# mattiagualtieri/multimodal-path-omic

Hardware: AMD Instinct MI355X
Metric: slides/sec (fwd+bwd) at 15k-patch bags (higher is better)
Workload: dtype bf16; 1 GPU; MCAT medium whole model fwd+bwd+Adam, 15000x1024 bf16 patch bag + 6x256 omic tokens per slide, ces loss; parallelism=dp1, resident_windows=2, launch=hipgraph(fwd+bwd+adam), setup_replays_before_warmup=40, training_state_rewound_every=48

## Files before the change

include/mpo_hip.h:

```cpp
#ifndef MPO_HIP_H
#define MPO_HIP_H
#include <stddef.h>
#include <stdint.h>

#define MPO_ABI_VERSION 14

#ifdef __cplusplus
extern "C" {
#endif

typedef struct ihipStream_t* mpo_stream_t;

enum { MPO_F32 = 0, MPO_BF16 = 1 };

typedef struct mpo_bag_plan {
    const int32_t* wg_start;
    int32_t n_wg;
    int32_t rows_per_wg;
} mpo_bag_plan;
int mpo_coattn_target_workgroups(void);
enum { MPO_ACT_NONE_ = 0, MPO_ACT_RELU_ = 1, MPO_ACT_ELU_ = 2, MPO_ACT_TANH_ = 3, MPO_ACT_SIGMOID_ = 4 };

int mpo_abi_version(void);
const char* mpo_last_error(void);

int mpo_linear_forward(const float* x, const float* weight, const float* bias, float* y,
                       int rows, int in_features, int out_features, float alpha, int act, mpo_stream_t stream);
int mpo_linear_backward_input(const float* dy, const float* weight, float* dx,
                              int rows, int in_features, int out_features, float alpha, int accumulate,
                              mpo_stream_t stream);
int mpo_linear_backward_weight(const float* dy, const float* x, float* dweight, float* dbias ,
                               int rows, int in_features, int out_features, float alpha, mpo_stream_t stream);

size_t mpo_coattn_saved_floats(int n_slides, int n_q, int embed);
size_t mpo_coattn_workspace_bytes(int n_slides, int n_q, int embed, int max_rows);
int mpo_coattn_mcat_forward(const void* bag, int bag_dtype, const int32_t* cu_rows, int n_slides,
                            int total_rows, int max_rows,
                            const float* query, int n_q, int embed,
                            const float* in_proj_weight, const float* in_proj_bias,
                            const float* out_proj_weight, const float* out_proj_bias,
                            float* out, float* attn_map, float* saved, const mpo_bag_plan* plan ,
                            void* workspace, size_t workspace_bytes, mpo_stream_t stream);
size_t mpo_patch_coattn_workspace_bytes(int n_slides, int n_q, int embed, int patch_dim);
int mpo_patch_coattn_mcat_forward(const void* patches, const int32_t* cu_rows, int n_slides, int total_rows, int max_rows,
                                  int patch_dim, const float* patch_weight, const float* patch_bias, float drop_p,
                                  uint64_t seed, uint64_t offset, const uint64_t* rng_epoch ,
                                  const float* query, int n_q, int embed,
                                  const float* in_proj_weight, const float* in_proj_bias,
                                  const float* out_proj_weight, const float* out_proj_bias,
                                  void* h_bag, float* out, float* attn_map , float* saved,
                                  const mpo_bag_plan* plan , void* workspace, size_t workspace_bytes,
                                  mpo_stream_t stream);
size_t mpo_patch_fc_workspace_bytes(int embed, int patch_dim);
int mpo_patch_fc_forward(const void* patches, const int32_t* cu_rows, int n_slides, int total_rows, int max_rows, int patch_dim,
                         const float* patch_weight, const float* patch_bias, int embed, float drop_p, uint64_t seed,
                         uint64_t offset, const uint64_t* rng_epoch, void* h_bag, const mpo_bag_plan* plan ,
                         void* workspace, size_t workspace_bytes, mpo_stream_t stream);
size_t mpo_patch_fc_f32_workspace_bytes(int backward);
int mpo_patch_fc_f32_forward(const float* patches, int64_t total_rows, int patch_dim, const float* patch_weight,
                             const float* patch_bias, int embed, float drop_p, uint64_t seed, uint64_t offset,
                             const uint64_t* rng_epoch, float x_scale, float* h_bag, void* workspace, size_t workspace_bytes,
                             mpo_stream_t stream);
int mpo_patch_fc_f32_backward(const float* d_h_bag, const float* h_bag , const float* patches, int64_t total_rows,
                              int embed, int patch_dim, float gate, float* d_weight, float* d_bias, void* workspace,
                              size_t workspace_bytes, mpo_stream_t stream);

int mpo_patch_coattn_fwd_bagpass(const void* patches, const void* w_packed, const float* bias, const int32_t* cu_rows, int n_slides,
                                 const float* qk2, void* h_bag, float* part_ml, float* part_ctx, int n_q, int max_rows,
                                 float drop_p, uint64_t seed, uint64_t offset, const mpo_bag_plan* plan ,
                                 mpo_stream_t stream);
int mpo_pack_patch_weight(const float* weight , void* packed, int embed, int patch_dim, mpo_stream_t stream);

int mpo_coattn_mcat_backward(const void* bag, int bag_dtype, const int32_t* cu_rows, int n_slides,
                             int total_rows, int max_rows,
                             const float* query, int n_q, int embed,
                             const float* in_proj_weight, const float* out_proj_weight,
                             const float* saved, const float* attn_map,
                             const float* d_out, const float* d_attn_map,
                             float* d_query, int d_query_accumulate ,
                             void* d_bag, float* d_bag_colsum ,
                             float* d_in_proj_weight, float* d_in_proj_bias,
                             float* d_out_proj_weight, float* d_out_proj_bias,
                             float bag_relu_gate, const mpo_bag_plan* plan ,
                             void* workspace, size_t workspace_bytes, mpo_stream_t stream);

int mpo_patch_epilogue_forward(void* h_bf16, const float* bias, int64_t rows, int cols, float drop_p, uint64_t seed,
                               uint64_t offset, const uint64_t* rng_epoch, mpo_stream_t stream);
size_t mpo_patch_epilogue_backward_workspace_bytes(int64_t n, int cols);
int mpo_patch_epilogue_backward(const void* h_bf16, const void* dy_bf16, void* g_bf16, int64_t n, int cols, float drop_p,
                                float* d_bias , void* workspace, size_t workspace_bytes, mpo_stream_t stream);
int mpo_colsum_bf16(const void* x_bf16, float* out, int64_t rows, int cols, mpo_stream_t stream);

size_t mpo_patch_weight_grad_workspace_bytes(int embed, int patch_dim);
int mpo_patch_weight_grad(const void* g_bf16, const void* patches_bf16, int64_t total_rows, int embed, int patch_dim,
                          float* d_weight, int workgroups, void* workspace, size_t workspace_bytes, mpo_stream_t stream);

int mpo_adam_step_flat(float* params, const float* grads, float* exp_avg, float* exp_avg_sq, int64_t n, float lr,
                       float beta1, float beta2, float eps, float weight_decay, int step,
                       const int32_t* step_dev ,
                       mpo_stream_t stream);

enum { MPO_OPTIM_ADAM = 0, MPO_OPTIM_ADAMAX = 1, MPO_OPTIM_ADADELTA = 2, MPO_OPTIM_SGD = 3 };
int mpo_optim_step_flat(int algorithm, float* params, const float* grads, float* state1, float* state2, int64_t n, float lr,
                        const float* lr_dev, float beta1, float beta2, float eps, float weight_decay, float l1, int step,
                        const int32_t* step_dev, mpo_stream_t stream);
size_t mpo_abs_sum_flat_workspace_bytes(int64_t n);
int mpo_abs_sum_flat(const float* x, int64_t n, float* out, void* workspace, size_t workspace_bytes, mpo_stream_t stream);

int mpo_set_gemm_fast_path(int enabled);

enum { MPO_GEMM_ROUTE_NONE = 0, MPO_GEMM_ROUTE_GENERAL_NB4 = 1, MPO_GEMM_ROUTE_GENERAL_NB8 = 2, MPO_GEMM_ROUTE_FAST = 3,
       MPO_GEMM_ROUTE_ROWS = 4, MPO_GEMM_ROUTE_LONGK = 5 };
int mpo_gemm_last_route(void);
int mpo_gemm_last_group_routes(void);

int mpo_set_coattn_bwd_two_wave(int enabled);

int mpo_set_coattn_bwd_f32_vector(int enabled);

int mpo_set_nacagat_one_pass_key_grad(int enabled);

int mpo_step_counters_bump(uint64_t* rng_epoch, int32_t* adam_step, mpo_stream_t stream);

int mpo_map_block_dot(const float* a_map, const float* b_map, const int32_t* cu_rows, int n_slides, int n_q, float* out,
                      mpo_stream_t stream);
int mpo_map_block_scale(const float* a_map, const float* scale, const int32_t* cu_rows, int n_slides, int n_q, float* out,
                        mpo_stream_t stream);

int mpo_key_projection(const void* hbag_bf16, int64_t rows, int embed, const float* w_k, const float* b_k, float* kbag,
                       mpo_stream_t stream);
size_t mpo_nacagat_saved_floats(int n_slides, int n_q, int embed);
size_t mpo_nacagat_workspace_bytes(int n_slides, int n_q, int embed, int max_rows, int total_rows);
int mpo_coattn_nacagat_forward(const void* kbag, int k_dtype, const void* hbag, int bag_dtype, const int32_t* cu_rows, int n_slides,
                               int total_rows, int max_rows, const float* query, int n_q, int embed,
                               const float* in_proj_weight, const float* in_proj_bias,
                               const float* out_proj_weight, const float* out_proj_bias,
                               float drop_p, uint64_t seed, uint64_t offset, const uint64_t* rng_epoch,
                               float* q_proj, float* out, float* attn_map, float* score_maps,
                               float* saved, const mpo_bag_plan* plan ,
                               void* workspace, size_t workspace_bytes, mpo_stream_t stream);
int mpo_coattn_nacagat_backward(const void* kbag, int k_dtype, const void* hbag, int bag_dtype,
                                const int32_t* cu_rows, int n_slides, int total_rows, int max_rows,
                                const float* query, int n_q, int embed,
                                const float* in_proj_weight, const float* in_proj_bias, const float* out_proj_weight,
                                float drop_p, uint64_t seed, uint64_t offset, const uint64_t* rng_epoch,
                                const float* saved, const float* score_maps, const float* attn_map,
                                const float* d_out, const float* d_attn_map, const float* d_q_proj,
                                float* d_query, int d_query_accumulate ,
                                void* d_kbag, int dk_dtype, float* d_kbag_colsum ,
                                void* d_hbag ,
                                float* d_ctx ,
                                float* d_in_proj_weight, float* d_in_proj_bias,
                                float* d_out_proj_weight, float* d_out_proj_bias, const mpo_bag_plan* plan ,
                                void* workspace, size_t workspace_bytes, mpo_stream_t stream);

int mpo_nacagat_patch_grad(const int32_t* cu_rows, int n_slides, int total_rows, int max_rows, int n_q, int embed,
                           const float* attn_map, const float* d_ctx, const void* addend_bf16, const void* hbag_bf16,
                           void* d_bag_bf16, float relu_gate, float* d_bias, const mpo_bag_plan* plan ,
                           void* workspace, size_t workspace_bytes, mpo_stream_t stream);

int mpo_nacagat_patch_grad_fused(const int32_t* cu_rows, int n_slides, int total_rows, int max_rows, int n_q, int embed,
                                 const float* attn_map, const float* d_ctx, const void* d_kbag_bf16, const float* w_k,
                                 const void* hbag_bf16, void* d_bag_bf16, float relu_gate, float* d_bias,
                                 const mpo_bag_plan* plan , void* workspace, size_t workspace_bytes,
                                 mpo_stream_t stream);


size_t mpo_encoder_saved_floats(int n_slides, int T, int d, int ff, int heads, int layers);
size_t mpo_encoder_workspace_bytes(int n_slides, int T, int d, int ff);
uint64_t mpo_encoder_rng_span(int n_slides, int T, int d, int ff, int layers);
int mpo_encoder_forward(const float* x, int n_branches, int n_slides, int T, int d, int ff, int heads, int layers,
                        const float* const* params, float drop_p, uint64_t seed, uint64_t offset, const uint64_t* rng_epoch,
                        float* y, float* saved, mpo_stream_t stream);
int mpo_encoder_backward(const float* x, int n_branches, int n_slides, int T, int d, int ff, int heads, int layers,
                         const float* const* params, float drop_p, uint64_t seed, uint64_t offset, const uint64_t* rng_epoch,
                         const float* saved, const float* dy, float* dx, float* const* grads,
                         void* workspace, size_t workspace_bytes, mpo_stream_t stream);

size_t mpo_bag_self_attention_saved_floats(int n_bags, int M, int d, int heads);
size_t mpo_bag_self_attention_workspace_bytes(int n_bags, int M, int d, int heads);
int mpo_set_bag_self_attention_bf16x3(int enabled);
int mpo_bag_self_attention_forward(const float* qkv, int n_bags, int M, int d, int heads, float drop_p, uint64_t seed, uint64_t offset,
                                   const uint64_t* rng_epoch, float* out, float* saved, float* attn_map, mpo_stream_t stream);
int mpo_bag_self_attention_backward(const float* qkv, const float* out, const float* saved, const float* d_out, int n_bags, int M, int d,
                                    int heads, float drop_p, uint64_t seed, uint64_t offset, const uint64_t* rng_epoch, float* d_qkv,
                                    void* workspace, size_t workspace_bytes, mpo_stream_t stream);

size_t mpo_gated_pool_saved_floats(int n_slides, int L, int d);
size_t mpo_gated_pool_workspace_bytes(int n_slides, int L, int d);
uint64_t mpo_gated_pool_rng_span(int n_slides, int L, int d);
int mpo_gated_pool_forward(const float* x, int n_branches, int n_slides, int L, int d, const float* const* params,
                           float head_drop_p, float rho_drop_p, uint64_t seed, uint64_t offset, const uint64_t* rng_epoch,
                           float* scores, float* h, int h_interleaved, float* saved, mpo_stream_t stream);
int mpo_gated_pool_backward(const float* x, int n_branches, int n_slides, int L, int d, const float* const* params,
                            float head_drop_p, float rho_drop_p, const float* saved, const float* h,
                            const float* dh, int h_interleaved, const float* d_scores_ext , float* dx,
                            float* const* grads,
                            void* workspace, size_t workspace_bytes, mpo_stream_t stream);

size_t mpo_fusion_head_saved_floats(int n_slides, int hidden, int dout, int n_classes);
size_t mpo_fusion_head_workspace_bytes(int n_slides, int hidden, int dout, int n_classes);
int mpo_fusion_head_forward(const float* hcat, int n_slides, int din, int hidden, int dout, int n_classes,
                            const float* const* params, float* hazards, float* survs, float* y, float* saved,
                            mpo_stream_t stream);
int mpo_fusion_head_backward(const float* hcat, int n_slides, int din, int hidden, int dout, int n_classes,
                             const float* const* params, const float* saved, const float* hazards,
                             const float* survs, const float* y, const float* d_hazards, const float* d_survs,
                             const float* d_y, float* d_hcat, float* const* grads,
                             void* workspace, size_t workspace_bytes, mpo_stream_t stream);

int mpo_survival_head_forward(const float* logits, int n_slides, int n_classes, float* hazards, float* survs, float* y,
                              mpo_stream_t stream);
int mpo_survival_head_backward(const float* hazards, const float* survs, const float* y, const float* d_hazards,
                               const float* d_survs, const float* d_y, int n_slides, int n_classes, float* d_logits,
                               mpo_stream_t stream);

int mpo_ces_loss_forward(const float* hazards, const float* survs, const int64_t* label, const float* censorship,
                         int n_slides, int n_classes, float alpha, float eps, float* loss, float* risk, mpo_stream_t stream);
int mpo_ces_loss_backward(const float* hazards, const float* survs, const int64_t* label, const float* censorship,
                          int n_slides, int n_classes, float alpha, float eps, const float* d_loss, int d_loss_is_scalar,
                          float* d_hazards, float* d_survs, mpo_stream_t stream);

size_t mpo_fusion_head_loss_saved_floats(int n_slides, int hidden, int dout, int n_classes);
int mpo_fusion_head_loss_forward(const float* hcat, int n_slides, int din, int hidden, int dout, int n_classes,
                                 const float* const* params, const int64_t* label, const float* censorship,
                                 const float* slide_weight, float alpha, float eps, float* hazards, float* survs, float* y,
                                 float* loss, float* risk , float* saved, mpo_stream_t stream);
int mpo_fusion_head_loss_backward(const float* hcat, int n_slides, int din, int hidden, int dout, int n_classes,
                                  const float* const* params, const float* saved, float* d_hcat, float* const* grads,
                                  void* workspace, size_t workspace_bytes, mpo_stream_t stream);

int mpo_sct_loss_forward(const float* y, const int64_t* label, const float* censorship, int n_slides, int n_classes,
                         float eps, float* loss, mpo_stream_t stream);
int mpo_sct_loss_backward(const float* y, const int64_t* label, const float* censorship, int n_slides, int n_classes,
                          float eps, const float* d_loss, int d_loss_is_scalar, float* d_y, mpo_stream_t stream);
int mpo_fusion_head_sct_loss_forward(const float* hcat, int n_slides, int din, int hidden, int dout, int n_classes,
                                     const float* const* params, const int64_t* label, const float* censorship,
                                     const float* slide_weight, float eps, float* hazards, float* survs, float* y,
                                     float* loss, float* risk , float* saved, mpo_stream_t stream);

int mpo_ge_head_loss_forward(const float* h, int n_bags, int d, int n_classes, const float* const* params,
                             const int64_t* label, float* y, float* loss, mpo_stream_t stream);
int mpo_ge_head_loss_backward(const float* h, int n_bags, int d, int n_classes, const float* const* params,
                              const int64_t* label, const float* d_loss, float* d_h, float* const* grads,
                              mpo_stream_t stream);

size_t mpo_cag_saved_floats(int rows, int hidden);
size_t mpo_cag_workspace_bytes(int rows, int hidden);
int mpo_cag_forward(const float* q, const float* q_hat, int rows, int dim, int hidden, const float* const* params,
                    float* c_out, float* saved, const float* residual ,
                    float* sum_out , mpo_stream_t stream);
int mpo_cag_backward(const float* q, const float* q_hat, int rows, int dim, int hidden, const float* const* params,
                     const float* saved, const float* c_out, const float* d_c, float* d_q, int d_q_accumulate, float* d_q_hat,
                     float* const* grads, void* workspace, size_t workspace_bytes, mpo_stream_t stream);

size_t mpo_omic_snn_saved_floats(int n_slides, int n_groups, int d);
size_t mpo_omic_snn_workspace_bytes(int n_slides, int n_groups, int d);
uint64_t mpo_omic_snn_rng_span(int n_slides, int n_groups, int d);
int mpo_omic_snn_forward(const float* const* x, const int* widths, int n_groups, int n_slides, int d,
                         const float* const* params, float drop_p, uint64_t seed, uint64_t offset,
                         const uint64_t* rng_epoch, float* g_bag, float* saved, mpo_stream_t stream);
int mpo_omic_snn_backward(const float* const* x, const int* widths, int n_groups, int n_slides, int d,
                          const float* const* params, float drop_p, uint64_t seed, uint64_t offset,
                          const uint64_t* rng_epoch, const float* g_bag, const float* saved, const float* d_g_bag,
                          float* const* grads, void* workspace, size_t workspace_bytes, mpo_stream_t stream);

int mpo_coattn_splits(int n_slides, int max_rows);
int mpo_coattn_fwd_bagpass(const void* bag, int bag_dtype, const int32_t* cu_rows, int n_slides, int embed,
                           const float* qk2, float* part_ml, float* part_ctx, float* raw_logits ,
                           int n_q, int max_rows, const mpo_bag_plan* plan , mpo_stream_t stream);
int mpo_nacagat_fwd_bagpass(const float* kbag, const int32_t* cu_rows, int n_slides, int embed, const float* qs2,
                            const float* tq, float* a_map, float* g_map, int n_q, int max_rows,
                            const mpo_bag_plan* plan , mpo_stream_t stream);
int mpo_coattn_bwd_bagpass(const void* bag, int bag_dtype, const int32_t* cu_rows, int n_slides, int embed,
                           const float* qk2, const float* lse2, const float* dctx, const float* delta,
                           const float* d_attn_map , void* d_bag, float* part_dqk,
                           int n_q, int max_rows, const mpo_bag_plan* plan , mpo_stream_t stream);

#include "mpo_bag_sample.h"

#include "mpo_fusion_next.h"

#include "mpo_cohort.h"

#include "mpo_feature_range.h"

#include "mpo_grad_guard.h"

#include "mpo_eval.h"

#include "mpo_classify.h"

#include "mpo_patch_f16.h"

#ifdef __cplusplus
}
#endif
#endif
```

multimodal_path_omic_amd/csrc/capi.hip:

```cpp
#include <stdarg.h>
#include <stdio.h>
#include <stdlib.h>

#include <algorithm>

#include "../../include/mpo_hip.h"
#include "coattn_tile.h"
#include "mpo_common.h"
#include "mpo_kernels.h"
#include "mpo_layout.h"

static thread_local char g_err[512] = "";

void mpo_set_error(const char* fmt, ...) {
    va_list ap;
    va_start(ap, fmt);
    vsnprintf(g_err, sizeof(g_err), fmt, ap);
    va_end(ap);
}

template <typename T> struct K1Saved { T *qs, *qk2, *ctx, *attn, *lse2; };
template <class A> K1Saved<typename A::elem> k1_saved(A& a, size_t R, size_t E) {
    return {a.floats(R * E), a.floats(R * E), a.floats(R * E), a.floats(R * E), a.floats(R)};
}
// ... 12 lines not shown
    return {a.floats(R * E), a.floats(R * E), a.floats(R * E), a.floats(R * E), a.floats(R * E), a.floats(R), a.floats(R)};
}
struct K2FwdWs { float *part, *hq1, *hq2, *hctx, *tmp_maps; };
template <class A> K2FwdWs k2_fwd_ws(A& a, size_t R, size_t parts, size_t n_q, size_t E, size_t total_rows) {
    K2FwdWs w{a.floats(parts * n_q * E), nullptr, nullptr, nullptr, nullptr};
    if (E == 512) { w.hq1 = a.floats(R * E / 2); w.hq2 = a.floats(R * E / 2); w.hctx = a.floats(R * E / 2); w.tmp_maps = a.floats(2 * n_q * total_rows); }
    return w;
}
struct K2BwdWs { float *dattn, *dctx, *dqt, *dtq, *dq, *spare, *dasum, *part, *part2, *part_cs, *ds1_map, *dg_map, *hb[6], *tmp_map; };
template <class A> K2BwdWs k2_bwd_ws(A& a, size_t R, size_t parts, size_t n_q, size_t E, size_t total_rows, bool colsum) {
    K2BwdWs w{a.floats(R * E), a.floats(R * E), a.floats(R * E), a.floats(R * E), a.floats(R * E), a.floats(R * E), a.floats(R),
              a.floats(parts * n_q * E), a.floats(parts * n_q * E), colsum ? a.floats(parts * E) : nullptr,
              a.floats(n_q * total_rows), a.floats(n_q * total_rows), {}, nullptr};
    if (E == 512) {
        for (float*& h : w.hb) h = a.floats(R * E / 2);
        w.tmp_map = a.floats(2 * n_q * total_rows);
    }
    return w;
}
template <class A> float* k2_patch_grad_ws(A& a, size_t parts, size_t E, bool colsum) { return colsum ? a.floats(parts * E) : nullptr; }

static size_t patch_weight_floats(int embed, int patch_dim) { return (size_t)(embed < 256 ? 256 : embed) * patch_dim / 2; }
static size_t patch_epilogue_bwd_floats(int64_t n, int cols) { return (size_t)mpo_relu_dropout_bwd_blocks((size_t)n, 1) * (size_t)cols; }
static size_t one_block_workspace_bytes(size_t n_floats) {
    WsCount c;
    c.floats(n_floats);
    return c.workspace_bytes();
}

namespace {
bool g_k2_one_pass_key = true;
}

extern "C" int mpo_coattn_target_workgroups(void) {
    return 256;
}

extern "C" int mpo_coattn_splits(int n_slides, int max_rows) {
    const int target = mpo_coattn_target_workgroups();
    int s = (target + n_slides - 1) / n_slides;
    if (s > 512) s = 512;
    const int cap = (max_rows + 127) / 128;
    if (s > cap) s = cap;
    if (s < 1) s = 1;
    return s;
}

static BagPlan make_plan(const mpo_bag_plan* p, int n_slides, int max_rows) {
    BagPlan pl;
    pl.n_slides = n_slides;
    if (p != nullptr && p->wg_start != nullptr) {
        pl.wg_start = p->wg_start;
        pl.n_wg = p->n_wg;
        pl.rows_per_wg = p->rows_per_wg;
    } else {
        pl.splits = mpo_coattn_splits(n_slides, max_rows);
    }
    return pl;
}
static int check_plan(const BagPlan& pl, int n_slides) {
    if (pl.wg_start == nullptr) return 0;
    MPO_CHECK(pl.rows_per_wg >= kTileRows && pl.rows_per_wg % kTileRows == 0, "bag plan: rows_per_wg %d must be a positive multiple of %d",
              pl.rows_per_wg, kTileRows);
    MPO_CHECK(pl.n_wg >= n_slides && pl.n_wg <= mpo_coattn_target_workgroups() + n_slides,
              "bag plan: n_wg %d outside [n_slides, target + n_slides]", pl.n_wg);
    return 0;
}
static size_t max_parts(int n_slides) { return (size_t)mpo_coattn_target_workgroups() + (size_t)n_slides; }

extern "C" {

int mpo_abi_version(void) { return MPO_ABI_VERSION; }
const char* mpo_last_error(void) { return g_err; }

int mpo_linear_forward(const float* x, const float* weight, const float* bias, float* y, int rows, int in_features,
                       int out_features, float alpha, int act, mpo_stream_t stream) {
    return mpo_linear_fwd(x, weight, bias, y, rows, in_features, out_features, alpha, act, stream);
}
int mpo_linear_backward_input(const float* dy, const float* weight, float* dx, int rows, int in_features,
                              int out_features, float alpha, int accumulate, mpo_stream_t stream) {
    return mpo_linear_bwd_input(dy, weight, dx, rows, in_features, out_features, alpha, accumulate, stream);
}
int mpo_linear_backward_weight(const float* dy, const float* x, float* dweight, float* dbias, int rows,
                               int in_features, int out_features, float alpha, mpo_stream_t stream) {
    return mpo_linear_bwd_weight(dy, x, dweight, dbias, rows, in_features, out_features, alpha, stream);
}
size_t mpo_coattn_saved_floats(int n_slides, int n_q, int embed) {
    Count<kPacked> c;
    k1_saved(c, (size_t)n_slides * n_q, embed);
    return c.n_floats();
}

size_t mpo_coattn_workspace_bytes(int n_slides, int n_q, int embed, int max_rows) {
    (void)max_rows;
    WsCount f, b;
    k1_fwd_ws(f, max_parts(n_slides), n_q, embed, 0);
    k1_bwd_ws(b, (size_t)n_slides * n_q, max_parts(n_slides), n_q, embed, true);
    return std::max(f.end, b.end) + kWorkspaceSlack;
}

static int check_common(int bag_dtype, int n_slides, int total_rows, int max_rows, int n_q, int embed) {
    MPO_CHECK(bag_dtype == MPO_F32 || bag_dtype == MPO_BF16, "bag dtype %d is neither MPO_F32 nor MPO_BF16", bag_dtype);
    MPO_CHECK(n_slides >= 1, "n_slides must be >= 1 (got %d)", n_slides);
    MPO_CHECK(n_q >= 1 && n_q <= 16, "number of omic queries must be in 1..16 (got %d)", n_q);
    MPO_CHECK(embed == 128 || embed == 256 || embed == 512, "embed_dim %d not in {128,256,512}", embed);
    MPO_CHECK(max_rows >= 1 && total_rows >= n_slides, "every slide needs at least one patch (total_rows %d, max_rows %d)",
              total_rows, max_rows);
    return 0;
}

struct PatchStep {
    const void* patches;
    const float *weight, *bias;
    int patch_dim;
    float drop_p;
    uint64_t seed, offset;
    const uint64_t* rng_epoch;
    void* h_bag;
};

static int k1_forward(const void* bag, int bag_f32, const PatchStep* patch, const int32_t* cu_rows, int n_slides, int max_rows,
                      const float* query, int n_q, int E, const float* in_w, const float* in_b, const float* out_w,
                      const float* out_b, float* out, float* attn_map, float* saved, const BagPlan& plan, const K1FwdWs& ws,
                      hipStream_t stream) {
    const int R = n_slides * n_q;
    Carve<kPacked> sv(saved);
    const K1Saved<float> S = k1_saved(sv, R, E);
    if (patch) RC(mpo_launch_pack_patch_weight(patch->weight, ws.w_bf16, E, patch->patch_dim, stream));
    RC(mpo_linear_fwd(query, in_w, in_b, S.qs, R, E, E, 1.0f / sqrtf((float)E), MPO_ACT_NONE, stream));
    RC(mpo_linear_bwd_input(S.qs, in_w + (size_t)E * E, S.qk2, R, E, E, kLog2e, 0, stream));
    if (patch) {
        RC(mpo_launch_patch_fc_fwd(patch->patches, ws.w_bf16, patch->bias, cu_rows, patch->h_bag, E, patch->patch_dim, patch->drop_p, patch->seed,
                                   patch->offset, reinterpret_cast<const unsigned long long*>(patch->rng_epoch), plan, stream));
        bag = patch->h_bag;
    }
    RC(mpo_launch_coattn_fwd_partial(bag, bag_f32, cu_rows, n_slides, E, S.qk2, ws.part_ml, ws.part_ctx, attn_map, n_q, plan, stream));
    RC(mpo_launch_coattn_combine(ws.part_ml, ws.part_ctx, S.ctx, S.lse2, n_slides, n_q, E, plan, stream));
    RC(mpo_linear_fwd(S.ctx, in_w + (size_t)2 * E * E, in_b + 2 * E, S.attn, R, E, E, 1.0f, MPO_ACT_NONE, stream));
    RC(mpo_linear_fwd(S.attn, out_w, out_b, out, R, E, E, 1.0f, MPO_ACT_NONE, stream));
    if (attn_map) RC(mpo_launch_coattn_normalize(attn_map, S.lse2, cu_rows, n_slides, n_q, max_rows, 0.f, 0, 0, stream));
    return 0;
}

int mpo_coattn_mcat_forward(const void* bag, int bag_dtype, const int32_t* cu_rows, int n_slides, int total_rows,
                            int max_rows, const float* query, int n_q, int embed, const float* in_w,
                            const float* in_b, const float* out_w, const float* out_b, float* out, float* attn_map,
                            float* saved, const mpo_bag_plan* plan_, void* workspace, size_t workspace_bytes,
                            mpo_stream_t stream) {
    RC(check_common(bag_dtype, n_slides, total_rows, max_rows, n_q, embed));
    const BagPlan plan = make_plan(plan_, n_slides, max_rows);
    RC(check_plan(plan, n_slides));
    WsCarve ws(workspace, workspace_bytes);
    const K1FwdWs W = k1_fwd_ws(ws, plan_parts(plan), n_q, embed, 0);
    MPO_CHECK(ws.ok(), "coattn forward: workspace too small (%zu bytes)", workspace_bytes);
    return k1_forward(bag, bag_dtype == MPO_F32, nullptr, cu_rows, n_slides, max_rows, query, n_q, embed, in_w, in_b, out_w, out_b,
                      out, attn_map, saved, plan, W, stream);
}

size_t mpo_patch_coattn_workspace_bytes(int n_slides, int n_q, int embed, int patch_dim) {
    WsCount c;
    k1_fwd_ws(c, max_parts(n_slides), n_q, embed, (size_t)embed * patch_dim / 2);
    return c.workspace_bytes();
}

int mpo_patch_coattn_mcat_forward(const void* patches, const int32_t* cu_rows, int n_slides, int total_rows, int max_rows,
                                  int patch_dim, const float* patch_weight, const float* patch_bias, float drop_p,
                                  uint64_t seed, uint64_t offset, const uint64_t* rng_epoch,
                                  const float* query, int n_q, int embed, const float* in_w, const float* in_b,
                                  const float* out_w, const float* out_b, void* h_bag, float* out, float* attn_map,
                                  float* saved, const mpo_bag_plan* plan_, void* workspace, size_t workspace_bytes,
                                  mpo_stream_t stream) {
    RC(check_common(MPO_BF16, n_slides, total_rows, max_rows, n_q, embed));
    MPO_CHECK(embed == 256 && patch_dim == 1024, "fused patch layer + co-attention is built for 1024 -> 256 (got %d -> %d)",
              patch_dim, embed);
    const BagPlan plan = make_plan(plan_, n_slides, max_rows);
    RC(check_plan(plan, n_slides));
    WsCarve ws(workspace, workspace_bytes);
    const K1FwdWs W = k1_fwd_ws(ws, plan_parts(plan), n_q, embed, (size_t)embed * patch_dim / 2);
    MPO_CHECK(ws.ok(), "fused patch layer + co-attention: workspace too small (%zu bytes)", workspace_bytes);
    const PatchStep patch{patches, patch_weight, patch_bias, patch_dim, drop_p, seed, offset, rng_epoch, h_bag};
    return k1_forward(nullptr, 0, &patch, cu_rows, n_slides, max_rows, query, n_q, embed, in_w, in_b, out_w, out_b, out, attn_map,
                      saved, plan, W, stream);
}

size_t mpo_patch_fc_workspace_bytes(int embed, int patch_dim) { return one_block_workspace_bytes(patch_weight_floats(embed, patch_dim)); }
int mpo_patch_fc_forward(const void* patches, const int32_t* cu_rows, int n_slides, int total_rows, int max_rows, int patch_dim,
                         const float* patch_weight, const float* patch_bias, int embed, float drop_p, uint64_t seed,
                         uint64_t offset, const uint64_t* rng_epoch, void* h_bag, const mpo_bag_plan* plan_, void* workspace,
                         size_t workspace_bytes, mpo_stream_t stream) {
    RC(check_common(MPO_BF16, n_slides, total_rows, max_rows, 1, embed));
    MPO_CHECK((embed == 128 || embed == 256 || embed == 512) && (patch_dim == 512 || patch_dim == 1024 || patch_dim == 2048),
              "patch layer kernel is built for patch_dim in {512, 1024, 2048} -> embed in {128, 256, 512} (got %d -> %d)", patch_dim, embed);
    MPO_CHECK((int64_t)max_rows * embed * 2 < ((int64_t)1 << 31), "patch layer: a slide's H_bag of 2 GiB or more (%d rows)", max_rows);
    const BagPlan plan = make_plan(plan_, n_slides, max_rows);
    RC(check_plan(plan, n_slides));
    WsCarve ws(workspace, workspace_bytes);
    float* w_bf16 = ws.floats(patch_weight_floats(embed, patch_dim));
    MPO_CHECK(ws.ok(), "patch layer: workspace too small (%zu bytes)", workspace_bytes);
    RC(mpo_launch_pack_patch_weight(patch_weight, w_bf16, embed, patch_dim, stream));
    return mpo_launch_patch_fc_fwd(patches, w_bf16, patch_bias, cu_rows, h_bag, embed, patch_dim, drop_p, seed, offset,
                                   reinterpret_cast<const unsigned long long*>(rng_epoch), plan, stream);
}

size_t mpo_patch_fc_f32_workspace_bytes(int backward) {
    return one_block_workspace_bytes(backward ? mpo_patch_wgrad_f32_workspace_floats() : mpo_patch_fc_f32_workspace_floats());
}
static int patch_fc_f32_forward(const float* patches, int64_t total_rows, int patch_dim, const float* patch_weight,
                                const float* patch_bias, int embed, float drop_p, uint64_t seed, uint64_t offset,
                                const uint64_t* rng_epoch, float x_scale, const float* x_scale_dev, float* h_bag, void* workspace,
                                size_t workspace_bytes, mpo_stream_t stream) {
    MPO_CHECK(patches && patch_weight && patch_bias && h_bag, "fp32 patch layer: null operand");
    MPO_CHECK(total_rows >= 1, "fp32 patch layer: total_rows %lld", (long long)total_rows);
    WsCarve ws(workspace, workspace_bytes);
    float* wpk = ws.floats(mpo_patch_fc_f32_workspace_floats());
    MPO_CHECK(ws.ok(), "fp32 patch layer: workspace too small (%zu bytes)", workspace_bytes);
    return mpo_launch_patch_fc_f32(patches, patch_weight, patch_bias, h_bag, total_rows, embed, patch_dim, drop_p, seed, offset,
                                   reinterpret_cast<const unsigned long long*>(rng_epoch), x_scale, x_scale_dev, wpk, stream);
}
int mpo_patch_fc_f32_forward(const float* patches, int64_t total_rows, int patch_dim, const float* patch_weight,
                             const float* patch_bias, int embed, float drop_p, uint64_t seed, uint64_t offset,
                             const uint64_t* rng_epoch, float x_scale, float* h_bag, void* workspace, size_t workspace_bytes,
                             mpo_stream_t stream) {
    return patch_fc_f32_forward(patches, total_rows, patch_dim, patch_weight, patch_bias, embed, drop_p, seed, offset, rng_epoch,
                                x_scale, nullptr, h_bag, workspace, workspace_bytes, stream);
}
int mpo_patch_fc_f32_forward_dev(const float* patches, int64_t total_rows, int patch_dim, const float* patch_weight,
                                 const float* patch_bias, int embed, float drop_p, uint64_t seed, uint64_t offset,
                                 const uint64_t* rng_epoch, const float* x_scale, float* h_bag, void* workspace,
                                 size_t workspace_bytes, mpo_stream_t stream) {
    MPO_CHECK(x_scale, "fp32 patch layer: null device scale (mpo_feature_range_f32 writes it)");
    return patch_fc_f32_forward(patches, total_rows, patch_dim, patch_weight, patch_bias, embed, drop_p, seed, offset, rng_epoch,
                                1.0f, x_scale, h_bag, workspace, workspace_bytes, stream);
}
int mpo_patch_fc_f32_backward(const float* d_h_bag, const float* h_bag, const float* patches, int64_t total_rows, int embed,
                              int patch_dim, float gate, float* d_weight, float* d_bias, void* workspace, size_t workspace_bytes,
                              mpo_stream_t stream) {
    MPO_CHECK(d_h_bag && patches && d_weight, "fp32 patch layer backward: null operand");
    MPO_CHECK(total_rows >= 1, "fp32 patch layer backward: total_rows %lld", (long long)total_rows);
    WsCarve ws(workspace, workspace_bytes);
    float* part = ws.floats(mpo_patch_wgrad_f32_workspace_floats());
    MPO_CHECK(ws.ok(), "fp32 patch layer backward: workspace too small (%zu bytes)", workspace_bytes);
    return mpo_launch_patch_wgrad_f32(d_h_bag, h_bag, patches, total_rows, embed, patch_dim, gate, d_weight, d_bias, part, stream);
}

size_t mpo_patch_fc_f16_workspace_bytes(int backward) {
    return one_block_workspace_bytes(backward ? mpo_patch_wgrad_f16x_workspace_floats() : mpo_patch_fc_f16_workspace_floats());
}
static int patch_f16_rate(int drop_256, float* p) {
    *p = (float)drop_256 / 256.0f;
    MPO_CHECK(drop_256 >= 0 && drop_256 <= 256, "patch-layer dropout p must be in [0,1) (got %f)", (double)*p);
    MPO_CHECK(drop_256 <= 255, "patch-layer dropout p = %g is realised as round(256 p) / 256 = %u/256: "
              "nothing would be kept (p must be below 1 - 1/512)", (double)*p, (unsigned)drop_256);
    return 0;
}
int mpo_patch_fc_f16_forward(const void* patches, int64_t total_rows, int patch_dim, const float* patch_weight,
                             const float* patch_bias, int embed, int drop_256, uint64_t seed, uint64_t offset,
                             const uint64_t* rng_epoch, float* h_bag, void* workspace, size_t workspace_bytes, mpo_stream_t stream) {
    MPO_CHECK(patches && patch_weight && patch_bias && h_bag, "fp16 patch layer: null operand");
    float drop_p;
    RC(patch_f16_rate(drop_256, &drop_p));
    MPO_CHECK(total_rows >= 1, "fp16 patch layer: total_rows %lld", (long long)total_rows);
    WsCarve ws(workspace, workspace_bytes);
    float* wpk = ws.floats(mpo_patch_fc_f16_workspace_floats());
    MPO_CHECK(ws.ok(), "fp16 patch layer: workspace too small (%zu bytes)", workspace_bytes);
    return mpo_launch_patch_fc_f16(patches, patch_weight, patch_bias, h_bag, total_rows, embed, patch_dim, drop_p, seed, offset,
                                   reinterpret_cast<const unsigned long long*>(rng_epoch), wpk, stream);
}
int mpo_patch_fc_f16_backward(const float* d_h_bag, const float* h_bag, const void* patches, int64_t total_rows, int embed,
                              int patch_dim, int drop_256, float* d_weight, float* d_bias, void* workspace, size_t workspace_bytes,
                              mpo_stream_t stream) {
    MPO_CHECK(d_h_bag && patches && d_weight, "fp16 patch layer backward: null operand");
    float drop_p;
    RC(patch_f16_rate(drop_256, &drop_p));
    const float gate = 256.0f / (256.0f - (float)drop_256);
    MPO_CHECK(total_rows >= 1, "fp16 patch layer backward: total_rows %lld", (long long)total_rows);
    WsCarve ws(workspace, workspace_bytes);
    float* part = ws.floats(mpo_patch_wgrad_f16x_workspace_floats());
    MPO_CHECK(ws.ok(), "fp16 patch layer backward: workspace too small (%zu bytes)", workspace_bytes);
    return mpo_launch_patch_wgrad_f16x(d_h_bag, h_bag, patches, total_rows, embed, patch_dim, gate, d_weight, d_bias, part, stream);
}

int mpo_patch_coattn_fwd_bagpass(const void* patches, const void* w_packed, const float* bias, const int32_t* cu_rows, int n_slides,
                                 const float* qk2, void* h_bag, float* part_ml, float* part_ctx, int n_q, int max_rows,
                                 float drop_p, uint64_t seed, uint64_t offset, const mpo_bag_plan* plan_, mpo_stream_t stream) {
    const BagPlan plan = make_plan(plan_, n_slides, max_rows);
    RC(check_plan(plan, n_slides));
    RC(mpo_launch_patch_fc_fwd(patches, w_packed, bias, cu_rows, h_bag, 256, 1024, drop_p, seed, offset, nullptr, plan, stream));
    if (qk2 == nullptr) return 0;
    return mpo_launch_coattn_fwd_partial(h_bag, 0, cu_rows, n_slides, 256, qk2, part_ml, part_ctx, nullptr, n_q, plan, stream);
}
int mpo_pack_patch_weight(const float* weight, void* packed, int embed, int patch_dim, mpo_stream_t stream) {
    return mpo_launch_pack_patch_weight(weight, packed, embed, patch_dim, stream);
}

int mpo_coattn_mcat_backward(const void* bag, int bag_dtype, const int32_t* cu_rows, int n_slides, int total_rows,
                             int max_rows, const float* query, int n_q, int embed, const float* in_w,
                             const float* out_w, const float* saved, const float* attn_map, const float* d_out,
                             const float* d_attn_map, float* d_query, int d_query_accumulate, void* d_bag,
                             float* d_bag_colsum, float* d_in_w,
                             float* d_in_b, float* d_out_w, float* d_out_b, float bag_relu_gate, const mpo_bag_plan* plan_,
                             void* workspace, size_t workspace_bytes, mpo_stream_t stream) {
    RC(check_common(bag_dtype, n_slides, total_rows, max_rows, n_q, embed));
    MPO_CHECK(!d_attn_map || attn_map, "coattn backward: a gradient on the attention map needs the forward's map");
    const int E = embed, R = n_slides * n_q;
    const BagPlan plan = make_plan(plan_, n_slides, max_rows);
    RC(check_plan(plan, n_slides));
    WsCarve ws(workspace, workspace_bytes);
    const K1BwdWs W = k1_bwd_ws(ws, R, plan_parts(plan), n_q, E, d_bag_colsum != nullptr);
    MPO_CHECK(ws.ok(), "coattn backward: workspace too small (%zu bytes)", workspace_bytes);
    Carve<kPacked, const float> sv(saved);
    const K1Saved<const float> S = k1_saved(sv, R, E);
    const float* w_q = in_w;
    const float* w_k = in_w + (size_t)E * E;
    const float* w_v = in_w + (size_t)2 * E * E;
    const float scale = 1.0f / sqrtf((float)E);
    RC(mpo_linear_bwd_pair(mpo_args_bwd_input(d_out, out_w, W.dattn, R, E, E, 1.0f, 0),
                           mpo_args_bwd_weight(d_out, S.attn, d_out_w, d_out_b, R, E, E, 1.0f), stream));
    RC(mpo_linear_bwd_pair(mpo_args_bwd_input(W.dattn, w_v, W.dctx, R, E, E, 1.0f, 0),
                           mpo_args_bwd_weight(W.dattn, S.ctx, d_in_w + (size_t)2 * E * E, d_in_b + 2 * E, R, E, E, 1.0f), stream));
    if (d_attn_map) {
        RC(mpo_launch_rowdot(W.dctx, S.ctx, W.delta, R, E, stream));
        RC(mpo_launch_map_rowdot(attn_map, d_attn_map, cu_rows, W.delta, n_slides, n_q, 1, stream));
    }
    RC(mpo_launch_coattn_bwd(bag, bag_dtype == MPO_F32, cu_rows, n_slides, E, S.qk2, S.lse2, W.dctx, d_attn_map ? W.delta : nullptr,
                             S.ctx, attn_map, d_attn_map, d_bag, W.part_dqk, W.part_cs, n_q, plan, bag_relu_gate, stream));
    {
        BagFinish f{};
        f.part[0] = W.part_dqk; f.out[0] = W.dqk; f.n_red = 1;
        f.part_cs = W.part_cs; f.colsum = d_bag_colsum; f.cs_cols = E;
        f.zero[0] = d_in_b + E; f.n_zero[0] = E;
        RC(mpo_launch_bag_finish(f, n_slides, n_q, E, plan, stream));
    }
    RC(mpo_gemm_together(stream, mpo_args_fwd(W.dqk, w_k, nullptr, W.dq_pre, R, E, E, scale, MPO_ACT_NONE),
                         mpo_args_bwd_weight(S.qs, W.dqk, d_in_w + (size_t)E * E, nullptr, R, E, E, 1.0f)));
    return mpo_linear_bwd_pair(mpo_args_bwd_input(W.dq_pre, w_q, d_query, R, E, E, 1.0f, d_query_accumulate ? 1 : 0),
                               mpo_args_bwd_weight(W.dq_pre, query, d_in_w, d_in_b, R, E, E, 1.0f), stream);
}

size_t mpo_nacagat_saved_floats(int n_slides, int n_q, int embed) {
    Count<kPacked> c;
    k2_saved(c, (size_t)n_slides * n_q, embed);
    return c.n_floats();
}
size_t mpo_nacagat_workspace_bytes(int n_slides, int n_q, int embed, int max_rows, int total_rows) {
    (void)max_rows;
    const size_t R = (size_t)n_slides * n_q, parts = max_parts(n_slides);
    WsCount f, b, p;
    k2_fwd_ws(f, R, parts, n_q, embed, total_rows);
    k2_bwd_ws(b, R, parts, n_q, embed, total_rows, true);
    k2_patch_grad_ws(p, parts, embed, true);
    return std::max({f.end, b.end, p.end}) + kWorkspaceSlack;
}

static int copy_cols(float* dst, size_t dst_ld, const float* src, size_t src_ld, int rows, int cols, hipStream_t s) {
    MPO_HIP(hipMemcpy2DAsync(dst, dst_ld * 4, src, src_ld * 4, (size_t)cols * 4, rows, hipMemcpyDeviceToDevice, s));
    return 0;
}

struct K2Call {
    BagPlan splits;
    int E, R, NH, EH, f32;
    size_t half_k, half_h, half_dk;
    hipStream_t stream;
    int take(const float*& half, const float* src, float* scratch, int h) const {
        half = NH > 1 ? scratch : src;
        return NH > 1 ? copy_cols(scratch, EH, src + h * EH, E, R, EH, stream) : 0;
    }
    float* put_to(float* dst, float* scratch) const { return NH > 1 ? scratch : dst; }
    int put(float* dst, const float* scratch, int h) const { return NH > 1 ? copy_cols(dst + h * EH, E, scratch, EH, R, EH, stream) : 0; }
    static float* map_to(float* map, float* tmp, int h) { return h == 0 ? map : tmp; }
    int map_add(float* map, const float* tmp, size_t n, int h) const { return h > 0 ? mpo_launch_ew_add(map, tmp, n, stream) : 0; }
};
static int k2_begin(K2Call& c, int k_dtype, int bag_dtype, int dk_dtype, int n_slides, int total_rows, int max_rows, int n_q, int embed,
                    float drop_p, const mpo_bag_plan* plan_, hipStream_t stream) {
    RC(check_common(bag_dtype, n_slides, total_rows, max_rows, n_q, embed));
    MPO_CHECK(drop_p >= 0.f && drop_p < 1.f, "attention dropout p must be in [0,1) (got %f)", (double)drop_p);
    MPO_CHECK(k_dtype == MPO_F32, "nacagat co-attention: K must be fp32 (k_dtype %d): the narrow gate amplifies key rounding", k_dtype);
    MPO_CHECK(dk_dtype == MPO_F32 || dk_dtype == MPO_BF16, "d_kbag dtype %d is neither MPO_F32 nor MPO_BF16", dk_dtype);
    const int f32 = bag_dtype == MPO_F32, NH = embed == 512 ? 2 : 1, EH = embed / NH;
    const size_t half = (size_t)total_rows * EH;
    c = {make_plan(plan_, n_slides, max_rows), embed, n_slides * n_q, NH, EH, f32, half * 4, half * (f32 ? 4 : 2),
         half * (dk_dtype == MPO_F32 ? 4 : 2), stream};
    return check_plan(c.splits, n_slides);
}

int mpo_coattn_nacagat_forward(const void* kbag, int k_dtype, const void* hbag, int bag_dtype, const int32_t* cu_rows, int n_slides,
                               int total_rows, int max_rows, const float* query, int n_q, int embed,
                               const float* in_w, const float* in_b, const float* out_w, const float* out_b,
                               float drop_p, uint64_t seed, uint64_t offset, const uint64_t* rng_epoch,
                               float* q_proj, float* out, float* attn_map, float* score_maps,
                               float* saved, const mpo_bag_plan* plan_, void* workspace, size_t workspace_bytes,
                               mpo_stream_t stream) {
    K2Call c;
    RC(k2_begin(c, k_dtype, bag_dtype, MPO_F32, n_slides, total_rows, max_rows, n_q, embed, drop_p, plan_, stream));
    const int E = c.E, R = c.R, NH = c.NH, EH = c.EH, f32 = c.f32;
    const BagPlan& splits = c.splits;
    WsCarve ws(workspace, workspace_bytes);
    const K2FwdWs W = k2_fwd_ws(ws, R, plan_parts(splits), n_q, E, total_rows);
    MPO_CHECK(ws.ok(), "nacagat forward: workspace too small (%zu bytes)", workspace_bytes);
    Carve<kPacked> sv(saved);
    const K2Saved<float> S = k2_saved(sv, R, E);
    const size_t map_n = (size_t)n_q * total_rows;
    float* a_map = score_maps;
    float* g_map = score_maps + map_n;
    RC(mpo_linear_fwd(query, in_w, in_b, q_proj, R, E, E, 1.0f, MPO_ACT_NONE, stream));
    RC(mpo_launch_qprep(q_proj, S.qt, S.qs2, S.tq, R * E, 1.0f / sqrtf((float)E), stream));
    for (int h = 0; h < NH; ++h) {
        const float *r1, *r2;
        RC(c.take(r1, S.qs2, W.hq1, h));
        RC(c.take(r2, S.tq, W.hq2, h));
        RC(mpo_launch_bag_rowdot_gated(static_cast<const char*>(kbag) + h * c.half_k, 1, cu_rows, n_slides, EH, r1, r2,
                                       c.map_to(a_map, W.tmp_maps, h), c.map_to(g_map, W.tmp_maps + map_n, h), n_q, splits, stream));
        RC(c.map_add(score_maps, W.tmp_maps, 2 * map_n, h));
    }
    RC(mpo_launch_gated_softmax_fwd(a_map, g_map, cu_rows, attn_map, S.lse2, S.asum, n_slides, n_q, drop_p, seed, offset,
                                    reinterpret_cast<const unsigned long long*>(rng_epoch), stream));
    for (int h = 0; h < NH; ++h) {
        RC(mpo_launch_bag_colacc(static_cast<const char*>(hbag) + h * c.half_h, f32, cu_rows, n_slides, EH, attn_map, W.part, n_q,
                                 splits, stream));
        RC(mpo_launch_coattn_bwd_reduce(W.part, c.put_to(S.ctx, W.hctx), n_slides, n_q, EH, splits, stream));
        RC(c.put(S.ctx, W.hctx, h));
    }
    RC(mpo_linear_fwd(S.ctx, in_w + (size_t)2 * E * E, nullptr, S.attn, R, E, E, 1.0f, MPO_ACT_NONE, stream));
    RC(mpo_launch_row_scaled_bias(S.attn, S.asum, in_b + 2 * E, R, E, stream));
    return mpo_linear_fwd(S.attn, out_w, out_b, out, R, E, E, 1.0f, MPO_ACT_NONE, stream);
}

int mpo_coattn_nacagat_backward(const void* kbag, int k_dtype, const void* hbag, int bag_dtype,
                                const int32_t* cu_rows, int n_slides, int total_rows, int max_rows,
                                const float* query, int n_q, int embed, const float* in_w, const float* in_b,
                                const float* out_w, float drop_p, uint64_t seed, uint64_t offset, const uint64_t* rng_epoch,
                                const float* saved, const float* score_maps, const float* attn_map,
                                const float* d_out, const float* d_attn_map, const float* d_q_proj,
                                float* d_query, int d_query_accumulate, void* d_kbag, int dk_dtype, float* d_kbag_colsum, void* d_hbag,
                                float* d_ctx, float* d_in_w, float* d_in_b, float* d_out_w, float* d_out_b,
                                const mpo_bag_plan* plan_, void* workspace, size_t workspace_bytes, mpo_stream_t stream) {
    K2Call c;
    RC(k2_begin(c, k_dtype, bag_dtype, dk_dtype, n_slides, total_rows, max_rows, n_q, embed, drop_p, plan_, stream));
    const int E = c.E, R = c.R, NH = c.NH, EH = c.EH, f32 = c.f32;
    const BagPlan& splits = c.splits;
    MPO_CHECK(d_ctx != nullptr || d_hbag != nullptr, "nacagat backward: neither d_hbag nor d_ctx given");
    WsCarve ws(workspace, workspace_bytes);
    const K2BwdWs W = k2_bwd_ws(ws, R, plan_parts(splits), n_q, E, total_rows, d_kbag_colsum != nullptr);
    MPO_CHECK(ws.ok(), "nacagat backward: workspace too small (%zu bytes)", workspace_bytes);
    float* dctx = d_ctx ? d_ctx : W.dctx;
    float* const* hb = W.hb;
    Carve<kPacked, const float> sv(saved);
    const K2Saved<const float> S = k2_saved(sv, R, E);
    const float* a_map = score_maps;
    const float* g_map = score_maps + (size_t)n_q * total_rows;
    const float* w_q = in_w;
    const float* w_v = in_w + (size_t)2 * E * E;
    const float* b_v = in_b + 2 * E;
    RC(mpo_linear_bwd_pair(mpo_args_bwd_input(d_out, out_w, W.dattn, R, E, E, 1.0f, 0),
                           mpo_args_bwd_weight(d_out, S.attn, d_out_w, d_out_b, R, E, E, 1.0f), stream));
    {
        const GemmArgs dbv = mpo_args_bwd_weight(S.asum, W.dattn, d_in_b + 2 * E, nullptr, R, E, 1, 1.0f);
        const GemmArgs das = mpo_args_fwd(W.dattn, b_v, nullptr, W.dasum, R, E, 1, 1.0f, MPO_ACT_NONE);
        RC(mpo_gemm_together(stream, mpo_args_bwd_input(W.dattn, w_v, dctx, R, E, E, 1.0f, 0),
                             mpo_args_bwd_weight(W.dattn, S.ctx, d_in_w + (size_t)2 * E * E, nullptr, R, E, E, 1.0f), &dbv, &das));
    }
    const float* dch[2];
    for (int h = 0; h < NH; ++h) {
        RC(c.take(dch[h], dctx, hb[h], h));
        RC(mpo_launch_bag_rowdot(static_cast<const char*>(hbag) + h * c.half_h, f32, cu_rows, n_slides, EH, dch[h],
                                 c.map_to(W.ds1_map, W.tmp_map, h), 1.0f, n_q, splits, stream));
        RC(c.map_add(W.ds1_map, W.tmp_map, (size_t)n_q * total_rows, h));
    }
    RC(mpo_launch_gated_softmax_bwd(a_map, g_map, cu_rows, S.lse2, W.dasum, d_attn_map, W.ds1_map, W.dg_map, n_slides, n_q, drop_p,
                                    seed, offset, reinterpret_cast<const unsigned long long*>(rng_epoch), stream));
    const bool one_pass = g_k2_one_pass_key && NH == 1 && n_q <= 6;
    for (int h = 0; h < NH && !one_pass; ++h) {
        RC(mpo_launch_bag_colacc_gated(static_cast<const char*>(kbag) + h * c.half_k, 1, cu_rows, n_slides, EH, W.ds1_map, W.dg_map,
                                       W.part, W.part2, n_q, splits, stream));
        BagFinish f{};
        f.part[0] = W.part; f.out[0] = c.put_to(W.dqt, hb[2]); f.part[1] = W.part2; f.out[1] = c.put_to(W.dtq, hb[3]); f.n_red = 2;
        RC(mpo_launch_bag_finish(f, n_slides, n_q, EH, splits, stream));
        RC(c.put(W.dqt, hb[2], h));
        RC(c.put(W.dtq, hb[3], h));
    }
    auto query_side = [&]() -> int {
        RC(mpo_launch_qprep_bwd(W.dqt, W.dtq, S.tq, d_q_proj, W.dq, R * E, 1.0f / sqrtf((float)E), stream));
        return mpo_linear_bwd_pair(mpo_args_bwd_input(W.dq, w_q, d_query, R, E, E, 1.0f, d_query_accumulate ? 1 : 0),
                                   mpo_args_bwd_weight(W.dq, query, d_in_w, d_in_b, R, E, E, 1.0f), stream);
    };
    if (!one_pass) RC(query_side());
    for (int h = 0; h < NH; ++h) {
        const float *qth, *tqh;
        RC(c.take(qth, S.qt, hb[4], h));
        RC(c.take(tqh, S.tq, hb[5], h));
        if (one_pass)
            RC(mpo_launch_bag_key_grad(reinterpret_cast<const float*>(kbag), cu_rows, n_slides, EH, W.ds1_map, qth, W.dg_map, tqh,
                                       d_kbag, dk_dtype == MPO_F32, W.part_cs, W.part, W.part2, n_q, splits, stream));
        else
            RC(mpo_launch_bag_outer_gated(reinterpret_cast<const float*>(static_cast<const char*>(kbag) + h * c.half_k), cu_rows,
                                          n_slides, EH, W.ds1_map, qth, W.dg_map, tqh, static_cast<char*>(d_kbag) + h * c.half_dk,
                                          dk_dtype == MPO_F32, W.part_cs, n_q, splits, stream));
        BagFinish f{};
        f.part_cs = d_kbag_colsum ? W.part_cs : nullptr; f.colsum = d_kbag_colsum ? d_kbag_colsum + h * EH : nullptr; f.cs_cols = EH;
        if (h == 0) {
            f.zero[0] = d_in_w + (size_t)E * E; f.n_zero[0] = E * E;
            if (d_kbag_colsum != d_in_b + E) { f.zero[1] = d_in_b + E; f.n_zero[1] = E; }
        }
        if (one_pass) { f.part[0] = W.part; f.out[0] = W.dqt; f.part[1] = W.part2; f.out[1] = W.dtq; f.n_red = 2; }
        RC(mpo_launch_bag_finish(f, n_slides, n_q, EH, splits, stream));
    }
    if (one_pass) RC(query_side());
    if (d_ctx == nullptr)
        for (int h = 0; h < NH; ++h)
            RC(mpo_launch_bag_outer(cu_rows, n_slides, EH, attn_map, dch[h], nullptr, nullptr,
                                    static_cast<char*>(d_hbag) + h * c.half_h, f32, n_q, splits, stream));
    return 0;
}

struct K2PatchGrad {
    BagPlan splits;
    float* part_cs;
};
static int k2_patch_grad_begin(K2PatchGrad& pg, int n_slides, int max_rows, int embed, bool colsum, const mpo_bag_plan* plan_,
                               void* workspace, size_t workspace_bytes) {
    pg.splits = make_plan(plan_, n_slides, max_rows);
    RC(check_plan(pg.splits, n_slides));
    WsCarve ws(workspace, workspace_bytes);
    pg.part_cs = k2_patch_grad_ws(ws, plan_parts(pg.splits), embed, colsum);
    MPO_CHECK(ws.ok(), "nacagat patch grad: workspace too small (%zu bytes)", workspace_bytes);
    return 0;
}
static int k2_patch_grad_end(const K2PatchGrad& pg, float* d_bias, int embed, hipStream_t stream) {
    return d_bias ? mpo_launch_colsum(pg.part_cs, d_bias, (int)plan_parts(pg.splits), embed, embed, 0, stream) : 0;
}

int mpo_nacagat_patch_grad(const int32_t* cu_rows, int n_slides, int total_rows, int max_rows, int n_q, int embed,
                           const float* attn_map, const float* d_ctx, const void* addend_bf16, const void* hbag_bf16,
                           void* d_bag_bf16, float relu_gate, float* d_bias, const mpo_bag_plan* plan_,
                           void* workspace, size_t workspace_bytes, mpo_stream_t stream) {
    RC(check_common(MPO_BF16, n_slides, total_rows, max_rows, n_q, embed));
    MPO_CHECK(attn_map && d_ctx && addend_bf16 && hbag_bf16 && d_bag_bf16, "nacagat patch grad: null operand");
    MPO_CHECK(((reinterpret_cast<uintptr_t>(addend_bf16) | reinterpret_cast<uintptr_t>(hbag_bf16) |
                reinterpret_cast<uintptr_t>(d_bag_bf16)) & 15) == 0, "nacagat patch grad: bag operands must be 16-byte aligned");
    K2PatchGrad pg;
    RC(k2_patch_grad_begin(pg, n_slides, max_rows, embed, d_bias != nullptr, plan_, workspace, workspace_bytes));
    RC(mpo_launch_bag_outer_gate(cu_rows, n_slides, embed, attn_map, d_ctx, addend_bf16, hbag_bf16, d_bag_bf16, relu_gate,
                                 pg.part_cs, n_q, pg.splits, stream));
    return k2_patch_grad_end(pg, d_bias, embed, stream);
}

int mpo_nacagat_patch_grad_fused(const int32_t* cu_rows, int n_slides, int total_rows, int max_rows, int n_q, int embed,
                                 const float* attn_map, const float* d_ctx, const void* d_kbag_bf16, const float* w_k,
                                 const void* hbag_bf16, void* d_bag_bf16, float relu_gate, float* d_bias,
                                 const mpo_bag_plan* plan_, void* workspace, size_t workspace_bytes, mpo_stream_t stream) {
    RC(check_common(MPO_BF16, n_slides, total_rows, max_rows, n_q, embed));
    MPO_CHECK(attn_map && d_ctx && d_kbag_bf16 && w_k && hbag_bf16 && d_bag_bf16, "nacagat patch grad: null operand");
    MPO_CHECK(d_bag_bf16 != d_kbag_bf16, "nacagat patch grad (fused): d_bag must not alias d_kbag");
    MPO_CHECK(((reinterpret_cast<uintptr_t>(d_kbag_bf16) | reinterpret_cast<uintptr_t>(hbag_bf16) |
                reinterpret_cast<uintptr_t>(d_bag_bf16)) & 15) == 0, "nacagat patch grad: bag operands must be 16-byte aligned");
    K2PatchGrad pg;
    RC(k2_patch_grad_begin(pg, n_slides, max_rows, embed, d_bias != nullptr, plan_, workspace, workspace_bytes));
    RC(mpo_launch_k2_patch_grad(cu_rows, d_kbag_bf16, w_k, attn_map, d_ctx, hbag_bf16, d_bag_bf16, relu_gate, pg.part_cs, n_q, embed,
                                pg.splits, stream));
    return k2_patch_grad_end(pg, d_bias, embed, stream);
}

int mpo_coattn_fwd_bagpass(const void* bag, int bag_dtype, const int32_t* cu_rows, int n_slides, int embed,
                           const float* qk2, float* part_ml, float* part_ctx, float* raw_logits, int n_q, int max_rows,
                           const mpo_bag_plan* plan_, mpo_stream_t stream) {
    const BagPlan plan = make_plan(plan_, n_slides, max_rows);
    RC(check_plan(plan, n_slides));
    return mpo_launch_coattn_fwd_partial(bag, bag_dtype == MPO_F32, cu_rows, n_slides, embed, qk2, part_ml, part_ctx,
                                         raw_logits, n_q, plan, stream);
}
int mpo_map_block_dot(const float* a_map, const float* b_map, const int32_t* cu_rows, int n_slides, int n_q, float* out,
                      mpo_stream_t stream) {
    MPO_CHECK(a_map && b_map && cu_rows && out && n_slides >= 1 && n_q >= 1, "map block dot: bad argument");
    return mpo_launch_map_rowdot(a_map, b_map, cu_rows, out, n_slides, n_q, 0, stream);
}
int mpo_map_block_scale(const float* a_map, const float* scale, const int32_t* cu_rows, int n_slides, int n_q, float* out,
                        mpo_stream_t stream) {
    MPO_CHECK(a_map && scale && cu_rows && out && n_slides >= 1 && n_q >= 1, "map block scale: bad argument");
    return mpo_launch_map_block_scale(a_map, scale, cu_rows, out, n_slides, n_q, stream);
}
int mpo_key_projection(const void* hbag_bf16, int64_t rows, int embed, const float* w_k, const float* b_k, float* kbag,
                       mpo_stream_t stream) {
    MPO_CHECK(rows >= 1 && rows <= 0x7fffffff, "key projection: %lld rows out of range", (long long)rows);
    return mpo_launch_key_proj(hbag_bf16, w_k, b_k, kbag, (int)rows, embed, stream);
}
int mpo_nacagat_fwd_bagpass(const float* kbag, const int32_t* cu_rows, int n_slides, int embed, const float* qs2,
                            const float* tq, float* a_map, float* g_map, int n_q, int max_rows, const mpo_bag_plan* plan_,
                            mpo_stream_t stream) {
    const BagPlan plan = make_plan(plan_, n_slides, max_rows);
    RC(check_plan(plan, n_slides));
    return mpo_launch_bag_rowdot_gated(kbag, 1, cu_rows, n_slides, embed, qs2, tq, a_map, g_map, n_q, plan, stream);
}
int mpo_coattn_bwd_bagpass(const void* bag, int bag_dtype, const int32_t* cu_rows, int n_slides, int embed,
                           const float* qk2, const float* lse2, const float* dctx, const float* delta,
                           const float* d_attn_map, void* d_bag, float* part_dqk, int n_q, int max_rows,
                           const mpo_bag_plan* plan_, mpo_stream_t stream) {
    const BagPlan plan = make_plan(plan_, n_slides, max_rows);
    RC(check_plan(plan, n_slides));
    MPO_CHECK(delta, "coattn backward bag pass: delta is required here");
    return mpo_launch_coattn_bwd(bag, bag_dtype == MPO_F32, cu_rows, n_slides, embed, qk2, lse2, dctx, delta, nullptr, nullptr,
                                 d_attn_map, d_bag, part_dqk, nullptr, n_q, plan, 0.f, stream);
}

int mpo_patch_epilogue_forward(void* h_bf16, const float* bias, int64_t rows, int cols, float drop_p, uint64_t seed,
                               uint64_t offset, const uint64_t* rng_epoch, mpo_stream_t stream) {
    MPO_CHECK(h_bf16 && bias, "patch epilogue: null operand");
    MPO_CHECK(rows >= 0, "patch epilogue: %lld rows", (long long)rows);
    MPO_CHECK(((reinterpret_cast<uintptr_t>(h_bf16) | reinterpret_cast<uintptr_t>(bias)) & 15) == 0,
              "patch epilogue: h and bias must be 16-byte aligned");
    return mpo_launch_bias_relu_dropout_bf16(h_bf16, bias, (size_t)rows, cols, drop_p, seed, offset,
                                             reinterpret_cast<const unsigned long long*>(rng_epoch), stream);
}
int mpo_colsum_bf16(const void* x_bf16, float* out, int64_t rows, int cols, mpo_stream_t stream) {
    MPO_CHECK(x_bf16 && out, "bf16 column sum: null operand");
    MPO_CHECK(rows >= 0, "bf16 column sum: %lld rows", (long long)rows);
    MPO_CHECK((reinterpret_cast<uintptr_t>(x_bf16) & 15) == 0, "bf16 column sum: x must be 16-byte aligned (bf16 x 8 loads)");
    return mpo_launch_colsum_bf16(x_bf16, out, (size_t)rows, cols, stream);
}
size_t mpo_patch_epilogue_backward_workspace_bytes(int64_t n, int cols) { return one_block_workspace_bytes(patch_epilogue_bwd_floats(n, cols)); }
int mpo_patch_epilogue_backward(const void* h_bf16, const void* dy_bf16, void* g_bf16, int64_t n, int cols, float drop_p,
                                float* d_bias, void* workspace, size_t workspace_bytes, mpo_stream_t stream) {
    MPO_CHECK(h_bf16 && dy_bf16 && g_bf16, "patch epilogue backward: null operand");
    MPO_CHECK(((reinterpret_cast<uintptr_t>(h_bf16) | reinterpret_cast<uintptr_t>(dy_bf16) |
                reinterpret_cast<uintptr_t>(g_bf16)) & 15) == 0,
              "patch epilogue backward: h, dy and g must be 16-byte aligned (bf16 x 8 loads)");
    if (!d_bias) return mpo_launch_relu_dropout_bwd_bf16(h_bf16, dy_bf16, g_bf16, (size_t)n, drop_p, cols, nullptr, stream);
    WsCarve ws(workspace, workspace_bytes);
    float* part = ws.floats(patch_epilogue_bwd_floats(n, cols));
    MPO_CHECK(workspace && ws.ok(), "patch epilogue backward: workspace too small (%zu bytes)", workspace_bytes);
    RC(mpo_launch_relu_dropout_bwd_bf16(h_bf16, dy_bf16, g_bf16, (size_t)n, drop_p, cols, part, stream));
    return mpo_launch_colsum(part, d_bias, mpo_relu_dropout_bwd_blocks((size_t)n, 1), cols, cols, 0, stream);
}

size_t mpo_patch_weight_grad_workspace_bytes(int embed, int patch_dim) {
    return one_block_workspace_bytes(mpo_patch_wgrad_partial_floats(embed, patch_dim));
}
int mpo_patch_weight_grad(const void* g_bf16, const void* patches_bf16, int64_t total_rows, int embed, int patch_dim,
                          float* d_weight, int workgroups, void* workspace, size_t workspace_bytes, mpo_stream_t stream) {
    MPO_CHECK(g_bf16 && patches_bf16 && d_weight, "patch weight gradient: null argument");
    MPO_CHECK(total_rows >= 1 && total_rows < (int64_t)1 << 31, "patch weight gradient: %lld rows", (long long)total_rows);
    WsCarve ws(workspace, workspace_bytes);
    float* part = ws.floats(mpo_patch_wgrad_partial_floats(embed, patch_dim));
    MPO_CHECK(ws.ok(), "patch weight gradient: workspace too small (%zu bytes)", workspace_bytes);
    return mpo_launch_patch_wgrad(g_bf16, patches_bf16, total_rows, embed, patch_dim, part, d_weight, workgroups,
                                  static_cast<hipStream_t>(stream));
}

int mpo_adam_step_flat(float* params, const float* grads, float* exp_avg, float* exp_avg_sq, int64_t n, float lr,
                       float beta1, float beta2, float eps, float weight_decay, int step, const int32_t* step_dev,
                       mpo_stream_t stream) {
    MPO_CHECK(step >= 1 || step_dev, "adam: step counts from 1 (got %d)", step);
    return mpo_launch_adam_flat(params, grads, exp_avg, exp_avg_sq, (size_t)n, lr, beta1, beta2, eps, weight_decay,
                                step < 1 ? 1 : step, step_dev, stream);
}

int mpo_optim_step_flat(int algorithm, float* params, const float* grads, float* state1, float* state2, int64_t n, float lr,
                        const float* lr_dev, float beta1, float beta2, float eps, float weight_decay, float l1, int step,
                        const int32_t* step_dev, mpo_stream_t stream) {
    MPO_CHECK(algorithm >= MPO_OPTIM_ADAM && algorithm <= MPO_OPTIM_SGD, "flat optimiser: unknown algorithm %d", algorithm);
    MPO_CHECK(n >= 0, "flat optimiser: n = %lld", (long long)n);
    MPO_CHECK(params && grads, "flat optimiser: null parameter or gradient buffer");
    const bool stateful = algorithm != MPO_OPTIM_SGD;
    MPO_CHECK(!stateful || (state1 && state2), "flat optimiser: algorithm %d needs both state buffers", algorithm);
    const auto misaligned = [](const void* q) { return (reinterpret_cast<uintptr_t>(q) & 3u) != 0; };
    MPO_CHECK(!misaligned(params) && !misaligned(grads) && !misaligned(state1) && !misaligned(state2) && !misaligned(lr_dev) &&
              !misaligned(step_dev), "flat optimiser: buffers must be 4-byte aligned");
    const bool counted = algorithm == MPO_OPTIM_ADAM || algorithm == MPO_OPTIM_ADAMAX;
    MPO_CHECK(!counted || step >= 1 || step_dev, "flat optimiser: step counts from 1 (got %d)", step);
    return mpo_launch_optim_flat(algorithm, params, grads, state1, state2, (size_t)n, lr, lr_dev, beta1, beta2, eps,
                                 weight_decay, l1, step < 1 ? 1 : step, step_dev, static_cast<hipStream_t>(stream));
}
size_t mpo_abs_sum_flat_workspace_bytes(int64_t n) {
    return n < 0 ? 0 : mpo_abs_sum_partials((size_t)n) * sizeof(float);
}
int mpo_abs_sum_flat(const float* x, int64_t n, float* out, void* workspace, size_t workspace_bytes, mpo_stream_t stream) {
    MPO_CHECK(n >= 1, "abs sum: n = %lld", (long long)n);
    MPO_CHECK(x && out && workspace, "abs sum: null argument");
    MPO_CHECK((reinterpret_cast<uintptr_t>(x) & 3u) == 0 && (reinterpret_cast<uintptr_t>(out) & 3u) == 0 &&
              (reinterpret_cast<uintptr_t>(workspace) & 3u) == 0, "abs sum: pointers must be 4-byte aligned");
    MPO_CHECK(workspace_bytes >= mpo_abs_sum_flat_workspace_bytes(n), "abs sum: workspace too small (%zu bytes)",
              workspace_bytes);
    return mpo_launch_abs_sum(x, (size_t)n, static_cast<float*>(workspace), out, static_cast<hipStream_t>(stream));
}

int mpo_set_gemm_fast_path(int enabled) { return mpo_gemm_fast_path(enabled); }
int mpo_gemm_last_route(void) { return mpo_gemm_route_last(); }
int mpo_gemm_last_group_routes(void) { return mpo_gemm_route_group_take(); }
int mpo_set_coattn_bwd_two_wave(int enabled) { return mpo_coattn_bwd8_enable(enabled); }
int mpo_set_coattn_bwd_f32_vector(int enabled) { return mpo_coattn_bwd_f32_enable(enabled); }
int mpo_set_nacagat_one_pass_key_grad(int enabled) {
    const int was = g_k2_one_pass_key ? 1 : 0;
    g_k2_one_pass_key = enabled != 0;
    return was;
}

int mpo_step_counters_bump(uint64_t* rng_epoch, int32_t* adam_step, mpo_stream_t stream) {
    MPO_CHECK(rng_epoch || adam_step, "step counters: nothing to bump");
    return mpo_launch_counters_bump(reinterpret_cast<unsigned long long*>(rng_epoch), adam_step, static_cast<hipStream_t>(stream));
}

}
```

multimodal_path_omic_amd/csrc/coattn_bwd8.hip:

```cpp
#include "coattn_tile.h"
#include "mpo_kernels.h"

namespace {

constexpr int E8 = 256;
constexpr int W8 = 8;
constexpr int QS = 8;
using G8 = TileGeom<E8>;
constexpr int OFF_Z8 = W8 * G8::TILEB;
constexpr int Z8_BYTES = G8::DT * 32 * 16;
constexpr int OFF_QF8 = OFF_Z8 + Z8_BYTES;
constexpr int QF8_ARR = G8::KS * 4 * QS * 16;
constexpr int LDS8 = OFF_QF8 + 4 * QF8_ARR;
static_assert(LDS8 <= 160 * 1024, "LDS budget");

__device__ __forceinline__ int sw8(int r) { return ((r & 7) << 1) ^ ((r >> 4) & 1); }
__device__ __forceinline__ bf16x8 row_frag8(const char* tile, int pt, int s, int lane) {
    const int p = lane & 15, g = lane >> 4;
    const int c = (4 * s + g) ^ ((lane & 7) << 1) ^ pt;
    return *reinterpret_cast<const bf16x8*>(tile + (16 * pt + p) * G8::ROWB + (c << 4));
}
__device__ __forceinline__ bf16x8 col_frag8(const char* tile, int t, int lane) {
    const int i = lane & 15, g = lane >> 4;
    const int q4 = i >> 2, p4 = i & 3;
    const int r0 = 4 * g + q4;
    const int c = (2 * t + (p4 >> 1)) ^ ((r0 & 7) << 1);
    const int off = r0 * G8::ROWB + 8 * (p4 & 1);
    s16x4 a = __builtin_amdgcn_ds_read_tr16_b64_v4i16(LDS_PTR(s16x4, tile + off + (c << 4)));
    s16x4 b = __builtin_amdgcn_ds_read_tr16_b64_v4i16(LDS_PTR(s16x4, tile + off + ((c ^ 1) << 4) + 16 * G8::ROWB));
    typedef __attribute__((ext_vector_type(8))) short s16x8;
    s16x8 v = {a[0], a[1], a[2], a[3], b[0], b[1], b[2], b[3]};
    return __builtin_bit_cast(bf16x8, v);
}

__device__ __forceinline__ unsigned lds_addr8(const char* p) {
    return (unsigned)(uintptr_t)(__attribute__((address_space(3))) const char*)p;
}
__device__ __forceinline__ void glds16_8(const char* src, unsigned lds_dst) {
#pragma clang diagnostic push
#pragma clang diagnostic ignored "-Winline-asm"
    asm volatile("s_mov_b32 m0, %1\n\ts_nop 0\n\tglobal_load_lds_dwordx4 %0, off" :: "v"(src), "s"(lds_dst) : "memory", "m0");
#pragma clang diagnostic pop
}

typedef __attribute__((ext_vector_type(4))) unsigned u32x4;

__global__ __launch_bounds__(W8 * 64, 1)
void coattn_bwd8_kernel(const __bf16* __restrict__ bag, const int* __restrict__ cu,
                        const float* __restrict__ qk2,
                        const float* __restrict__ lse2,
                        const float* __restrict__ dctx,
                        const float* __restrict__ delta,
                        const float* __restrict__ ctx,
                        __bf16* __restrict__ dbag,
                        float* __restrict__ part_dqk,
                        float* __restrict__ part_colsum,
                        int n_q, BagPlan plan,
                        float relu_gate ) {
    __shared__ __attribute__((aligned(1024))) char lds[LDS8];
    const int tid = threadIdx.x;
    const int lane = tid & 63;
    const int wave = __builtin_amdgcn_readfirstlane(tid >> 6);
    const WgGeom wg = wg_geom(cu, plan);
    const int b = wg.b, row_begin = wg.row_begin, m_rows = wg.m_rows, r0 = wg.r0, r1 = wg.r1, ntiles = wg.ntiles;
    const int n_my = wave < ntiles ? (ntiles - wave + W8 - 1) / W8 : 0;
    const int c16 = lane & 15, g = lane >> 4;
    const float* qk_b = qk2 + (size_t)b * n_q * E8;
    const float* dc_b = dctx + (size_t)b * n_q * E8;
    char* img = lds + wave * G8::TILEB;
    const unsigned img_lds = lds_addr8(img);
    const char* slide = reinterpret_cast<const char*>(bag) + (size_t)row_begin * G8::ROWB;
    char* dslide = reinterpret_cast<char*>(dbag) + (size_t)row_begin * G8::ROWB;

    auto issue_tile = [&](int trow) {
        int el = lane;
        asm volatile("" : "+v"(el));
        const int rl = el >> 5, cpos = el & 31;
#pragma unroll
        for (int i = 0; i < 16; ++i) {
            const int r = 2 * i + rl;
            const int c = cpos ^ sw8(r);
            const int grow = min(trow + r, m_rows - 1);
            glds16_8(slide + (size_t)grow * G8::ROWB + (c << 4), img_lds + i * 1024);
        }
    };
    if (n_my > 0) issue_tile(r0 + kTileRows * wave);

    {
        for (int e = tid; e < 2 * G8::KS * 4 * QS; e += W8 * 64) {
            const int slot = e % QS;
            int rest = e / QS;
            const int gg = rest & 3;
            rest >>= 2;
            const int s = rest & (G8::KS - 1), pair = rest >> 3;
            const float* row = (pair ? dc_b : qk_b) + (slot < n_q ? slot : 0) * E8 + 32 * s + 8 * gg;
            const float live = slot < n_q ? 1.0f : 0.0f;
            const f32x4 a = *reinterpret_cast<const f32x4*>(row), c = *reinterpret_cast<const f32x4*>(row + 4);
            float v[8];
#pragma unroll
            for (int j = 0; j < 4; ++j) {
                v[j] = a[j] * live;
                v[4 + j] = c[j] * live;
            }
            bf16x8 h, l;
            pack_hi_lo(v, h, l);
            char* dst = lds + OFF_QF8 + (2 * pair) * QF8_ARR + (((s * 4 + gg) * QS + slot) << 4);
            *reinterpret_cast<bf16x8*>(dst) = h;
            *reinterpret_cast<bf16x8*>(dst + QF8_ARR) = l;
        }
        const float zs = relu_gate != 0.f ? relu_gate : 1.0f;
        for (int e = tid; e < G8::DT * 32; e += W8 * 64) {
            const int i = e & 15, gg = (e >> 4) & 1, t = e >> 5;
            float z[8];
#pragma unroll
            for (int j = 0; j < 4; ++j) {
                const int qq = 4 * gg + j;
                const int qc = qq < n_q ? qq : n_q - 1;
                const float live = qq < n_q ? zs : 0.0f;
                z[j] = dc_b[qc * E8 + 16 * t + i] * live;
                z[4 + j] = qk_b[qc * E8 + 16 * t + i] * (live * kLn2);
            }
            bf16x8 h, l;
            pack_hi_lo(z, h, l);
            *reinterpret_cast<bf16x8*>(lds + OFF_Z8 + (e << 4)) = h;
        }
    }
    const float lse_q = c16 < n_q ? lse2[(size_t)b * n_q + c16] : INFINITY;
    float del_q, lse_p[4], del_p[4];
    if (delta != nullptr) {
        del_q = c16 < n_q ? delta[(size_t)b * n_q + c16] : 0.f;
#pragma unroll
        for (int r = 0; r < 4; ++r) del_p[r] = 4 * g + r < n_q ? delta[(size_t)b * n_q + 4 * g + r] : 0.f;
    } else {
        const float* cx_b = ctx + (size_t)b * n_q * E8;
        float acc = 0.f;
        if (c16 < n_q) {
#pragma unroll 4
            for (int e = g * (E8 / 4); e < (g + 1) * (E8 / 4); e += 4) {
                const f32x4 u = *reinterpret_cast<const f32x4*>(dc_b + c16 * E8 + e);
                const f32x4 v = *reinterpret_cast<const f32x4*>(cx_b + c16 * E8 + e);
                acc += (u[0] * v[0] + u[1] * v[1]) + (u[2] * v[2] + u[3] * v[3]);
            }
        }
        acc += __shfl_xor(acc, 16, 64);
        acc += __shfl_xor(acc, 32, 64);
        del_q = c16 < n_q ? acc : 0.f;
#pragma unroll
        for (int r = 0; r < 4; ++r) {
            const float t = __shfl(acc, 4 * g + r, 64);
            del_p[r] = 4 * g + r < n_q ? t : 0.f;
        }
    }
#pragma unroll
    for (int r = 0; r < 4; ++r) lse_p[r] = 4 * g + r < n_q ? lse2[(size_t)b * n_q + 4 * g + r] : INFINITY;
    __syncthreads();

    f32x4 accq[G8::DT];
#pragma unroll
    for (int t = 0; t < G8::DT; ++t) accq[t] = f32x4{0.f, 0.f, 0.f, 0.f};
    float csum[8];
#pragma unroll
    for (int j = 0; j < 8; ++j) csum[j] = 0.f;
    const bool gate_on = relu_gate != 0.f;

    for (int it = 0; it < n_my; ++it) {
        const int trow = r0 + kTileRows * (wave + it * W8);
        const int nvalid = min(kTileRows, r1 - trow);
        int el = lane;
        asm volatile("" : "+v"(el));
        const int ec = el & 15, eg = el >> 4;
        asm volatile("s_waitcnt vmcnt(0)" ::: "memory");

        bf16x8 wph[2], wh, wl;
        {
            f32x4 sT[2], dT[2], sN[2], dN[2];
#pragma unroll
            for (int pt = 0; pt < 2; ++pt) sT[pt] = dT[pt] = sN[pt] = dN[pt] = f32x4{0.f, 0.f, 0.f, 0.f};
            const char* qf = lds + OFF_QF8 + ((eg * QS + (ec & 7)) << 4);
#pragma unroll
            for (int s = 0; s < G8::KS; ++s) {
                const bf16x8 a0 = row_frag8(img, 0, s, el);
                const bf16x8 a1 = row_frag8(img, 1, s, el);
                const char* qs = qf + s * (4 * QS * 16);
                const bf16x8 qh = *reinterpret_cast<const bf16x8*>(qs);
                const bf16x8 ql = *reinterpret_cast<const bf16x8*>(qs + QF8_ARR);
                const bf16x8 dh = *reinterpret_cast<const bf16x8*>(qs + 2 * QF8_ARR);
                const bf16x8 dl = *reinterpret_cast<const bf16x8*>(qs + 3 * QF8_ARR);
                sT[0] = mfma_bf16(qh, a0, sT[0]);
                sT[1] = mfma_bf16(qh, a1, sT[1]);
                dT[0] = mfma_bf16(dh, a0, dT[0]);
                dT[1] = mfma_bf16(dh, a1, dT[1]);
                sN[0] = mfma_bf16(a0, qh, sN[0]);
                sN[1] = mfma_bf16(a1, qh, sN[1]);
                dN[0] = mfma_bf16(a0, dh, dN[0]);
                dN[1] = mfma_bf16(a1, dh, dN[1]);
                sT[0] = mfma_bf16(ql, a0, sT[0]);
                sT[1] = mfma_bf16(ql, a1, sT[1]);
                dT[0] = mfma_bf16(dl, a0, dT[0]);
                dT[1] = mfma_bf16(dl, a1, dT[1]);
                sN[0] = mfma_bf16(a0, ql, sN[0]);
                sN[1] = mfma_bf16(a1, ql, sN[1]);
                dN[0] = mfma_bf16(a0, dl, dN[0]);
                dN[1] = mfma_bf16(a1, dl, dN[1]);
            }
#pragma unroll
            for (int pt = 0; pt < 2; ++pt) {
                const bool ok = 16 * pt + ec < nvalid;
                float w[8];
#pragma unroll
                for (int r = 0; r < 4; ++r) {
                    const float a = ok ? __builtin_amdgcn_exp2f(sT[pt][r] - lse_p[r]) : 0.f;
                    w[r] = a;
                    w[4 + r] = a * (dT[pt][r] - del_p[r]);
                }
                bf16x8 lo_unused;
                pack_hi_lo(w, wph[pt], lo_unused);
            }
            float ds[8];
#pragma unroll
            for (int pt = 0; pt < 2; ++pt)
#pragma unroll
                for (int r = 0; r < 4; ++r) {
                    const bool ok = 16 * pt + 4 * eg + r < nvalid;
                    const float a = ok ? __builtin_amdgcn_exp2f(sN[pt][r] - lse_q) : 0.f;
                    ds[4 * pt + r] = a * (dN[pt][r] - del_q);
                }
            pack_hi_lo(ds, wh, wl);
        }
#pragma unroll
        for (int t = 0; t < G8::DT; ++t) {
            const bf16x8 hf = col_frag8(img, t, el);
            accq[t] = mfma_bf16(hf, wh, accq[t]);
            accq[t] = mfma_bf16(hf, wl, accq[t]);
        }

        {
            const int row = 16 * (eg & 1) + ec;
            char* rowp = img + row * G8::ROWB;
            const int swz = sw8(row), chi = eg >> 1;
            const char* zf = lds + OFF_Z8 + ((((eg & 1) << 4) + ec) << 4);
#pragma unroll
            for (int t = 0; t < G8::DT; ++t) {
                const bf16x8 zh = *reinterpret_cast<const bf16x8*>(zf + t * 512);
                const f32x4 z4 = {0.f, 0.f, 0.f, 0.f};
                const f32x4 o0 = mfma_bf16(zh, wph[0], z4);
                const f32x4 o1 = mfma_bf16(zh, wph[1], z4);
                const bf16x4 b0 = {f2bf(o0[0]), f2bf(o0[1]), f2bf(o0[2]), f2bf(o0[3])};
                const bf16x4 b1 = {f2bf(o1[0]), f2bf(o1[1]), f2bf(o1[2]), f2bf(o1[3])};
                typedef __attribute__((ext_vector_type(2))) unsigned u32x2;
                const u32x2 x = __builtin_bit_cast(u32x2, b0), y = __builtin_bit_cast(u32x2, b1);
                const auto s0 = __builtin_amdgcn_permlane16_swap(x[0], y[0], false, false);
                const auto s1 = __builtin_amdgcn_permlane16_swap(x[1], y[1], false, false);
                u32x4 out = {s0[0], s1[0], s0[1], s1[1]};
                u32x4* slot = reinterpret_cast<u32x4*>(rowp + (((2 * t + chi) ^ swz) << 4));
                if (gate_on) {
                    const u32x4 hv = *slot;
#pragma unroll
                    for (int k = 0; k < 4; ++k) {
                        const unsigned u = ((hv[k] & 0x7FFF7FFFu) + 0x7FFF7FFFu) & 0x80008000u;
                        out[k] &= __umul24(u >> 15, 0xFFFFu);
                    }
                }
                *slot = out;
            }
        }
        __builtin_amdgcn_fence(__ATOMIC_RELEASE, "wavefront");
        __builtin_amdgcn_wave_barrier();

        {
            const int rl = el >> 5, cc = el & 31;
#pragma unroll
            for (int i = 0; i < 16; ++i) {
                const int r = 2 * i + rl;
                const f32x4 v = *reinterpret_cast<const f32x4*>(img + r * G8::ROWB + ((cc ^ sw8(r)) << 4));
                if (r < nvalid) *reinterpret_cast<f32x4*>(dslide + ((size_t)(trow + r) * 32 + cc) * 16) = v;
                if (part_colsum != nullptr) {
                    const bf16x8 hv = __builtin_bit_cast(bf16x8, v);
#pragma unroll
                    for (int j = 0; j < 8; ++j) csum[j] += (float)hv[j];
                }
            }
        }
        asm volatile("s_waitcnt lgkmcnt(0)" ::: "memory");
        if (it + 1 < n_my) issue_tile(trow + kTileRows * W8);
    }

    asm volatile("s_waitcnt vmcnt(0)" ::: "memory");
    __syncthreads();
    {
        float* wq = reinterpret_cast<float*>(img);
#pragma unroll
        for (int t = 0; t < G8::DT; ++t)
            *reinterpret_cast<f32x4*>(wq + c16 * E8 + 16 * t + 4 * g) = accq[t];
    }
    __syncthreads();
    const size_t pbase = wg.part;
    for (int idx = tid; idx < n_q * E8; idx += W8 * 64) {
        float a = 0.f;
#pragma unroll
        for (int w = 0; w < W8; ++w) a += reinterpret_cast<const float*>(lds + w * G8::TILEB)[idx];
        part_dqk[pbase * n_q * E8 + idx] = a;
    }
    if (part_colsum != nullptr) {
        __syncthreads();
#pragma unroll
        for (int j = 0; j < 8; ++j) csum[j] += __shfl_xor(csum[j], 32);
        float* wc = reinterpret_cast<float*>(img);
        if (lane < 32) {
#pragma unroll
            for (int j = 0; j < 8; ++j) wc[lane * 8 + j] = csum[j];
        }
        __syncthreads();
        for (int idx = tid; idx < E8; idx += W8 * 64) {
            float a = 0.f;
#pragma unroll
            for (int w = 0; w < W8; ++w) a += reinterpret_cast<const float*>(lds + w * G8::TILEB)[idx];
            part_colsum[pbase * E8 + idx] = a;
        }
    }
}

int g_bwd8_enabled = 1;

}

int mpo_coattn_bwd8_enable(int enabled) {
    const int prev = g_bwd8_enabled;
    g_bwd8_enabled = enabled ? 1 : 0;
    return prev;
}

bool mpo_coattn_bwd8_covers(int bag_f32, int embed, int n_q, const float* da_map) {
    return g_bwd8_enabled && !bag_f32 && embed == E8 && n_q >= 1 && n_q <= 8 && da_map == nullptr;
}

int mpo_launch_coattn_bwd8(const void* bag, const int* cu, const float* qk2, const float* lse2, const float* dctx,
                           const float* delta, const float* ctx, void* dbag, float* part_dqk, float* part_colsum, int n_q,
                           const BagPlan& plan, float relu_gate, hipStream_t stream) {
    MPO_CHECK(n_q >= 1 && n_q <= 8, "coattn backward (8 waves): 1..8 queries (got %d)", n_q);
    MPO_CHECK(delta || ctx, "coattn backward: delta or ctx");
    coattn_bwd8_kernel<<<plan_grid(plan), W8 * 64, 0, stream>>>(
        reinterpret_cast<const __bf16*>(bag), cu, qk2, lse2, dctx, delta, ctx, reinterpret_cast<__bf16*>(dbag), part_dqk,
        part_colsum, n_q, plan, relu_gate);
    MPO_LAUNCH_CHECK();
    return 0;
}
```

multimodal_path_omic_amd/csrc/mpo_kernels.h:

```cpp
#pragma once
#include <hip/hip_runtime.h>
#include <stddef.h>

#include <stdint.h>
enum { MPO_ACT_NONE = 0, MPO_ACT_RELU = 1, MPO_ACT_ELU = 2, MPO_ACT_TANH = 3, MPO_ACT_SIGMOID = 4 };
enum { MPO_GATE_NONE = 0, MPO_GATE_RELU = 1, MPO_GATE_ELU = 2, MPO_GATE_TANH = 3, MPO_GATE_SIGMOID = 4,
       MPO_GATE_RNG = 5, MPO_GATE_MUL = 6, MPO_GATE_ELU_ADROP = 7 };

struct GemmArgs {
    const float* A = nullptr;
    const float* B = nullptr;
    float* C = nullptr;
    const float* bias = nullptr;
    const float* residual = nullptr;
    const float* mask = nullptr;
    int M = 0, N = 0, K = 0;
    int lda = 0, ldb = 0, ldc = 0;
    float alpha = 1.0f;
    int act = MPO_ACT_NONE;
    int accumulate = 0;
    int alpha_dropout = 0;
    float drop_p = 0.f;
    uint64_t drop_seed = 0, drop_off = 0;
    const float* gate = nullptr;
    int gate_mode = MPO_GATE_NONE;
    float gate_p = 0.f;
    uint64_t gate_seed = 0, gate_off = 0;
    float* bias_grad = nullptr;
    const unsigned long long* rng_epoch = nullptr;
    int layout = 3;
};

struct DropSpec {
    float p = 0.f;
    uint64_t seed = 0, off = 0;
    const unsigned long long* epoch = nullptr;
};
struct GateSpec {
    const float* g = nullptr;
    int mode = MPO_GATE_NONE;
    float p = 0.f;
    uint64_t seed = 0, off = 0;
    const unsigned long long* epoch = nullptr;
};

int mpo_launch_gemm(const GemmArgs& g, int a_kc, int b_kc, hipStream_t stream);
struct GemmGroup {
    GemmArgs g[8];
    int n = 0;
};
int mpo_launch_gemm_group(const GemmGroup& grp, int a_kc, int b_kc, hipStream_t stream);
int mpo_launch_gemm_mixed(const GemmGroup& grp, hipStream_t stream);
int mpo_launch_colsum(const float* x, float* out, int M, int N, int ld, int accumulate, hipStream_t stream);

inline GemmArgs mpo_args_fwd(const float* x, const float* w, const float* b, float* y, int R, int I, int O,
                             float alpha, int act, const float* residual = nullptr, DropSpec drop = DropSpec()) {
    GemmArgs g;
    g.A = x; g.B = w; g.C = y; g.bias = b; g.residual = residual;
    g.M = R; g.N = O; g.K = I; g.lda = I; g.ldb = I; g.ldc = O; g.alpha = alpha; g.act = act;
    g.drop_p = drop.p; g.drop_seed = drop.seed; g.drop_off = drop.off; g.rng_epoch = drop.epoch;
    g.layout = 3;
    return g;
}
inline int mpo_linear_fwd(const float* x, const float* w, const float* b, float* y, int R, int I, int O,
                          float alpha, int act, hipStream_t s, const float* residual = nullptr,
                          DropSpec drop = DropSpec()) {
    return mpo_launch_gemm(mpo_args_fwd(x, w, b, y, R, I, O, alpha, act, residual, drop), 1, 1, s);
}
inline GemmArgs mpo_args_bwd_input(const float* dy, const float* w, float* dx, int R, int I, int O, float alpha,
                                   int accumulate, GateSpec gate = GateSpec()) {
    GemmArgs g;
    g.A = dy; g.B = w; g.C = dx;
    g.M = R; g.N = I; g.K = O; g.lda = O; g.ldb = I; g.ldc = I; g.alpha = alpha; g.accumulate = accumulate;
    g.gate = gate.g; g.gate_mode = gate.mode; g.gate_p = gate.p; g.gate_seed = gate.seed; g.gate_off = gate.off;
    g.rng_epoch = gate.epoch;
    g.layout = 2;
    return g;
}
inline int mpo_linear_bwd_input(const float* dy, const float* w, float* dx, int R, int I, int O, float alpha,
                                int accumulate, hipStream_t s, GateSpec gate = GateSpec()) {
    return mpo_launch_gemm(mpo_args_bwd_input(dy, w, dx, R, I, O, alpha, accumulate, gate), 1, 0, s);
}
inline GemmArgs mpo_args_bwd_weight(const float* dy, const float* x, float* dw, float* db, int R, int I, int O,
                                    float alpha, GateSpec gate = GateSpec()) {
    GemmArgs g;
    g.A = dy; g.B = x; g.C = dw;
    g.M = O; g.N = I; g.K = R; g.lda = O; g.ldb = I; g.ldc = I; g.alpha = alpha;
    g.gate = gate.g; g.gate_mode = gate.mode; g.gate_p = gate.p; g.gate_seed = gate.seed; g.gate_off = gate.off;
    g.rng_epoch = gate.epoch;
    g.bias_grad = db;
    g.layout = 0;
    return g;
}
inline int mpo_linear_bwd_weight(const float* dy, const float* x, float* dw, float* db, int R, int I, int O,
                                 float alpha, hipStream_t s, GateSpec gate = GateSpec()) {
    return mpo_launch_gemm(mpo_args_bwd_weight(dy, x, dw, db, R, I, O, alpha, gate), 0, 0, s);
}
inline int mpo_linear_bwd_pair(const GemmArgs& dx, const GemmArgs& dw, hipStream_t s) {
    GemmGroup grp;
    grp.g[0] = dx; grp.g[1] = dw; grp.n = 2;
    return mpo_launch_gemm_mixed(grp, s);
}
inline int mpo_gemm_together(hipStream_t s, const GemmArgs& a, const GemmArgs& b, const GemmArgs* c = nullptr,
                             const GemmArgs* d = nullptr) {
    GemmGroup grp;
    grp.g[0] = a; grp.g[1] = b; grp.n = 2;
    if (c) grp.g[grp.n++] = *c;
    if (d) grp.g[grp.n++] = *d;
    return mpo_launch_gemm_mixed(grp, s);
}

struct BagPlan;
extern "C" int mpo_coattn_splits(int n_slides, int max_rows);
int mpo_launch_pack_patch_weight(const float* w, void* out, int embed, int patch_dim, hipStream_t stream);
int mpo_launch_patch_fc_fwd(const void* x, const void* w_packed, const float* bias, const int* cu, void* h_out, int embed, int patch_dim,
                            float drop_p, unsigned long long seed, unsigned long long offset, const unsigned long long* epoch,
                            const BagPlan& plan, hipStream_t stream);
int mpo_launch_coattn_fwd_partial(const void* bag, int bag_f32, const int* cu, int n_slides, int embed,
                                  const float* qk2, float* part_ml, float* part_ctx, float* s_out,
                                  int n_q, const BagPlan& plan, hipStream_t stream);
int mpo_launch_coattn_combine(const float* part_ml, const float* part_ctx, float* ctx, float* lse2,
                              int n_slides, int n_q, int embed, const BagPlan& plan, hipStream_t stream);
int mpo_launch_coattn_normalize(float* a, const float* lse2, const int* cu, int n_slides, int n_q, int max_rows,
                                float drop_p, unsigned long long seed, unsigned long long offset, hipStream_t stream);
int mpo_launch_coattn_bwd(const void* bag, int bag_f32, const int* cu, int n_slides, int embed,
                          const float* qk2, const float* lse2, const float* dctx, const float* delta ,
                          const float* ctx, const float* a_map, const float* da_map,
                          void* dbag, float* part_dqk, float* part_colsum , int n_q, const BagPlan& plan,
                          float relu_gate, hipStream_t stream);
bool mpo_coattn_bwd8_covers(int bag_f32, int embed, int n_q, const float* da_map);
int mpo_coattn_bwd_f32_enable(int enabled);
bool mpo_coattn_bwd_f32_covers(int bag_f32, int embed, int n_q, const float* da_map);
int mpo_launch_coattn_bwd_f32(const void* bag, const int* cu, const float* qk2, const float* lse2, const float* dctx,
                              const float* delta, const float* ctx, const float* da_map, void* dbag, float* part_dqk,
                              float* part_colsum, int n_q, const BagPlan& plan, hipStream_t stream);
int mpo_coattn_bwd8_enable(int enabled);
int mpo_launch_coattn_bwd8(const void* bag, const int* cu, const float* qk2, const float* lse2, const float* dctx,
                           const float* delta, const float* ctx, void* dbag, float* part_dqk, float* part_colsum, int n_q,
                           const BagPlan& plan, float relu_gate, hipStream_t stream);
size_t mpo_patch_fc_f32_workspace_floats();
size_t mpo_patch_wgrad_f32_workspace_floats();
int mpo_launch_patch_fc_f32(const float* x, const float* w, const float* bias, float* h, long long total_rows, int embed,
                            int patch_dim, float drop_p, unsigned long long seed, unsigned long long offset,
                            const unsigned long long* epoch, float x_scale, const float* x_scale_dev ,
                            float* ws, hipStream_t stream);
int mpo_launch_patch_wgrad_f32(const float* dh, const float* hbag, const float* x, long long total_rows, int embed, int patch_dim,
                               float gate, float* d_weight, float* d_bias, float* ws, hipStream_t stream);
size_t mpo_patch_fc_f16_workspace_floats();
size_t mpo_patch_wgrad_f16x_workspace_floats();
int mpo_launch_patch_fc_f16(const void* x, const float* w, const float* bias, float* h, long long total_rows, int embed,
                            int patch_dim, float drop_p, unsigned long long seed, unsigned long long offset,
                            const unsigned long long* epoch, float* ws, hipStream_t stream);
int mpo_launch_patch_wgrad_f16x(const float* dh, const float* hbag, const void* x, long long total_rows, int embed, int patch_dim,
                                float gate, float* d_weight, float* d_bias, float* ws, hipStream_t stream);
int mpo_launch_k2_patch_grad(const int* cu, const void* dk_bf16, const float* w_k, const float* amap, const float* dctx,
                             const void* hbag_bf16, void* out_bf16, float gate, float* part_colsum, int n_q, int embed,
                             const BagPlan& plan, hipStream_t stream);
int mpo_gemm_fast_path(int enabled);
int mpo_gemm_route_last();
int mpo_gemm_route_group_take();
size_t mpo_patch_wgrad_partial_floats(int embed, int patch_dim);
int mpo_launch_patch_wgrad(const void* g_bf16, const void* x_bf16, int64_t total_rows, int embed, int patch_dim, float* part,
                           float* d_weight, int workgroups, hipStream_t stream);
struct BagFinish {
    const float* part[2];
    float* out[2];
    int n_red;
    const float* part_cs;
    float* colsum;
    int cs_cols;
    float* zero[2];
    int n_zero[2];
};
int mpo_launch_bag_finish(const BagFinish& f, int n_slides, int n_q, int embed, const BagPlan& plan, hipStream_t stream);
int mpo_launch_coattn_bwd_reduce(const float* part_dqk, float* dqk, int n_slides, int n_q, int embed, const BagPlan& plan,
                                 hipStream_t stream);
int mpo_launch_rowdot(const float* a, const float* b, float* out, int rows, int cols, hipStream_t stream);
int mpo_launch_map_block_scale(const float* a_map, const float* scale, const int* cu, float* out, int n_slides, int n_q,
                               hipStream_t stream);
int mpo_launch_map_rowdot(const float* a_map, const float* da_map, const int* cu, float* delta, int n_slides, int n_q,
                          int accumulate, hipStream_t stream);

int mpo_launch_bag_rowdot(const void* bag, int bag_f32, const int* cu, int n_slides, int embed, const float* r,
                          float* map, float alpha, int n_q, const BagPlan& plan, hipStream_t stream);
int mpo_launch_bag_colacc(const void* bag, int bag_f32, const int* cu, int n_slides, int embed, const float* wmap,
                          float* part, int n_q, const BagPlan& plan, hipStream_t stream);
int mpo_launch_bag_outer(const int* cu, int n_slides, int embed, const float* w1, const float* z1, const float* w2,
                         const float* z2, void* dx, int out_f32, int n_q, const BagPlan& plan, hipStream_t stream);
int mpo_launch_gated_softmax_fwd(const float* amap_a, const float* gmap, const int* cu, float* out_map, float* lse2,
                                 float* asum, int n_slides, int n_q, float drop_p, unsigned long long seed,
                                 unsigned long long offset, const unsigned long long* epoch, hipStream_t stream);
int mpo_launch_gated_softmax_bwd(const float* amap_a, const float* gmap, const int* cu, const float* lse2,
                                 const float* dasum, const float* d_ext, float* da_map, float* dg_map, int n_slides,
                                 int n_q, float drop_p, unsigned long long seed, unsigned long long offset,
                                 const unsigned long long* epoch, hipStream_t stream);
int mpo_launch_qprep(const float* q, float* qt, float* qs2, float* tq, int n, float c_nat, hipStream_t stream);
int mpo_launch_qprep_bwd(const float* dqt, const float* dtq, const float* tq, const float* d_ext, float* dq, int n,
                         float c_nat, hipStream_t stream);
int mpo_launch_row_scaled_bias(float* y, const float* s, const float* bias, int rows, int cols, hipStream_t stream);

constexpr int kMaxBranches = 4;
struct LnBranches {
    const float* w[kMaxBranches] = {};
    const float* b[kMaxBranches] = {};
    float* dw[kMaxBranches] = {};
    float* db[kMaxBranches] = {};
    int rows_per_branch = 0, n = 0;
};
int mpo_launch_ln_fwd_br(const float* x, const LnBranches& p, float* y, float* stats, int rows, int d, float eps, hipStream_t s);
int mpo_launch_ln_bwd_br(const float* dy, const float* x, const float* stats, const LnBranches& p, float* dx, int rows, int d,
                         int accumulate, int what, hipStream_t s);
int mpo_launch_ln_bwd_params_only(const float* dy, const float* x, const float* stats, float* dw, float* db, int rows, int d,
                                  hipStream_t s);
constexpr int kSmallAttnMaxT = 16;
int mpo_bag_sa_supported_head_dim(int hd);
int mpo_bag_sa_set_bf16x3(int enabled);
size_t mpo_bag_sa_saved_floats(int n_seq, int M, int d, int H);
size_t mpo_bag_sa_bwd_floats(int n_seq, int M, int d, int H);
int mpo_launch_bag_sa_fwd(const float* qkv, int n_seq, int M, int d, int H, float drop_p, unsigned long long seed,
                          unsigned long long offset, const unsigned long long* epoch, float* o, float* saved, float* map, hipStream_t s);
int mpo_launch_bag_sa_bwd(const float* qkv, const float* o, const float* saved, const float* d_o, int n_seq, int M, int d, int H,
                          float drop_p, unsigned long long seed, unsigned long long offset, const unsigned long long* epoch,
                          float* dqkv, float* scratch, hipStream_t s);
int mpo_check_mha_small(int T, int d, int H);
int mpo_launch_mha_small_fwd(const float* qkv, float* o, float* p_save, int B, int T, int d, int H, float drop_p,
                             unsigned long long seed, unsigned long long offset, const unsigned long long* epoch,
                             hipStream_t s);
int mpo_launch_mha_small_bwd(const float* qkv, const float* p_save, const float* d_o, float* dqkv, int B, int T, int d, int H,
                             hipStream_t s);
struct PoolScorer {
    const float* wc[2] = {nullptr, nullptr};
    const float* bc[2] = {nullptr, nullptr};
    float* dwc[2] = {nullptr, nullptr};
    float* dbc[2] = {nullptr, nullptr};
    int n_slides = 1;
};
int mpo_launch_pool_score_fwd(const float* a, const float* b, const float* x, const PoolScorer& ps, float* scores, float* w,
                              float* h, int B, int L, int d, hipStream_t s);
int mpo_launch_pool_score_bwd(const float* dh, const float* x, const float* w, const float* d_ext, const float* a, const float* b,
                              const PoolScorer& ps, float* d_scores, float* dx, float* da, float* db, int B, int L, int d,
                              hipStream_t s);
int mpo_launch_pool_fwd(const float* scores, const float* x, float* w, float* h, int B, int L, int d, hipStream_t s);
int mpo_launch_pool_bwd(const float* dh, const float* x, const float* w, const float* d_ext, float* d_scores, float* dx,
                        int B, int L, int d, hipStream_t s);
int mpo_head_max_classes();
int mpo_launch_head_fwd(const float* logits, float* hazards, float* survs, float* y, int B, int C, hipStream_t s);
int mpo_launch_head_loss(const float* logits, const long long* label, const float* cens, const float* w, float* hazards,
                         float* survs, float* y, float* loss, float* risk, float* dlogits, int B, int C, float alpha,
                         float eps, hipStream_t s);
int mpo_launch_sct_loss_fwd(const float* y, const long long* label, const float* cens, float* loss, int B, int C, float eps,
                            hipStream_t s);
int mpo_launch_sct_loss_bwd(const float* y, const long long* label, const float* cens, const float* d_loss,
                            int d_loss_scalar, float* d_y, int B, int C, float eps, hipStream_t s);
int mpo_launch_head_sct_loss(const float* logits, const long long* label, const float* cens, const float* w, float* hazards,
                             float* survs, float* y, float* loss, float* risk, float* dlogits, int B, int C, float eps,
                             hipStream_t s);
int mpo_launch_counters_bump(unsigned long long* epoch, int* step, hipStream_t s);
int mpo_launch_head_bwd(const float* hazards, const float* survs, const float* y, const float* dhz, const float* dsv,
                        const float* dy, float* dlogits, int B, int C, hipStream_t s);
int mpo_check_gate_concat(const float* x0, const float* x1, int ldx, int n_slides, int d);
int mpo_launch_gate_concat_fwd(const float* x0, const float* x1, int ldx, const float* const* params, float* hcat, float* g,
                               int n_slides, int d, hipStream_t s);
int mpo_launch_gate_concat_bwd(const float* x0, const float* x1, int ldx, const float* const* params, const float* d_hcat,
                               const float* g, float* t, float* dx0, float* dx1, float* const* grads, int n_slides, int d,
                               hipStream_t s);
unsigned long long mpo_bilinear_stream_stride(int n_slides);
int mpo_check_bilinear(const float* x0, const float* x1, int ldx, int n_slides, int d, int hidden, int mm_hidden);
int mpo_launch_bilinear_z_fwd(const float* x0, const float* x1, int ld, const float* wz0, const float* wz1, float* zp, int B, int d,
                              hipStream_t s);
int mpo_launch_bilinear_gate_fwd(const float* zp, const float* bz0, const float* bz1, const float* h, float* sz, float* gated, int B,
                                 hipStream_t s);
int mpo_launch_bilinear_gate_bwd(const float* dgated, const float* h, const float* sz, float* dz, float* dh, int B, hipStream_t s);
int mpo_launch_bilinear_kron_fc1_fwd(const float* o, const float* W1, const float* b1, float* cat, int B, float p,
                                     unsigned long long seed, unsigned long long off, const unsigned long long* epoch, hipStream_t s);
int mpo_launch_bilinear_kron_fc1_bwd(const float* o, const float* W1, const float* cat, const float* dcat, float* dupre, float* d_o,
                                     float* dW1, float* db1, int B, float p, unsigned long long seed, unsigned long long off,
                                     const unsigned long long* epoch, hipStream_t s);
int mpo_launch_bilinear_z_bwd(const float* x0, const float* x1, int ld, const float* wz0, const float* wz1, const float* dz,
                              float* dwz0, float* dwz1, float* dbz0, float* dbz1, float* da_part, float* dx_part, float* dx0,
                              float* dx1, int B, int d, hipStream_t s);
int mpo_launch_ew_add(float* acc, const float* b, size_t n, hipStream_t s);
int mpo_launch_ew_mul(const float* a, const float* b, float* out, int n, hipStream_t s);
int mpo_launch_ew_mul2(const float* x, const float* p, const float* q, float* xp, float* xq, int n, hipStream_t s);
int mpo_launch_ew_add(const float* a, const float* b, float* out, int n, hipStream_t s);
int mpo_launch_cag_mid_fwd(const float* u1, const float* u2, const float* u3, const float* gw, const float* gb, const float* ew,
                           const float* eb, float* t1, float* t3, float* gout, float* eout, float* m, float* stats_g, float* stats_e,
                           int rows, int d, float eps, hipStream_t s);
int mpo_launch_cag_mid_bwd(const float* dm, const float* t1, const float* t3, const float* gout, const float* eout,
                           const float* gw, const float* ew, const float* stats_g, const float* stats_e, float* dG, float* dE,
                           float* ds12, float* ds3, int rows, int d, hipStream_t s);

int mpo_launch_bias_relu_dropout_bf16(void* h, const float* bias, size_t rows, int cols, float drop_p,
                                      unsigned long long seed, unsigned long long offset, const unsigned long long* epoch,
                                      hipStream_t stream);
int mpo_relu_dropout_bwd_blocks(size_t n, int with_colsum);
int mpo_launch_relu_dropout_bwd_bf16(const void* h, const void* dy, void* g, size_t n, float drop_p, int cols,
                                     float* part_colsum , hipStream_t stream);
int mpo_launch_colsum_bf16(const void* x, float* out, size_t rows, int cols, hipStream_t stream);

int mpo_launch_adam_flat(float* p, const float* g, float* m, float* v, size_t n, float lr, float b1, float b2, float eps,
                         float wd, int step, const int* step_dev, hipStream_t stream);
int mpo_launch_optim_flat(int algorithm, float* p, const float* g, float* s1, float* s2, size_t n, float lr,
                          const float* lr_dev, float b1, float b2, float eps, float wd, float l1, int step,
                          const int* step_dev, hipStream_t stream);
size_t mpo_abs_sum_partials(size_t n);
int mpo_launch_abs_sum(const float* x, size_t n, float* partials, float* out, hipStream_t stream);

int mpo_launch_bag_rowdot_gated(const void* bag, int bag_f32, const int* cu, int n_slides, int embed, const float* r1,
                                const float* r2, float* a_map, float* g_map, int n_q, const BagPlan& plan, hipStream_t stream);
int mpo_launch_bag_colacc_gated(const void* bag, int bag_f32, const int* cu, int n_slides, int embed, const float* w1map,
                                const float* w2map, float* part1, float* part2, int n_q, const BagPlan& plan,
                                hipStream_t stream);
int mpo_launch_bag_outer_gate(const int* cu, int n_slides, int embed, const float* w1, const float* z1, const void* addend,
                              const void* hbag, void* out, float gate, float* part_colsum, int n_q, const BagPlan& plan,
                              hipStream_t stream);
int mpo_launch_bag_key_grad(const float* kbag, const int* cu, int n_slides, int embed, const float* w1, const float* z1,
                            const float* w2, const float* z2, void* dk, int dk_f32, float* part_colsum, float* part1,
                            float* part2, int n_q, const BagPlan& plan, hipStream_t stream);
int mpo_launch_bag_outer_gated(const float* kbag, const int* cu, int n_slides, int embed, const float* w1, const float* z1,
                               const float* w2, const float* z2, void* dk, int dk_f32, float* part_colsum ,
                               int n_q, const BagPlan& plan, hipStream_t stream);

int mpo_launch_ces_loss_fwd(const float* hazards, const float* survs, const long long* label, const float* cens, float* loss,
                            float* risk, int B, int C, float alpha, float eps, hipStream_t s);
int mpo_launch_ces_loss_bwd(const float* hazards, const float* survs, const long long* label, const float* cens,
                            const float* d_loss, int d_loss_scalar, float* d_hazards, float* d_survs, int B, int C,
                            float alpha, float eps, hipStream_t s);

int mpo_launch_key_proj(const void* hbag_bf16, const float* w, const float* bias, float* kout, int rows, int embed,
                        hipStream_t stream);
```

multimodal_path_omic_amd/csrc/mpo_layout.h:

```cpp
#pragma once
#include <stddef.h>
#include <stdint.h>

#include <type_traits>

enum Placement {
    kWorkspace,
    kPad64,
    kPacked
};
constexpr size_t kWorkspaceSlack = 256;

template <Placement P>
inline size_t place_block(size_t& end, size_t n) {
    const size_t o = P == kWorkspace ? (end + 255) / 256 * 256 : end;
    end = o + (P == kPad64 ? (n + 63) / 64 * 64 : n) * sizeof(float);
    return o;
}

template <Placement P>
struct Count {
    using elem = float;
    size_t end = 0;
    float* floats(size_t n) { place_block<P>(end, n); return nullptr; }
    size_t n_floats() const { return end / sizeof(float); }
    size_t workspace_bytes() const { return end + kWorkspaceSlack; }
};

template <Placement P, typename T = float>
struct Carve {
    using elem = T;
    using Raw = typename std::conditional<std::is_const<T>::value, const void, void>::type;
    T* base;
    size_t size, end = 0;
    bool fits = true;
    explicit Carve(Raw* p, size_t bytes = SIZE_MAX) : base(static_cast<T*>(p)), size(bytes) {}
    T* floats(size_t n) {
        size_t e = end;
        const size_t o = place_block<P>(e, n);
        if (e > size) { fits = false; return nullptr; }
        end = e;
        return base + o / sizeof(float);
    }
    bool ok() const { return fits; }
};

using WsCount = Count<kWorkspace>;
using WsCarve = Carve<kWorkspace>;
```

multimodal_path_omic_amd/ops.py:

```python
from __future__ import annotations

import ctypes
import math
from dataclasses import dataclass
from typing import List, Optional

import torch

from . import _lib as L


plan_workgroups = None
wgrad_workgroups = None


@dataclass
class BagBatch:
    data: torch.Tensor
    cu: torch.Tensor
    lengths: List[int]
    _plan: object = None
    sampler_source = "window"
    cycle = False

    def __post_init__(self):
        if len(self.lengths) == 0 or any(int(m) <= 0 for m in self.lengths):
            raise ValueError(f"every slide of a window needs at least one patch row (lengths {list(self.lengths)[:8]}...)")
        if int(self.data.shape[0]) != sum(int(m) for m in self.lengths):
            raise ValueError(f"{int(self.data.shape[0])} rows for lengths summing to {sum(self.lengths)}")

    def plan(self):
        if self._plan is None:
            target = L.lib().mpo_coattn_target_workgroups()
            if plan_workgroups is not None:
                target = max(len(self.lengths), min(target, int(plan_workgroups)))
            rpw = -(-self.total_rows // target)
            rpw = max(32, -(-rpw // 32) * 32)
            while len(self.lengths) <= target and sum(-(-m // rpw) for m in self.lengths) > target:
                rpw += 32
            starts = [0]
            for m in self.lengths:
                starts.append(starts[-1] + -(-m // rpw))
            wg = torch.tensor(starts, dtype=torch.int32).to(self.data.device, non_blocking=True)
            c = L.BagPlanC(L.ptr(wg), starts[-1], rpw)
            self._plan = (wg, c)
        return ctypes.byref(self._plan[1])

    @property
    def n_slides(self):
        return len(self.lengths)

    @property
    def total_rows(self):
        return int(self.data.shape[0])

    @property
    def max_rows(self):
        return max(self.lengths)

    @property
    def width(self):
        return int(self.data.shape[1])

    @property
    def dtype(self):
        return self.data.dtype

    @property
    def device(self):
        return self.data.device

    def row_tensors(self):
        return [self.data]

    @staticmethod
    def from_list(bags: "List[torch.Tensor]") -> "BagBatch":
        lengths = [int(b.shape[0]) for b in bags]
        data = bags[0] if len(bags) == 1 else torch.cat(bags, 0)
        return BagBatch(data.contiguous(), make_cu(lengths, data.device), lengths)

    @staticmethod
    def from_lengths(data: torch.Tensor, lengths: "List[int]") -> "BagBatch":
        lengths = [int(m) for m in lengths]
        if int(data.shape[0]) != sum(lengths):
            raise ValueError(f"{int(data.shape[0])} rows for lengths summing to {sum(lengths)}")
        return BagBatch(data, make_cu(lengths, data.device), lengths)

    def with_data(self, data: torch.Tensor) -> "BagBatch":
        assert data.shape[0] == self.total_rows
        return BagBatch(data, self.cu, self.lengths, self._plan)

    def split_map(self, flat_map: torch.Tensor, n_q: int) -> "List[torch.Tensor]":
        out, off = RaggedMaps(), 0
        out.flat, out.batch, out.n_q = flat_map, self, n_q
        for m in self.lengths:
            out.append(flat_map[n_q * off:n_q * (off + m)].view(n_q, m))
            off += m
        return out


@dataclass
class SlideSet:
    slides: List[torch.Tensor]
    lengths: List[int]
    table_ptrs: torch.Tensor
    table_lens: torch.Tensor
    ids: torch.Tensor
    cycle: bool = False
    sampler_source = "slides"

    def __post_init__(self):
        self.lengths = [int(m) for m in self.lengths]
        if len(self.lengths) == 0 or any(m <= 0 for m in self.lengths):
            raise ValueError(f"every slide of a window needs at least one patch row (lengths {self.lengths[:8]}...)")
        if len(self.slides) != len(self.lengths) or int(self.ids.numel()) != len(self.lengths):
            raise ValueError(f"SlideSet: {len(self.slides)} slides, {len(self.lengths)} lengths and {int(self.ids.numel())} ids")
        if self.ids.dtype != torch.int32 or self.table_lens.dtype != torch.int32 or self.table_ptrs.dtype != torch.int64:
            raise ValueError("SlideSet: ids and table_lens are int32, table_ptrs int64 (device addresses)")
        if self.table_ptrs.numel() != self.table_lens.numel():
            raise ValueError("SlideSet: table_ptrs and table_lens differ in length")

    @property
    def n_slides(self):
        return len(self.lengths)

    @property
    def n_table(self):
        return int(self.table_lens.numel())

    @property
    def width(self):
        return int(self.slides[0].shape[1])

    @property
    def dtype(self):
        return self.slides[0].dtype

    @property
    def device(self):
        return self.slides[0].device

    def row_tensors(self):
        return self.slides

    @staticmethod
    def slide_table(slides: "List[torch.Tensor]"):
        for i, x in enumerate(slides):
            if x.dim() != 2 or not x.is_contiguous() or x.data_ptr() % 16:
                raise ValueError(f"SlideSet: slide {i} must be a contiguous (M, width) tensor whose first row is 16-byte aligned")
        dev = slides[0].device
        return (torch.tensor([x.data_ptr() for x in slides], dtype=torch.int64).to(dev, non_blocking=True),
                torch.tensor([int(x.shape[0]) for x in slides], dtype=torch.int32).to(dev, non_blocking=True))

    @staticmethod
    def from_batch(bags: "BagBatch", cycle: bool = False) -> "SlideSet":
        slides = list(bags.data.split(bags.lengths))
        ptrs, lens = SlideSet.slide_table(slides)
        ids = torch.arange(len(slides), dtype=torch.int32).to(bags.data.device, non_blocking=True)
        return SlideSet(slides, list(bags.lengths), ptrs, lens, ids, bool(cycle))

    def materialize(self) -> "BagBatch":
        return BagBatch.from_list(list(self.slides))


class RaggedMaps(list):
    flat: Optional[torch.Tensor] = None
    batch: Optional["BagBatch"] = None
    n_q: int = 0


def make_cu(lengths, device):
    cu = [0]
    for m in lengths:
        if m < 1:
            raise ValueError("every slide needs at least one patch")
        cu.append(cu[-1] + int(m))
    return torch.tensor(cu, dtype=torch.int32).to(device, non_blocking=True)


def grad_out(p):
    view = getattr(p, "_mpo_grad_view", None)
    if view is not None and p.grad is None and not getattr(p, "_mpo_slice_taken", False):
        p._mpo_slice_taken = True
        return view.view(p.shape)
    return torch.empty_like(p)


_rng_epoch_tensor = None


def set_rng_epoch(t):
    global _rng_epoch_tensor
    _rng_epoch_tensor = t


def _epoch():
    return L.ptr(_rng_epoch_tensor) if _rng_epoch_tensor is not None else None


def _workspace(nbytes, device):
    return torch.empty(max(int(nbytes), 256), dtype=torch.uint8, device=device)


class LinearFn(torch.autograd.Function):

    @staticmethod
    def forward(ctx, x, weight, bias, act: str = "none"):
        x2 = x.reshape(-1, x.shape[-1]).contiguous()
        y = torch.empty(x2.shape[0], weight.shape[0], device=x.device, dtype=torch.float32)
        L.call("mpo_linear_forward", L.ptr(x2), L.ptr(weight), L.ptr(bias), L.ptr(y), x2.shape[0],
               weight.shape[1], weight.shape[0], 1.0, L.ACT[act], L.stream_of(x))
        ctx.save_for_backward(x2, weight, y)
        ctx.act = act
        ctx.has_bias = bias is not None
        ctx.xshape = x.shape
        return y.view(*x.shape[:-1], weight.shape[0])

    @staticmethod
    def backward(ctx, dy):
        x2, weight, y = ctx.saved_tensors
        dy = dy.reshape(-1, dy.shape[-1]).contiguous()
        if ctx.act == "relu":
            dy = dy * (y > 0)
        elif ctx.act == "tanh":
            dy = dy * (1 - y * y)
        elif ctx.act == "sigmoid":
            dy = dy * (y * (1 - y))
        elif ctx.act == "elu":
            dy = dy * torch.where(y > 0, torch.ones_like(y), y + 1)
        dy = dy.contiguous()
        R, I, O = x2.shape[0], weight.shape[1], weight.shape[0]
        dx = torch.empty_like(x2) if ctx.needs_input_grad[0] else None
        dw = torch.empty_like(weight)
        db = torch.empty(O, device=dy.device, dtype=torch.float32) if ctx.has_bias else None
        s = L.stream_of(dy)
        if dx is not None:
            L.call("mpo_linear_backward_input", L.ptr(dy), L.ptr(weight), L.ptr(dx), R, I, O, 1.0, 0, s)
        L.call("mpo_linear_backward_weight", L.ptr(dy), L.ptr(x2), L.ptr(dw), L.ptr(db), R, I, O, 1.0, s)
        return (dx.view(ctx.xshape) if dx is not None else None), dw, db, None


def linear(x, weight, bias=None, act="none"):
    return LinearFn.apply(x, weight, bias, act)


class CoAttnMCATFn(torch.autograd.Function):

    @staticmethod
    def forward(ctx, query, bag_data, in_w, in_b, out_w, out_b, batch: BagBatch, need_weights: bool,
                bag_relu_gate: float = 0.0):
        lib = L.lib()
        ctx.set_materialize_grads(False)
        ctx.bag_relu_gate = float(bag_relu_gate)
        ctx.bag_bias = getattr(bag_data, "_mpo_bias_param", None)
        n_slides = batch.n_slides
        R, E = query.shape
        n_q = R // n_slides
        dev = query.device
        query = query.contiguous()
        out = torch.empty(R, E, device=dev, dtype=torch.float32)
        amap = torch.empty(n_q * batch.total_rows, device=dev, dtype=torch.float32) if need_weights else None
        saved = torch.empty(lib.mpo_coattn_saved_floats(n_slides, n_q, E), device=dev, dtype=torch.float32)
        ws = _workspace(lib.mpo_coattn_workspace_bytes(n_slides, n_q, E, batch.max_rows), dev)
        L.call("mpo_coattn_mcat_forward",
            L.ptr(bag_data), L.bag_dtype_code(bag_data), L.ptr(batch.cu), n_slides, batch.total_rows, batch.max_rows,
            L.ptr(query), n_q, E, L.ptr(in_w), L.ptr(in_b), L.ptr(out_w), L.ptr(out_b),
            L.ptr(out), L.ptr(amap), L.ptr(saved), batch.plan(), L.ptr(ws), ws.numel(), L.stream_of(query))
        ctx.save_for_backward(query, bag_data, in_w, out_w, saved, amap)
        ctx.param_refs = (in_w, in_b, out_w, out_b)
        ctx.batch = batch
        ctx.n_q = n_q
        return out, amap

    @staticmethod
    def backward(ctx, d_out, d_map):
        lib = L.lib()
        query, bag_data, in_w, out_w, saved, amap = ctx.saved_tensors
        batch, n_q = ctx.batch, ctx.n_q
        R, E = query.shape
        dev = query.device
        d_out = d_out.contiguous() if d_out is not None else torch.zeros(R, E, device=dev)
        if d_map is not None:
            d_map = d_map.contiguous()
        d_query = torch.empty_like(query)
        d_bag = torch.empty_like(bag_data)
        colsum = _bias_grad_slot(ctx.bag_bias, E, dev) if ctx.bag_relu_gate != 0.0 else None
        d_in_w, d_in_b, d_out_w, d_out_b = (grad_out(p) for p in ctx.param_refs)
        ws = _workspace(lib.mpo_coattn_workspace_bytes(batch.n_slides, n_q, E, batch.max_rows), dev)
        L.call("mpo_coattn_mcat_backward",
            L.ptr(bag_data), L.bag_dtype_code(bag_data), L.ptr(batch.cu), batch.n_slides, batch.total_rows,
            batch.max_rows, L.ptr(query), n_q, E, L.ptr(in_w), L.ptr(out_w), L.ptr(saved), L.ptr(amap),
            L.ptr(d_out), L.ptr(d_map), L.ptr(d_query), 0, L.ptr(d_bag), L.ptr(colsum), L.ptr(d_in_w), L.ptr(d_in_b),
            L.ptr(d_out_w), L.ptr(d_out_b), ctx.bag_relu_gate, batch.plan(), L.ptr(ws), ws.numel(), L.stream_of(query))
        if colsum is not None:
            d_bag._mpo_colsum = colsum
        return d_query, d_bag, d_in_w, d_in_b, d_out_w, d_out_b, None, None, None


def coattn_mcat(query, batch: BagBatch, in_w, in_b, out_w, out_b, need_weights: bool, bag_relu_gate: float = 0.0):
    return CoAttnMCATFn.apply(query, batch.data, in_w, in_b, out_w, out_b, batch, need_weights, bag_relu_gate)


stats = {"colsum_handoffs": 0, "qpass_in_place": 0, "qpass_copied": 0, "head_loss_ces": 0, "head_loss_sct": 0,
         "head_loss_ce": 0, "gated_concat_head": 0, "bilinear_head": 0}


def _query_grad_buffer(d_qpass, owned: bool, query):
    if d_qpass is None:
        return torch.empty_like(query), False
    if owned:
        stats["qpass_in_place"] += 1
        return d_qpass.contiguous(), True
    stats["qpass_copied"] += 1
    return d_qpass.clone(memory_format=torch.contiguous_format), True


def _bias_grad_slot(bag_param, E, dev):
    if bag_param is not None and getattr(bag_param, "_mpo_grad_view", None) is not None and bag_param.grad is None \
            and bag_param.numel() == E and not getattr(bag_param, "_mpo_slice_taken", False):
        return bag_param._mpo_grad_view.view(E)
    return torch.empty(E, device=dev, dtype=torch.float32)

defer_patch_weight_grad = False
_deferred_patch = []

def flush_patch_weight_grads():
    for g, x, dw in _deferred_patch:
        patch_weight_grad(g, x, dw)
    _deferred_patch.clear()

def _patch_weight_grad_now_or_deferred(g, x, dw, weight):
    if defer_patch_weight_grad and getattr(weight, "_mpo_grad_view", None) is not None \
            and dw.data_ptr() == weight._mpo_grad_view.data_ptr():
        _deferred_patch.append((g, x, dw))
    else:
        patch_weight_grad(g, x, dw)


class PatchFcFn(torch.autograd.Function):

    @staticmethod
    def forward(ctx, x, weight, bias, drop_p: float, pre_gated_grad: bool, batch=None):
        lib = L.lib()
        if not patch_fc_kernel_supported(x, weight):
            raise ValueError(f"patch layer: built for a contiguous bf16 window through Linear(512 | 1024 | 2048, 128 | 256 | 512) "
                             f"(patch_dim in {set(PATCH_DIMS)}; got {x.dtype} {tuple(x.shape)} through a weight {tuple(weight.shape)})")
        if batch is None:
            batch = BagBatch(x, make_cu([x.shape[0]], x.device), [x.shape[0]])
        h = torch.empty(x.shape[0], weight.shape[0], device=x.device, dtype=torch.bfloat16)
        realised = _realised_drop(drop_p) if drop_p > 0 else 0.0
        seed, off = _reserve(h.numel() // 16 + 2) if drop_p > 0 else (0, 0)
        ws = _workspace(lib.mpo_patch_fc_workspace_bytes(weight.shape[0], weight.shape[1]), x.device)
        L.call("mpo_patch_fc_forward", L.ptr(x), L.ptr(batch.cu), batch.n_slides, batch.total_rows, batch.max_rows,
               x.shape[1], L.ptr(weight), L.ptr(bias), weight.shape[0], float(drop_p), seed, off,
               _epoch(), L.ptr(h), batch.plan(), L.ptr(ws), ws.numel(), L.stream_of(x))
        ctx.save_for_backward(x, h)
        ctx.param_refs = (weight, bias)
        ctx.drop_p, ctx.pre_gated = float(realised), bool(pre_gated_grad)
        return h

    @staticmethod
    def backward(ctx, dh):
        lib = L.lib()
        x, h = ctx.saved_tensors
        dh = dh.contiguous()
        if ctx.pre_gated:
            g = dh
        else:
            g = None
        dw, db = (grad_out(p) for p in ctx.param_refs)
        if g is None:
            g = torch.empty_like(dh)
            ws = _workspace(lib.mpo_patch_epilogue_backward_workspace_bytes(g.numel(), g.shape[1]), g.device)
            L.call("mpo_patch_epilogue_backward", L.ptr(h), L.ptr(dh), L.ptr(g), g.numel(), g.shape[1], ctx.drop_p,
                   L.ptr(db), L.ptr(ws), ws.numel(), L.stream_of(g))
        else:
            ready = getattr(dh, "_mpo_colsum", None)
            if ready is not None and ready.shape == db.shape:
                if ready.data_ptr() != db.data_ptr():
                    db.copy_(ready)
                stats["colsum_handoffs"] += 1
            else:
                _colsum_two_stage(g, db)
        _patch_weight_grad_now_or_deferred(g, x, dw, ctx.param_refs[0])
        return None, dw, db, None, None, None


def _colsum_two_stage(g: torch.Tensor, out: torch.Tensor, block: int = 256) -> torch.Tensor:
    rows, d = g.shape
    main = rows // block * block
    if main:
        torch.sum(g[:main].view(rows // block, block, d).sum(1, dtype=torch.float32), 0, out=out)
    else:
        out.zero_()
    if main < rows:
        out += g[main:].sum(0, dtype=torch.float32)
    return out


def patch_weight_grad(g: torch.Tensor, x: torch.Tensor, out: torch.Tensor) -> torch.Tensor:
    e, k = out.shape
    if not (g.dtype == torch.bfloat16 and x.dtype == torch.bfloat16 and e in (128, 256, 512) and k in (128, 256, 512, 1024, 2048)
            and g.shape == (x.shape[0], e) and x.shape[1] == k
            and g.is_contiguous() and x.is_contiguous() and out.is_contiguous() and out.dtype == torch.float32):
        raise ValueError(f"patch weight gradient: g {g.dtype} {tuple(g.shape)} x {x.dtype} {tuple(x.shape)} -> {tuple(out.shape)} is not a "
                         f"geometry the kernel is built for (contiguous bf16, embed 128/256/512, patch_dim 128/256/512/1024/2048)")
    lib = L.lib()
    ws = _workspace(lib.mpo_patch_weight_grad_workspace_bytes(e, k), g.device)
    wgs = int(wgrad_workgroups or 0)
    if wgs and k != 1024:
        wgs = 0
    L.call("mpo_patch_weight_grad", L.ptr(g), L.ptr(x), g.shape[0], e, k, L.ptr(out), wgs, L.ptr(ws), ws.numel(),
           L.stream_of(g))
    return out


class PatchFcF32Fn(torch.autograd.Function):

    @staticmethod
    def forward(ctx, x, weight, bias, drop_p: float):
        lib = L.lib()
        h = torch.empty(x.shape[0], weight.shape[0], device=x.device, dtype=torch.float32)
        ctx.gate = 1.0 / (1.0 - _realised_drop(drop_p)) if drop_p > 0 else 1.0
        seed, off = _reserve(h.numel() // 16 + 2) if drop_p > 0 else (0, 0)
        ws = _workspace(lib.mpo_patch_fc_f32_workspace_bytes(0), x.device)
        scale_dev = getattr(x, "_mpo_feature_scale_dev", None)
        entry, scale = ("mpo_patch_fc_f32_forward", feature_scale(x)) if scale_dev is None else \
                       ("mpo_patch_fc_f32_forward_dev", L.ptr(_check_scale_tensor(scale_dev, x)))
        L.call(entry, L.ptr(x), x.shape[0], x.shape[1], L.ptr(weight), L.ptr(bias), weight.shape[0],
               float(drop_p), seed, off, _epoch(), scale, L.ptr(h), L.ptr(ws), ws.numel(),
               L.stream_of(x))
        ctx.save_for_backward(x, h)
        ctx.param_refs = (weight, bias)
        return h

    @staticmethod
    def backward(ctx, dh):
        lib = L.lib()
        x, h = ctx.saved_tensors
        dh = dh.contiguous()
        dw, db = (grad_out(p) for p in ctx.param_refs)
        ws = _workspace(lib.mpo_patch_fc_f32_workspace_bytes(1), x.device)
        L.call("mpo_patch_fc_f32_backward", L.ptr(dh), L.ptr(h), L.ptr(x), x.shape[0], h.shape[1], x.shape[1], ctx.gate, L.ptr(dw),
               L.ptr(db), L.ptr(ws), ws.numel(), L.stream_of(x))
        return None, dw, db, None


def feature_scale(x) -> float:
    if x.numel() == 0:
        return 1.0
    try:
        key = (x._version, x.data_ptr(), tuple(x.shape))
    except RuntimeError:
        key = None
    cached = getattr(x, "_mpo_feature_scale", None) if key is not None else None
    if cached is not None and cached[:3] == key:
        return cached[3]
    if x.is_cuda and torch.cuda.is_current_stream_capturing():
        raise RuntimeError("feature_scale(x) needs one host read: call ops.feature_scale(window.data) before capturing the graph")
    m = float(x.detach().abs().amax())
    s = math.ldexp(1.0, max(-100, min(100, 15 - math.frexp(m)[1]))) if (m > 0.0 and math.isfinite(m)) else 1.0
    if key is not None:
        try:
            x._mpo_feature_scale = (*key, s)
        except AttributeError:
            pass
    return s


def _check_scale_tensor(scale, x):
    if scale.shape != (1,) or scale.dtype != torch.float32 or scale.device != x.device or not scale.is_contiguous():
        raise ValueError(f"a device feature scale is one contiguous fp32 value on the window's device (got {tuple(scale.shape)} "
                         f"{scale.dtype} on {scale.device})")
    return scale


def feature_scale_device(x, out=None) -> torch.Tensor:
    if not x.is_cuda or x.dtype != torch.float32:
        raise ValueError(f"feature_scale_device: an fp32 tensor on the GPU (got {x.dtype} on {x.device})")
    out = torch.empty(1, dtype=torch.float32, device=x.device) if out is None else _check_scale_tensor(out, x)
    ws = _workspace(L.lib().mpo_feature_range_workspace_bytes(), x.device)
    L.call("mpo_feature_range_f32", L.ptr(x) if x.numel() else None, x.numel(), L.ptr(out), L.ptr(ws), ws.numel(), L.stream_of(x))
    return out


def patch_fc_f32_supported(x, weight) -> bool:
    return x.dtype == torch.float32 and x.is_contiguous() and tuple(weight.shape) == (256, 1024)


def patch_fc_f32(x, weight, bias, drop_p: float):
    return PatchFcF32Fn.apply(x, weight, bias, float(drop_p))


class PatchFcF16Fn(torch.autograd.Function):

    @staticmethod
    def forward(ctx, x, weight, bias, drop_p: float):
        lib = L.lib()
        if not patch_fc_f16_supported(x, weight):
            raise ValueError(f"fp16 patch layer: built for a contiguous fp16 window through Linear(1024, 256) (got {x.dtype} "
                             f"{tuple(x.shape)} through a weight {tuple(weight.shape)})")
        h = torch.empty(x.shape[0], weight.shape[0], device=x.device, dtype=torch.float32)
        ctx.drop_256 = int(round(_realised_drop(drop_p) * 256)) if drop_p > 0 else 0
        ctx.gate = 256.0 / (256.0 - ctx.drop_256)
        seed, off = _reserve(h.numel() // 16 + 2) if drop_p > 0 else (0, 0)
        ws = _workspace(lib.mpo_patch_fc_f16_workspace_bytes(0), x.device)
        L.call("mpo_patch_fc_f16_forward", L.ptr(x), x.shape[0], x.shape[1], L.ptr(weight), L.ptr(bias), weight.shape[0],
               ctx.drop_256, seed, off, _epoch(), L.ptr(h), L.ptr(ws), ws.numel(), L.stream_of(x))
        ctx.save_for_backward(x, h)
        ctx.param_refs = (weight, bias)
        return h

    @staticmethod
    def backward(ctx, dh):
        lib = L.lib()
        x, h = ctx.saved_tensors
        dh = dh.contiguous()
        dw, db = (grad_out(p) for p in ctx.param_refs)
        ws = _workspace(lib.mpo_patch_fc_f16_workspace_bytes(1), x.device)
        L.call("mpo_patch_fc_f16_backward", L.ptr(dh), L.ptr(h), L.ptr(x), x.shape[0], h.shape[1], x.shape[1], ctx.drop_256,
               L.ptr(dw), L.ptr(db), L.ptr(ws), ws.numel(), L.stream_of(x))
        return None, dw, db, None


def patch_fc_f16_supported(x, weight) -> bool:
    return x.dtype == torch.float16 and x.is_contiguous() and x.dim() == 2 and x.shape[1] == 1024 and tuple(weight.shape) == (256, 1024)


def patch_fc_f16(x, weight, bias, drop_p: float):
    return PatchFcF16Fn.apply(x, weight, bias, float(drop_p))


class PatchCoAttnMCATFn(torch.autograd.Function):

    @staticmethod
    def forward(ctx, x, patch_w, patch_b, query, in_w, in_b, out_w, out_b, batch: BagBatch, need_weights: bool, drop_p: float,
                tokens: "TokenPair | None" = None, qpass_owned: bool = False):
        lib = L.lib()
        ctx.set_materialize_grads(False)
        n_slides = batch.n_slides
        R, E = query.shape
        n_q = R // n_slides
        dev, T = query.device, batch.total_rows
        query = query.contiguous()
        h_bag = torch.empty(T, E, device=dev, dtype=torch.bfloat16)
        out = tokens.slot(0, (R, E)) if tokens is not None else torch.empty(R, E, device=dev, dtype=torch.float32)
        amap = torch.empty(n_q * T, device=dev, dtype=torch.float32) if need_weights else None
        saved = torch.empty(lib.mpo_coattn_saved_floats(n_slides, n_q, E), device=dev, dtype=torch.float32)
        ws = _workspace(lib.mpo_patch_coattn_workspace_bytes(n_slides, n_q, E, x.shape[1]), dev)
        ctx.gate = 1.0 / (1.0 - _realised_drop(drop_p)) if drop_p > 0 else 1.0
        seed, off = _reserve(T * E // 16 + 2) if drop_p > 0 else (0, 0)
        L.call("mpo_patch_coattn_mcat_forward",
            L.ptr(x), L.ptr(batch.cu), n_slides, T, batch.max_rows, x.shape[1], L.ptr(patch_w), L.ptr(patch_b), float(drop_p),
            seed, off, _epoch(), L.ptr(query), n_q, E, L.ptr(in_w), L.ptr(in_b), L.ptr(out_w), L.ptr(out_b),
            L.ptr(h_bag), L.ptr(out), L.ptr(amap), L.ptr(saved), batch.plan(), L.ptr(ws), ws.numel(), L.stream_of(query))
        ctx.save_for_backward(x, h_bag, query, in_w, out_w, saved, amap)
        ctx.param_refs = (patch_w, patch_b, in_w, in_b, out_w, out_b)
        ctx.batch, ctx.n_q = batch, n_q
        ctx.qpass_owned = bool(qpass_owned)
        ctx.mark_non_differentiable(h_bag)
        return out, amap, h_bag, query.view_as(query)

    @staticmethod
    def backward(ctx, d_out, d_map, _d_h, d_qpass):
        lib = L.lib()
        x, h_bag, query, in_w, out_w, saved, amap = ctx.saved_tensors
        batch, n_q = ctx.batch, ctx.n_q
        R, E = query.shape
        dev = query.device
        d_out = d_out.contiguous() if d_out is not None else torch.zeros(R, E, device=dev)
        d_map = d_map.contiguous() if d_map is not None else None
        d_query, accumulate = _query_grad_buffer(d_qpass, ctx.qpass_owned, query)
        g = torch.empty_like(h_bag)
        patch_w, patch_b, p_in_w, p_in_b, p_out_w, p_out_b = ctx.param_refs
        d_pw, d_pb = grad_out(patch_w), grad_out(patch_b)
        d_in_w, d_in_b, d_out_w, d_out_b = (grad_out(p) for p in (p_in_w, p_in_b, p_out_w, p_out_b))
        ws = _workspace(lib.mpo_coattn_workspace_bytes(batch.n_slides, n_q, E, batch.max_rows), dev)
        L.call("mpo_coattn_mcat_backward",
            L.ptr(h_bag), L.MPO_BF16, L.ptr(batch.cu), batch.n_slides, batch.total_rows, batch.max_rows, L.ptr(query), n_q, E,
            L.ptr(in_w), L.ptr(out_w), L.ptr(saved), L.ptr(amap), L.ptr(d_out), L.ptr(d_map), L.ptr(d_query), int(accumulate),
            L.ptr(g), L.ptr(d_pb), L.ptr(d_in_w), L.ptr(d_in_b), L.ptr(d_out_w), L.ptr(d_out_b), ctx.gate, batch.plan(),
            L.ptr(ws), ws.numel(), L.stream_of(query))
        stats["colsum_handoffs"] += 1
        _patch_weight_grad_now_or_deferred(g, x, d_pw, patch_w)
        return None, d_pw, d_pb, d_query, d_in_w, d_in_b, d_out_w, d_out_b, None, None, None, None, None


class TokenPair:

    def __init__(self, rows: int, d: int, device):
        self.buf = torch.empty(2, rows, d, device=device, dtype=torch.float32)

    def slot(self, i: int, shape):
        return self.buf[i].view(*shape)

    def stack(self, first, second):
        for i, t in enumerate((first, second)):
            if t.data_ptr() != self.buf[i].data_ptr() or t.numel() != self.buf[i].numel() or not t.is_contiguous():
                raise ValueError("TokenPair.stack: the halves must be the tensors produced into slot(0) and slot(1)")
        return _TokenPairFn.apply(first, second, self)


class _TokenPairFn(torch.autograd.Function):
    @staticmethod
    def forward(ctx, first, second, pair):
        ctx.shapes = (first.shape, second.shape)
        return pair.buf.view_as(pair.buf)

    @staticmethod
    def backward(ctx, d):
        return d[0].view(ctx.shapes[0]), d[1].view(ctx.shapes[1]), None


def _realised_drop(p: float) -> float:
    thr8 = int(p * 256.0 + 0.5)
    if thr8 > 255:
        raise ValueError(f"patch-layer dropout p = {p:g} is realised as round(256 p) / 256 = {thr8}/256: nothing would be kept "
                         f"(p must be below 1 - 1/512)")
    return float(thr8) / 256.0


def patch_coattn_mcat(x_bf16, batch: BagBatch, patch_w, patch_b, drop_p: float, query, in_w, in_b, out_w, out_b,
                      need_weights: bool, tokens: "TokenPair | None" = None, _qpass_owned: bool = False):
    return PatchCoAttnMCATFn.apply(x_bf16, patch_w, patch_b, query, in_w, in_b, out_w, out_b, batch, need_weights,
                                   float(drop_p), tokens, bool(_qpass_owned))


def fused_patch_coattn_supported(x, embed: int, n_q: int) -> bool:
    return x.dtype == torch.bfloat16 and x.shape[1] == 1024 and embed == 256 and n_q <= 8


PATCH_DIMS = (512, 1024, 2048)


def patch_fc_kernel_supported(x, weight) -> bool:
    return (x.dtype == torch.bfloat16 and x.is_contiguous() and x.dim() == 2 and weight.shape[0] in (128, 256, 512)
            and weight.shape[1] in PATCH_DIMS and x.shape[1] == weight.shape[1])


def patch_fc(x_bf16, weight, bias, drop_p: float, pre_gated_grad: bool = False, batch: "BagBatch | None" = None):
    h = PatchFcFn.apply(x_bf16, weight, bias, drop_p, pre_gated_grad, batch)
    if pre_gated_grad:
        h._mpo_bias_param = bias
    if drop_p > 0:
        h._mpo_keep_scale = 1.0 / (1.0 - _realised_drop(drop_p))
    return h


import torch.nn.functional as F


_rng_calls = 0


def _reserve(span: int):
    global _rng_calls
    seed = torch.initial_seed() & 0xFFFFFFFFFFFFFFFF
    off = _rng_calls
    _rng_calls += int(span) + 1
    return seed, off


def gated_scores(x, wa, ba, wb, bb, wc, bc, drop_p: float):
    a = linear(x, wa, ba, "tanh")
    b = linear(x, wb, bb, "sigmoid")
    if drop_p > 0.0:
        a = F.dropout(a, drop_p, True)
        b = F.dropout(b, drop_p, True)
    return linear(a * b, wc, bc)


class CagFn(torch.autograd.Function):

    @staticmethod
    def forward(ctx, q, q_hat, residual, dest, qpass_owned, *params):
        lib = L.lib()
        ctx.set_materialize_grads(False)
        q, q_hat = q.contiguous(), q_hat.contiguous()
        rows, dim = q.shape
        hidden = params[0].shape[0]
        c = torch.empty(rows, hidden, device=q.device, dtype=torch.float32)
        saved = torch.empty(lib.mpo_cag_saved_floats(rows, hidden), device=q.device, dtype=torch.float32)
        pa = L.ptr_array(params)
        total = None
        if residual is not None:
            residual = residual.contiguous()
            total = dest[0].slot(dest[1], (rows, hidden)) if dest is not None else torch.empty_like(c)
        L.call("mpo_cag_forward", L.ptr(q), L.ptr(q_hat), rows, dim, hidden, pa, L.ptr(c), L.ptr(saved), L.ptr(residual),
               L.ptr(total), L.stream_of(q))
        ctx.save_for_backward(q, q_hat, c, saved, *params)
        ctx.param_refs = params
        ctx.has_residual = residual is not None
        ctx.qpass_owned = bool(qpass_owned)
        return (total if total is not None else c), q.view_as(q)

    @staticmethod
    def backward(ctx, dc, d_qpass):
        lib = L.lib()
        q, q_hat, c, saved, *params = ctx.saved_tensors
        rows, dim = q.shape
        hidden = params[0].shape[0]
        if dc is None:
            dc = torch.zeros_like(c)
        dc = dc.contiguous()
        dq, accumulate = _query_grad_buffer(d_qpass, ctx.qpass_owned, q)
        dqh = torch.empty_like(q_hat)
        grads = [grad_out(p) for p in ctx.param_refs]
        ws = _workspace(lib.mpo_cag_workspace_bytes(rows, hidden), q.device)
        pa, ga = L.ptr_array(params), L.ptr_array(grads)
        L.call("mpo_cag_backward", L.ptr(q), L.ptr(q_hat), rows, dim, hidden, pa, L.ptr(saved), L.ptr(c),
               L.ptr(dc), L.ptr(dq), int(accumulate), L.ptr(dqh), ga, L.ptr(ws), ws.numel(),
               L.stream_of(q))
        return (dq, dqh, dc if ctx.has_residual else None, None, None, *grads)


def contextual_gate(q, q_hat, cag, residual=None, dest=None, hand_on: bool = False, _qpass_owned: bool = False):
    out, q_pass = CagFn.apply(q, q_hat, residual, dest, bool(_qpass_owned), cag.fc1[0].weight, cag.fc1[0].bias, cag.fc2[0].weight, cag.fc2[0].bias,
                              cag.fc3[0].weight, cag.fc3[0].bias, cag.G[1].weight, cag.G[1].bias,
                              cag.E[1].weight, cag.E[1].bias, cag.fc_c[0].weight, cag.fc_c[0].bias)
    return (out, q_pass) if hand_on else out


class EncoderFn(torch.autograd.Function):

    @staticmethod
    def forward(ctx, x, geom, drop_p, *params):
        lib = L.lib()
        branches, n_slides, T, d, ff, heads, layers = geom
        x = x.contiguous()
        y = torch.empty_like(x)
        saved = torch.empty(lib.mpo_encoder_saved_floats(branches * n_slides, T, d, ff, heads, layers), device=x.device,
                            dtype=torch.float32)
        seed, off = _reserve(lib.mpo_encoder_rng_span(branches * n_slides, T, d, ff, layers)) if drop_p > 0 else (0, 0)
        pa = L.ptr_array(params)
        L.call("mpo_encoder_forward", L.ptr(x), branches, n_slides, T, d, ff, heads, layers, pa, float(drop_p), seed, off,
               _epoch(), L.ptr(y), L.ptr(saved), L.stream_of(x))
        ctx.save_for_backward(x, saved, *params)
        ctx.param_refs = params
        ctx.geom, ctx.drop = geom, (float(drop_p), seed, off)
        return y

    @staticmethod
    def backward(ctx, dy):
        lib = L.lib()
        x, saved, *params = ctx.saved_tensors
        branches, n_slides, T, d, ff, heads, layers = ctx.geom
        drop_p, seed, off = ctx.drop
        dx = torch.empty_like(x)
        grads = [grad_out(p) for p in ctx.param_refs]
        ws = _workspace(lib.mpo_encoder_workspace_bytes(branches * n_slides, T, d, ff), x.device)
        pa, ga = L.ptr_array(params), L.ptr_array(grads)
        dy = dy.contiguous()
        L.call("mpo_encoder_backward",
            L.ptr(x), branches, n_slides, T, d, ff, heads, layers, pa, drop_p, seed, off, _epoch(), L.ptr(saved), L.ptr(dy),
            L.ptr(dx), ga, L.ptr(ws), ws.numel(), L.stream_of(x))
        return (dx, None, None, *grads)


def _encoder_params(layers):
    params = []
    for ly in layers:
        params += [ly.self_attn.in_proj_weight, ly.self_attn.in_proj_bias, ly.self_attn.out_proj.weight,
                   ly.self_attn.out_proj.bias, ly.linear1.weight, ly.linear1.bias, ly.linear2.weight, ly.linear2.bias,
                   ly.norm1.weight, ly.norm1.bias, ly.norm2.weight, ly.norm2.bias]
    return params


def _encoder_geom(layers):
    l0 = layers[0]
    return (l0.linear1.in_features, l0.linear1.out_features, l0.self_attn.num_heads, len(layers), l0.dropout.p)


def encoder(x, layers, training: bool):
    return encoder_branches([x], [layers], training)[0]


def encoder_branches(xs, layer_stacks, training: bool):
    if len(xs) == 1:
        return [encoder_stacked(xs[0].unsqueeze(0), layer_stacks, training)[0]]
    if any(x.shape != xs[0].shape for x in xs):
        raise ValueError("branch-batched encoders need identical input shapes")
    return list(encoder_stacked(torch.stack(list(xs)), layer_stacks, training).unbind(0))


def encoder_stacked(x, layer_stacks, training: bool):
    nb, b, t, d = x.shape
    g0 = _encoder_geom(layer_stacks[0])
    if len(layer_stacks) != nb or any(_encoder_geom(ls) != g0 for ls in layer_stacks) or g0[0] != d:
        raise ValueError("branch-batched encoders need one layer stack per branch, all of identical geometry")
    params = [p for ls in layer_stacks for p in _encoder_params(ls)]
    geom = (nb, b, t, d, g0[1], g0[2], g0[3])
    y = EncoderFn.apply(x.reshape(nb * b * t, d), geom, g0[4] if training else 0.0, *params)
    return y.view(nb, b, t, d)


class BagSelfAttentionFn(torch.autograd.Function):

    @staticmethod
    def forward(ctx, qkv, heads: int, drop_p: float, need_map: bool):
        lib = L.lib()
        n_bags, m, d3 = qkv.shape
        d = d3 // 3
        qkv = qkv.contiguous()
        out = torch.empty((n_bags, m, d), device=qkv.device, dtype=torch.float32)
        saved = torch.empty(lib.mpo_bag_self_attention_saved_floats(n_bags, m, d, heads), device=qkv.device, dtype=torch.float32)
        amap = torch.empty((n_bags, m, m), device=qkv.device, dtype=torch.float32) if need_map else None
        seed, off = _reserve(1) if drop_p > 0 else (0, 0)
        L.call("mpo_bag_self_attention_forward", L.ptr(qkv), n_bags, m, d, heads, float(drop_p), seed, off, _epoch(), L.ptr(out),
               L.ptr(saved), L.ptr(amap), L.stream_of(qkv))
        ctx.save_for_backward(qkv, out, saved)
        ctx.geom, ctx.drop = (n_bags, m, d, heads), (float(drop_p), seed, off)
        if amap is not None:
            ctx.mark_non_differentiable(amap)
        return out, amap

    @staticmethod
    def backward(ctx, d_out, _d_map):
        lib = L.lib()
        qkv, out, saved = ctx.saved_tensors
        n_bags, m, d, heads = ctx.geom
        drop_p, seed, off = ctx.drop
        d_qkv = torch.empty_like(qkv)
        ws = _workspace(lib.mpo_bag_self_attention_workspace_bytes(n_bags, m, d, heads), qkv.device)
        d_out = d_out.contiguous()
        L.call("mpo_bag_self_attention_backward", L.ptr(qkv), L.ptr(out), L.ptr(saved), L.ptr(d_out), n_bags, m, d, heads, drop_p,
               seed, off, _epoch(), L.ptr(d_qkv), L.ptr(ws), ws.numel(), L.stream_of(qkv))
        return d_qkv, None, None, None


def bag_self_attention(x, mha, training: bool, need_weights: bool = True):
    if mha.in_proj_weight is None or mha.bias_k is not None or mha.add_zero_attn:
        raise NotImplementedError("bag self-attention: packed in_proj, no bias_k / zero-attn (the reference's constructor)")
    if need_weights and mha.num_heads != 1:
        raise NotImplementedError("bag self-attention: the M x M map is returned for one head (models/ge_nacagat/ge_nacagat.py:27)")
    xb = x if x.dim() == 3 else x.unsqueeze(0)
    qkv = linear(xb.float(), mha.in_proj_weight, mha.in_proj_bias)
    out, amap = BagSelfAttentionFn.apply(qkv, mha.num_heads, mha.dropout if training else 0.0, bool(need_weights))
    out = linear(out, mha.out_proj.weight, mha.out_proj.bias)
    if x.dim() == 2:
        out, amap = out[0], (amap[0] if amap is not None else None)
    return out, amap


class GatedPoolFn(torch.autograd.Function):

    @staticmethod
    def forward(ctx, x, geom, head_p, rho_p, interleave, *params):
        lib = L.lib()
        ctx.set_materialize_grads(False)
        branches, n_slides, Lr, d = geom
        bt = branches * n_slides
        x = x.contiguous()
        scores = torch.empty(bt * Lr, device=x.device, dtype=torch.float32)
        h = torch.empty((n_slides, branches * d) if interleave else (bt, d), device=x.device, dtype=torch.float32)
        saved = torch.empty(lib.mpo_gated_pool_saved_floats(bt, Lr, d), device=x.device, dtype=torch.float32)
        seed, off = _reserve(lib.mpo_gated_pool_rng_span(bt, Lr, d)) if (head_p > 0 or rho_p > 0) else (0, 0)
        pa = L.ptr_array(params)
        L.call("mpo_gated_pool_forward", L.ptr(x), branches, n_slides, Lr, d, pa, float(head_p), float(rho_p), seed, off,
               _epoch(), L.ptr(scores), L.ptr(h), int(interleave), L.ptr(saved), L.stream_of(x))
        ctx.save_for_backward(x, saved, h, *params)
        ctx.param_refs = params
        ctx.geom, ctx.drop, ctx.interleave = geom, (float(head_p), float(rho_p)), bool(interleave)
        return scores, h

    @staticmethod
    def backward(ctx, d_scores, dh):
        lib = L.lib()
        x, saved, h, *params = ctx.saved_tensors
        branches, n_slides, Lr, d = ctx.geom
        head_p, rho_p = ctx.drop
        dx = torch.empty_like(x)
        grads = [grad_out(p) for p in ctx.param_refs]
        if dh is None:
            dh = torch.zeros_like(h)
        ws = _workspace(lib.mpo_gated_pool_workspace_bytes(branches * n_slides, Lr, d), x.device)
        pa, ga = L.ptr_array(params), L.ptr_array(grads)
        dh = dh.contiguous()
        d_sc = d_scores.contiguous() if d_scores is not None else None
        L.call("mpo_gated_pool_backward",
            L.ptr(x), branches, n_slides, Lr, d, pa, head_p, rho_p, L.ptr(saved), L.ptr(h), L.ptr(dh), int(ctx.interleave),
            L.ptr(d_sc), L.ptr(dx), ga, L.ptr(ws), ws.numel(), L.stream_of(x))
        return (dx, None, None, None, None, *grads)


def gated_pool(tokens, head, rho, training: bool):
    return gated_pool_branches([tokens], [head], [rho], training)[0]

# ... 780 lines not shown
```

Before: 30530 slides/s.

## Emit bag gradient in low-rank coefficient form and rebuild it inside patch wgrad

```diff
diff --git a/include/mpo_hip.h b/include/mpo_hip.h
--- a/include/mpo_hip.h
+++ b/include/mpo_hip.h
@@ -83,6 +83,8 @@
                              float* d_out_proj_weight, float* d_out_proj_bias,
                              float bag_relu_gate, const mpo_bag_plan* plan ,
                              void* workspace, size_t workspace_bytes, mpo_stream_t stream);
+#define MPO_DBAG_COEFFICIENTS 2
+#define MPO_WGRAD_G_COEFFICIENTS 65536
 
 int mpo_patch_epilogue_forward(void* h_bf16, const float* bias, int64_t rows, int cols, float drop_p, uint64_t seed,
                                uint64_t offset, const uint64_t* rng_epoch, mpo_stream_t stream);
diff --git a/multimodal_path_omic_amd/csrc/capi.hip b/multimodal_path_omic_amd/csrc/capi.hip
--- a/multimodal_path_omic_amd/csrc/capi.hip
+++ b/multimodal_path_omic_amd/csrc/capi.hip
@@ -338,6 +338,13 @@
                              void* workspace, size_t workspace_bytes, mpo_stream_t stream) {
     RC(check_common(bag_dtype, n_slides, total_rows, max_rows, n_q, embed));
     MPO_CHECK(!d_attn_map || attn_map, "coattn backward: a gradient on the attention map needs the forward's map");
+    const bool coef_form = (d_query_accumulate & MPO_DBAG_COEFFICIENTS) != 0;
+    d_query_accumulate &= 1;
+    const BagCoefLayout coef_at = bag_coef_layout((size_t)total_rows, (size_t)n_slides);
+    MPO_CHECK(!coef_form || (bag_dtype == MPO_BF16 && embed == 256 && n_q <= 8 && !d_attn_map && d_bag && bag_relu_gate != 0.f && coef_at.ok),
+              "coattn backward: d_bag in coefficient form is built for a gated bf16 bag of embed 256, at most 8 queries, no map "
+              "gradient and at least %d rows per slide on average (got dtype %d, embed %d, n_q %d, %d rows in %d slides)",
+              43, bag_dtype, embed, n_q, total_rows, n_slides);
     const int E = embed, R = n_slides * n_q;
     const BagPlan plan = make_plan(plan_, n_slides, max_rows);
     RC(check_plan(plan, n_slides));
@@ -358,6 +365,11 @@
         RC(mpo_launch_rowdot(W.dctx, S.ctx, W.delta, R, E, stream));
         RC(mpo_launch_map_rowdot(attn_map, d_attn_map, cu_rows, W.delta, n_slides, n_q, 1, stream));
     }
+    if (coef_form)
+        RC(mpo_launch_coattn_bwd8_coef(bag, cu_rows, S.qk2, S.lse2, W.dctx, S.ctx, d_bag,
+                                       reinterpret_cast<float*>(static_cast<char*>(d_bag) + coef_at.u_offset), W.part_dqk, W.part_cs, n_q,
+                                       plan, bag_relu_gate, stream));
+    else
     RC(mpo_launch_coattn_bwd(bag, bag_dtype == MPO_F32, cu_rows, n_slides, E, S.qk2, S.lse2, W.dctx, d_attn_map ? W.delta : nullptr,
                              S.ctx, attn_map, d_attn_map, d_bag, W.part_dqk, W.part_cs, n_q, plan, bag_relu_gate, stream));
     {
@@ -678,6 +690,14 @@
     WsCarve ws(workspace, workspace_bytes);
     float* part = ws.floats(mpo_patch_wgrad_partial_floats(embed, patch_dim));
     MPO_CHECK(ws.ok(), "patch weight gradient: workspace too small (%zu bytes)", workspace_bytes);
+    if (workgroups & MPO_WGRAD_G_COEFFICIENTS) {
+        MPO_CHECK(embed == 256 && bag_coef_layout((size_t)total_rows, 1).ok,
+                  "patch weight gradient: g in coefficient form is built for embed 256 and at least 43 rows (got %d, %lld)", embed,
+                  (long long)total_rows);
+        const float* u = reinterpret_cast<const float*>(static_cast<const char*>(g_bf16) + bag_coef_layout((size_t)total_rows, 1).u_offset);
+        return mpo_launch_patch_wgrad_hc(g_bf16, u, patches_bf16, (int)total_rows, patch_dim, part, d_weight,
+                                         workgroups & ~MPO_WGRAD_G_COEFFICIENTS, static_cast<hipStream_t>(stream));
+    }
     return mpo_launch_patch_wgrad(g_bf16, patches_bf16, total_rows, embed, patch_dim, part, d_weight, workgroups,
                                   static_cast<hipStream_t>(stream));
 }
diff --git a/multimodal_path_omic_amd/csrc/coattn_bwd8.hip b/multimodal_path_omic_amd/csrc/coattn_bwd8.hip
--- a/multimodal_path_omic_amd/csrc/coattn_bwd8.hip
+++ b/multimodal_path_omic_amd/csrc/coattn_bwd8.hip
@@ -1,5 +1,6 @@
 #include "coattn_tile.h"
 #include "mpo_kernels.h"
+#include "mpo_layout.h"
 
 namespace {
 
@@ -44,7 +45,18 @@
 }
 
 typedef __attribute__((ext_vector_type(4))) unsigned u32x4;
-
+__device__ __forceinline__ unsigned nz_byte8(bf16x8 v) {
+    const u32x4 x = __builtin_bit_cast(u32x4, v);
+    unsigned out = 0;
+#pragma unroll
+    for (int k = 0; k < 4; ++k) {
+        const unsigned u = ((x[k] & 0x7FFF7FFFu) + 0x7FFF7FFFu) & 0x80008000u;
+        out |= (((u >> 15) | (u >> 30)) & 3u) << (2 * k);
+    }
+    return out;
+}
+
+template <bool COEF>
 __global__ __launch_bounds__(W8 * 64, 1)
 void coattn_bwd8_kernel(const __bf16* __restrict__ bag, const int* __restrict__ cu,
                         const float* __restrict__ qk2,
@@ -56,7 +68,9 @@
                         float* __restrict__ part_dqk,
                         float* __restrict__ part_colsum,
                         int n_q, BagPlan plan,
-                        float relu_gate ) {
+                        float relu_gate ,
+                        char* __restrict__ rec,
+                        float* __restrict__ u_out           ) {
     __shared__ __attribute__((aligned(1024))) char lds[LDS8];
     const int tid = threadIdx.x;
     const int lane = tid & 63;
@@ -108,8 +122,20 @@
             *reinterpret_cast<bf16x8*>(dst) = h;
             *reinterpret_cast<bf16x8*>(dst + QF8_ARR) = l;
         }
+        if constexpr (COEF) {
+            if (r0 == 0) {
+                const float us = relu_gate != 0.f ? relu_gate : 1.0f;
+                float* ub = u_out + (size_t)b * 16 * E8;
+                for (int e = tid; e < 16 * E8; e += W8 * 64) {
+                    const int k = e >> 8, d = e & (E8 - 1), qq = k & 7;
+                    float v = 0.f;
+                    if (qq < n_q) v = k < 8 ? dc_b[qq * E8 + d] * us : qk_b[qq * E8 + d] * (us * kLn2);
+                    ub[e] = v;
+                }
+            }
+        }
         const float zs = relu_gate != 0.f ? relu_gate : 1.0f;
-        for (int e = tid; e < G8::DT * 32; e += W8 * 64) {
+        for (int e = tid; e < (COEF ? 0 : G8::DT * 32); e += W8 * 64) {
             const int i = e & 15, gg = (e >> 4) & 1, t = e >> 5;
             float z[8];
 #pragma unroll
@@ -158,6 +184,9 @@
     f32x4 accq[G8::DT];
 #pragma unroll
     for (int t = 0; t < G8::DT; ++t) accq[t] = f32x4{0.f, 0.f, 0.f, 0.f};
+    f32x4 accm[COEF ? G8::DT : 1];
+#pragma unroll
+    for (int t = 0; t < (COEF ? G8::DT : 1); ++t) accm[t] = f32x4{0.f, 0.f, 0.f, 0.f};
     float csum[8];
 #pragma unroll
     for (int j = 0; j < 8; ++j) csum[j] = 0.f;
@@ -171,9 +200,10 @@
         const int ec = el & 15, eg = el >> 4;
         asm volatile("s_waitcnt vmcnt(0)" ::: "memory");
 
-        bf16x8 wph[2], wh, wl;
+        bf16x8 wph[2], wh, wl, mh, ml;
         {
             f32x4 sT[2], dT[2], sN[2], dN[2];
+            unsigned mk[2][2] = {{0u, 0u}, {0u, 0u}};
 #pragma unroll
             for (int pt = 0; pt < 2; ++pt) sT[pt] = dT[pt] = sN[pt] = dN[pt] = f32x4{0.f, 0.f, 0.f, 0.f};
             const char* qf = lds + OFF_QF8 + ((eg * QS + (ec & 7)) << 4);
@@ -181,23 +211,31 @@
             for (int s = 0; s < G8::KS; ++s) {
                 const bf16x8 a0 = row_frag8(img, 0, s, el);
                 const bf16x8 a1 = row_frag8(img, 1, s, el);
+                if constexpr (COEF) {
+                    mk[0][s >> 2] |= nz_byte8(a0) << (8 * (s & 3));
+                    mk[1][s >> 2] |= nz_byte8(a1) << (8 * (s & 3));
+                }
                 const char* qs = qf + s * (4 * QS * 16);
                 const bf16x8 qh = *reinterpret_cast<const bf16x8*>(qs);
                 const bf16x8 ql = *reinterpret_cast<const bf16x8*>(qs + QF8_ARR);
                 const bf16x8 dh = *reinterpret_cast<const bf16x8*>(qs + 2 * QF8_ARR);
                 const bf16x8 dl = *reinterpret_cast<const bf16x8*>(qs + 3 * QF8_ARR);
-                sT[0] = mfma_bf16(qh, a0, sT[0]);
-                sT[1] = mfma_bf16(qh, a1, sT[1]);
-                dT[0] = mfma_bf16(dh, a0, dT[0]);
-                dT[1] = mfma_bf16(dh, a1, dT[1]);
+                if constexpr (!COEF) {
+                    sT[0] = mfma_bf16(qh, a0, sT[0]);
+                    sT[1] = mfma_bf16(qh, a1, sT[1]);
+                    dT[0] = mfma_bf16(dh, a0, dT[0]);
+                    dT[1] = mfma_bf16(dh, a1, dT[1]);
+                }
                 sN[0] = mfma_bf16(a0, qh, sN[0]);
                 sN[1] = mfma_bf16(a1, qh, sN[1]);
                 dN[0] = mfma_bf16(a0, dh, dN[0]);
                 dN[1] = mfma_bf16(a1, dh, dN[1]);
-                sT[0] = mfma_bf16(ql, a0, sT[0]);
-                sT[1] = mfma_bf16(ql, a1, sT[1]);
-                dT[0] = mfma_bf16(dl, a0, dT[0]);
-                dT[1] = mfma_bf16(dl, a1, dT[1]);
+                if constexpr (!COEF) {
+                    sT[0] = mfma_bf16(ql, a0, sT[0]);
+                    sT[1] = mfma_bf16(ql, a1, sT[1]);
+                    dT[0] = mfma_bf16(dl, a0, dT[0]);
+                    dT[1] = mfma_bf16(dl, a1, dT[1]);
+                }
                 sN[0] = mfma_bf16(a0, ql, sN[0]);
                 sN[1] = mfma_bf16(a1, ql, sN[1]);
                 dN[0] = mfma_bf16(a0, dl, dN[0]);
@@ -206,17 +244,26 @@
 #pragma unroll
             for (int pt = 0; pt < 2; ++pt) {
                 const bool ok = 16 * pt + ec < nvalid;
-                float w[8];
-#pragma unroll
-                for (int r = 0; r < 4; ++r) {
-                    const float a = ok ? __builtin_amdgcn_exp2f(sT[pt][r] - lse_p[r]) : 0.f;
-                    w[r] = a;
-                    w[4 + r] = a * (dT[pt][r] - del_p[r]);
-                }
-                bf16x8 lo_unused;
-                pack_hi_lo(w, wph[pt], lo_unused);
-            }
-            float ds[8];
+                if constexpr (COEF) {
+                    if (ok) {
+                        char* rp = rec + (size_t)(row_begin + trow + 16 * pt + ec) * kBagRecBytes;
+                        typedef __attribute__((ext_vector_type(2))) unsigned u32x2;
+                        *reinterpret_cast<u32x2*>(rp + 64 + 8 * eg) = u32x2{mk[pt][0], mk[pt][1]};
+                        if (eg == 3) *reinterpret_cast<int*>(rp + 96) = b;
+                    }
+                } else {
+                    float w[8];
+#pragma unroll
+                    for (int r = 0; r < 4; ++r) {
+                        const float a = ok ? __builtin_amdgcn_exp2f(sT[pt][r] - lse_p[r]) : 0.f;
+                        w[r] = a;
+                        w[4 + r] = a * (dT[pt][r] - del_p[r]);
+                    }
+                    bf16x8 lo_unused;
+                    pack_hi_lo(w, wph[pt], lo_unused);
+                }
+            }
+            float ds[8], cm[8];
 #pragma unroll
             for (int pt = 0; pt < 2; ++pt)
 #pragma unroll
@@ -224,17 +271,42 @@
                     const bool ok = 16 * pt + 4 * eg + r < nvalid;
                     const float a = ok ? __builtin_amdgcn_exp2f(sN[pt][r] - lse_q) : 0.f;
                     ds[4 * pt + r] = a * (dN[pt][r] - del_q);
+                    cm[4 * pt + r] = a;
                 }
             pack_hi_lo(ds, wh, wl);
+            if constexpr (COEF) {
+#pragma unroll
+                for (int j = 0; j < 8; ++j) {
+                    const float up = __shfl_up(ds[j], 8, 16);
+                    cm[j] = ec < 8 ? cm[j] : up;
+                }
+                pack_hi_lo(cm, mh, ml);
+#pragma unroll
+                for (int j = 0; j < 8; ++j) {
+                    const int row = (j < 4 ? 0 : 12) + 4 * eg + j;
+                    if (row < nvalid)
+                        *reinterpret_cast<float*>(rec + (size_t)(row_begin + trow + row) * kBagRecBytes + 4 * ec) = cm[j];
+                }
+            }
         }
 #pragma unroll
         for (int t = 0; t < G8::DT; ++t) {
             const bf16x8 hf = col_frag8(img, t, el);
             accq[t] = mfma_bf16(hf, wh, accq[t]);
             accq[t] = mfma_bf16(hf, wl, accq[t]);
-        }
-
-        {
+            if constexpr (COEF) {
+                if (part_colsum != nullptr) {
+                    u32x4 hv = __builtin_bit_cast(u32x4, hf);
+#pragma unroll
+                    for (int k = 0; k < 4; ++k) hv[k] = ((((hv[k] & 0x7FFF7FFFu) + 0x7FFF7FFFu) & 0x80008000u) >> 15) * 0x3F80u;
+                    const bf16x8 one = __builtin_bit_cast(bf16x8, hv);
+                    accm[t] = mfma_bf16(one, mh, accm[t]);
+                    accm[t] = mfma_bf16(one, ml, accm[t]);
+                }
+            }
+        }
+
+        if constexpr (!COEF) {
             const int row = 16 * (eg & 1) + ec;
             char* rowp = img + row * G8::ROWB;
             const int swz = sw8(row), chi = eg >> 1;
@@ -267,7 +339,7 @@
         __builtin_amdgcn_fence(__ATOMIC_RELEASE, "wavefront");
         __builtin_amdgcn_wave_barrier();
 
-        {
+        if constexpr (!COEF) {
             const int rl = el >> 5, cc = el & 31;
 #pragma unroll
             for (int i = 0; i < 16; ++i) {
@@ -301,7 +373,34 @@
         for (int w = 0; w < W8; ++w) a += reinterpret_cast<const float*>(lds + w * G8::TILEB)[idx];
         part_dqk[pbase * n_q * E8 + idx] = a;
     }
-    if (part_colsum != nullptr) {
+    if constexpr (COEF) {
+        if (part_colsum != nullptr) {
+            __syncthreads();
+            const float us = relu_gate != 0.f ? relu_gate : 1.0f;
+            const int qq = c16 & 7;
+            const float* urow = (c16 < 8 ? dc_b : qk_b) + (qq < n_q ? qq : 0) * E8;
+            const float uscale = qq < n_q ? (c16 < 8 ? us : us * kLn2) : 0.f;
+            float* wq = reinterpret_cast<float*>(img);
+#pragma unroll
+            for (int t = 0; t < G8::DT; ++t) {
+                const f32x4 uv = *reinterpret_cast<const f32x4*>(urow + 16 * t + 4 * g);
+                f32x4 v;
+#pragma unroll
+                for (int r = 0; r < 4; ++r) v[r] = accm[t][r] * (uv[r] * uscale);
+                *reinterpret_cast<f32x4*>(wq + c16 * E8 + 16 * t + 4 * g) = v;
+            }
+            __syncthreads();
+            for (int idx = tid; idx < E8; idx += W8 * 64) {
+                float a = 0.f;
+#pragma unroll
+                for (int w = 0; w < W8; ++w)
+#pragma unroll
+                    for (int k = 0; k < 16; ++k) a += reinterpret_cast<const float*>(lds + w * G8::TILEB)[k * E8 + idx];
+                part_colsum[pbase * E8 + idx] = a;
+            }
+        }
+    }
+    if (!COEF && part_colsum != nullptr) {
         __syncthreads();
 #pragma unroll
         for (int j = 0; j < 8; ++j) csum[j] += __shfl_xor(csum[j], 32);
@@ -339,9 +438,23 @@
                            const BagPlan& plan, float relu_gate, hipStream_t stream) {
     MPO_CHECK(n_q >= 1 && n_q <= 8, "coattn backward (8 waves): 1..8 queries (got %d)", n_q);
     MPO_CHECK(delta || ctx, "coattn backward: delta or ctx");
-    coattn_bwd8_kernel<<<plan_grid(plan), W8 * 64, 0, stream>>>(
+    coattn_bwd8_kernel<false><<<plan_grid(plan), W8 * 64, 0, stream>>>(
         reinterpret_cast<const __bf16*>(bag), cu, qk2, lse2, dctx, delta, ctx, reinterpret_cast<__bf16*>(dbag), part_dqk,
-        part_colsum, n_q, plan, relu_gate);
+        part_colsum, n_q, plan, relu_gate, nullptr, nullptr);
     MPO_LAUNCH_CHECK();
     return 0;
 }
+
+int mpo_launch_coattn_bwd8_coef(const void* bag, const int* cu, const float* qk2, const float* lse2, const float* dctx,
+                                const float* ctx, void* records, float* u, float* part_dqk, float* part_colsum, int n_q,
+                                const BagPlan& plan, float relu_gate, hipStream_t stream) {
+    MPO_CHECK(n_q >= 1 && n_q <= 8, "coattn backward (coefficient form): 1..8 queries (got %d)", n_q);
+    MPO_CHECK(ctx && records && u, "coattn backward (coefficient form): null argument");
+    MPO_CHECK(((reinterpret_cast<uintptr_t>(records) | reinterpret_cast<uintptr_t>(u)) & 15) == 0,
+              "coattn backward (coefficient form): d_bag must be 16-byte aligned");
+    coattn_bwd8_kernel<true><<<plan_grid(plan), W8 * 64, 0, stream>>>(
+        reinterpret_cast<const __bf16*>(bag), cu, qk2, lse2, dctx, nullptr, ctx, nullptr, part_dqk, part_colsum, n_q, plan,
+        relu_gate, static_cast<char*>(records), u);
+    MPO_LAUNCH_CHECK();
+    return 0;
+}
diff --git a/multimodal_path_omic_amd/csrc/mpo_kernels.h b/multimodal_path_omic_amd/csrc/mpo_kernels.h
--- a/multimodal_path_omic_amd/csrc/mpo_kernels.h
+++ b/multimodal_path_omic_amd/csrc/mpo_kernels.h
@@ -138,6 +138,11 @@
 int mpo_launch_coattn_bwd8(const void* bag, const int* cu, const float* qk2, const float* lse2, const float* dctx,
                            const float* delta, const float* ctx, void* dbag, float* part_dqk, float* part_colsum, int n_q,
                            const BagPlan& plan, float relu_gate, hipStream_t stream);
+int mpo_launch_coattn_bwd8_coef(const void* bag, const int* cu, const float* qk2, const float* lse2, const float* dctx,
+                                const float* ctx, void* records, float* u, float* part_dqk, float* part_colsum, int n_q,
+                                const BagPlan& plan, float relu_gate, hipStream_t stream);
+int mpo_launch_patch_wgrad_hc(const void* records, const float* u, const void* x_bf16, int total_rows, int patch_dim, float* part,
+                              float* d_weight, int workgroups, hipStream_t stream);
 size_t mpo_patch_fc_f32_workspace_floats();
 size_t mpo_patch_wgrad_f32_workspace_floats();
 int mpo_launch_patch_fc_f32(const float* x, const float* w, const float* bias, float* h, long long total_rows, int embed,
diff --git a/multimodal_path_omic_amd/csrc/mpo_layout.h b/multimodal_path_omic_amd/csrc/mpo_layout.h
--- a/multimodal_path_omic_amd/csrc/mpo_layout.h
+++ b/multimodal_path_omic_amd/csrc/mpo_layout.h
@@ -47,3 +47,14 @@
 
 using WsCount = Count<kWorkspace>;
 using WsCarve = Carve<kWorkspace>;
+
+constexpr size_t kBagRecBytes = 128;
+constexpr size_t kBagCoefUFloats = 16 * 256;
+struct BagCoefLayout { size_t u_offset, end; bool ok; };
+inline BagCoefLayout bag_coef_layout(size_t total_rows, size_t n_slides) {
+    BagCoefLayout l;
+    l.u_offset = total_rows * kBagRecBytes;
+    l.end = l.u_offset + n_slides * kBagCoefUFloats * sizeof(float);
+    l.ok = l.end <= total_rows * 256 * 2;
+    return l;
+}
diff --git a/multimodal_path_omic_amd/csrc/patch_wgrad_hc.hip b/multimodal_path_omic_amd/csrc/patch_wgrad_hc.hip
--- /dev/null
+++ b/multimodal_path_omic_amd/csrc/patch_wgrad_hc.hip
@@ -0,0 +1,241 @@
+#include "coattn_tile.h"
+#include "mpo_kernels.h"
+#include "mpo_layout.h"
+
+namespace {
+
+constexpr int HC_E = 256;
+constexpr int HC_CB = 256;
+constexpr int HC_BK = 32;
+constexpr int HC_STAGES = 4;
+constexpr int HC_TILE = HC_BK * 512;
+constexpr int HC_REC = HC_BK * (int)kBagRecBytes;
+constexpr int HC_STAGE = HC_TILE + HC_REC;
+constexpr int HC_LDS = HC_STAGES * HC_STAGE;
+constexpr int HC_WAVES = 4;
+constexpr int HC_WGS = 256;
+static_assert(HC_LDS <= 160 * 1024, "LDS budget");
+static_assert(kBagRecBytes == 128, "record addressing below");
+
+typedef __attribute__((ext_vector_type(4))) unsigned hc_u32x4;
+
+__device__ __forceinline__ f32x4 mfma16(s16x4 a, s16x4 b, f32x4 c) {
+    return __builtin_amdgcn_mfma_f32_16x16x16bf16_1k(a, b, c, 0, 0, 0);
+}
+__device__ __forceinline__ void split4(const f32x4 v, s16x4& hi, s16x4& lo) {
+    bf16x4 h, l;
+#pragma unroll
+    for (int j = 0; j < 4; ++j) {
+        __bf16 a, b;
+        split_bf16(v[j], a, b);
+        h[j] = a;
+        l[j] = b;
+    }
+    hi = __builtin_bit_cast(s16x4, h);
+    lo = __builtin_bit_cast(s16x4, l);
+}
+__device__ __forceinline__ void hc_wait_vm(int chunks_younger) {
+    switch (chunks_younger) {
+        case 0: asm volatile("s_waitcnt vmcnt(0)" ::: "memory"); break;
+        case 1: asm volatile("s_waitcnt vmcnt(5)" ::: "memory"); break;
+        default: asm volatile("s_waitcnt vmcnt(10)" ::: "memory"); break;
+    }
+}
+__device__ __forceinline__ void hc_dma16(unsigned off, const char* base, unsigned dst) {
+#pragma clang diagnostic push
+#pragma clang diagnostic ignored "-Winline-asm"
+    asm volatile("s_mov_b32 m0, %2\n\ts_nop 0\n\tglobal_load_lds_dwordx4 %0, %1" :: "v"(off), "s"(base), "s"(dst) : "memory", "m0");
+#pragma clang diagnostic pop
+}
+
+__global__ __launch_bounds__(HC_WAVES * 64, 1)
+void patch_wgrad_hc_kernel(const char* __restrict__ rec, const float* __restrict__ u, const __bf16* __restrict__ x, int total_rows,
+                           int patch_dim, int rows_per_range, int slide_max ,
+                           float* __restrict__ part) {
+    __shared__ __attribute__((aligned(1024))) char lds[HC_LDS];
+    const int lane = threadIdx.x & 63;
+    const int wave = __builtin_amdgcn_readfirstlane(threadIdx.x >> 6);
+    const int n_cb = patch_dim / HC_CB;
+    const int xcd = blockIdx.x & 7, slot = blockIdx.x >> 3;
+    const int rr = xcd + 8 * (slot / n_cb), cb = slot % n_cb;
+    const int rb = min(total_rows, rr * rows_per_range), re = min(total_rows, rb + rows_per_range);
+    const int n_chunks = (re - rb + HC_BK - 1) / HC_BK;
+
+    const char* x_base = reinterpret_cast<const char*>(x) + (size_t)cb * HC_CB * 2;
+    const unsigned x_row = (unsigned)patch_dim * 2u;
+    auto issue = [&](int chunk) {
+        char* stage = lds + (chunk % HC_STAGES) * HC_STAGE;
+        const unsigned sdst = (unsigned)(uintptr_t)(__attribute__((address_space(3))) char*)stage;
+        const int row0 = rb + chunk * HC_BK;
+#pragma unroll
+        for (int i = 0; i < 4; ++i) {
+            const int k = 4 * wave + i;
+            const int r = 2 * k + (lane >> 5), cs = lane & 31;
+            const unsigned c16 = (unsigned)((cs ^ ((r & 7) << 1)) * 16);
+            const unsigned grow = (unsigned)min(row0 + r, total_rows - 1);
+            hc_dma16(grow * x_row + c16, x_base, sdst + k * 1024);
+        }
+        {
+            const unsigned grow = (unsigned)min(row0 + 8 * wave + (lane >> 3), total_rows - 1);
+            hc_dma16(grow * (unsigned)kBagRecBytes + (unsigned)((lane & 7) * 16), rec, sdst + HC_TILE + wave * 1024);
+        }
+    };
+    auto arrive = [&](int m) {
+        hc_wait_vm(min(HC_STAGES - 2, n_chunks - 1 - m));
+        asm volatile("s_waitcnt lgkmcnt(0)\n\ts_barrier" ::: "memory");
+        if (m + HC_STAGES - 1 < n_chunks) issue(m + HC_STAGES - 1);
+    };
+
+    f32x4 acc[4][16];
+#pragma unroll
+    for (int i = 0; i < 4; ++i)
+#pragma unroll
+        for (int j = 0; j < 16; ++j) acc[i][j] = f32x4{0.f, 0.f, 0.f, 0.f};
+
+    int sl_loaded = -1;
+    s16x4 uh[4], ul[4];
+#pragma unroll
+    for (int i = 0; i < 4; ++i) uh[i] = ul[i] = s16x4{0, 0, 0, 0};
+    auto load_u = [&](int b) {
+        const float* ub = u + (size_t)b * kBagCoefUFloats + (size_t)(4 * (lane >> 4)) * HC_E + 64 * wave + (lane & 15);
+#pragma unroll
+        for (int i = 0; i < 4; ++i) {
+            const f32x4 v = {ub[16 * i], ub[HC_E + 16 * i], ub[2 * HC_E + 16 * i], ub[3 * HC_E + 16 * i]};
+            split4(v, uh[i], ul[i]);
+        }
+    };
+
+    bf16x8 ga[4], xf[16];
+    auto build = [&](int m, bf16x8 (&out)[4]) {
+        const char* recs = lds + (m % HC_STAGES) * HC_STAGE + HC_TILE;
+        const int c0 = rb + m * HC_BK, n_valid = min(HC_BK, re - c0);
+        f32x4 cv[2];
+        int sid[2];
+#pragma unroll
+        for (int rt = 0; rt < 2; ++rt) {
+            const char* rp = recs + (16 * rt + (lane & 15)) * (int)kBagRecBytes;
+            cv[rt] = *reinterpret_cast<const f32x4*>(rp + (lane >> 4) * 16);
+            sid[rt] = *reinterpret_cast<const int*>(rp + 96);
+        }
+        unsigned mbit[4];
+#pragma unroll
+        for (int i = 0; i < 4; ++i) {
+            const int d = 64 * wave + 16 * i + (lane & 15);
+            const char* mp = recs + 64 + 8 * ((d >> 3) & 3) + (d >> 5);
+            unsigned bits = 0;
+#pragma unroll
+            for (int j = 0; j < 8; ++j) {
+                const int row = (j < 4 ? 4 * (lane >> 4) + j : 16 + 4 * (lane >> 4) + (j - 4));
+                const unsigned byte = *reinterpret_cast<const unsigned char*>(mp + row * (int)kBagRecBytes);
+                bits |= ((byte >> (d & 7)) & 1u) << j;
+            }
+            mbit[i] = bits;
+        }
+        const int s_first = min(max(__builtin_amdgcn_readfirstlane(*reinterpret_cast<const int*>(recs + 96)), 0), slide_max);
+        const int s_last = min(__builtin_amdgcn_readfirstlane(*reinterpret_cast<const int*>(recs + (n_valid - 1) * (int)kBagRecBytes + 96)), slide_max);
+        f32x4 bo[4][2];
+#pragma unroll
+        for (int i = 0; i < 4; ++i) bo[i][0] = bo[i][1] = f32x4{0.f, 0.f, 0.f, 0.f};
+        for (int b = s_first; b <= s_last; ++b) {
+            if (b != sl_loaded) {
+                load_u(b);
+                sl_loaded = b;
+            }
+#pragma unroll
+            for (int rt = 0; rt < 2; ++rt) {
+                const bool in = sid[rt] == b && 16 * rt + (lane & 15) < n_valid;
+                const f32x4 z4 = {0.f, 0.f, 0.f, 0.f};
+                s16x4 ch, cl;
+                split4(in ? cv[rt] : z4, ch, cl);
+#pragma unroll
+                for (int i = 0; i < 4; ++i) {
+                    bo[i][rt] = mfma16(ch, uh[i], bo[i][rt]);
+                    bo[i][rt] = mfma16(cl, uh[i], bo[i][rt]);
+                    bo[i][rt] = mfma16(ch, ul[i], bo[i][rt]);
+                }
+            }
+        }
+#pragma unroll
+        for (int i = 0; i < 4; ++i) {
+            const bf16x8 gb = {f2bf(bo[i][0][0]), f2bf(bo[i][0][1]), f2bf(bo[i][0][2]), f2bf(bo[i][0][3]),
+                               f2bf(bo[i][1][0]), f2bf(bo[i][1][1]), f2bf(bo[i][1][2]), f2bf(bo[i][1][3])};
+            hc_u32x4 gv = __builtin_bit_cast(hc_u32x4, gb);
+#pragma unroll
+            for (int k = 0; k < 4; ++k) {
+                const unsigned two = (mbit[i] >> (2 * k)) & 3u;
+                gv[k] &= (two & 1u) * 0xFFFFu + (two >> 1) * 0xFFFF0000u;
+            }
+            out[i] = __builtin_bit_cast(bf16x8, gv);
+        }
+    };
+
+    for (int c = 0; c < min(HC_STAGES - 1, n_chunks); ++c) issue(c);
+    if (n_chunks > 0) {
+        arrive(0);
+        build(0, ga);
+#pragma unroll
+        for (int j = 0; j < 16; ++j) xf[j] = col_frag<HC_E>(lds, j, lane);
+    }
+    for (int m = 0; m < n_chunks; ++m) {
+        const int nxt = min(m + 1, n_chunks - 1);
+        bf16x8 gn[4];
+        if (m + 1 < n_chunks) arrive(m + 1);
+        const char* xt = lds + (nxt % HC_STAGES) * HC_STAGE;
+#pragma unroll
+        for (int j = 0; j < 16; ++j) {
+#pragma unroll
+            for (int i = 0; i < 4; ++i) acc[i][j] = mfma_bf16(ga[i], xf[j], acc[i][j]);
+            xf[j] = col_frag<HC_E>(xt, j, lane);
+            if (j == 3) build(nxt, gn);
+            __builtin_amdgcn_sched_barrier(0);
+        }
+#pragma unroll
+        for (int i = 0; i < 4; ++i) ga[i] = gn[i];
+    }
+
+    float* out = part + ((size_t)rr * HC_E) * patch_dim + (size_t)cb * HC_CB;
+#pragma unroll
+    for (int i = 0; i < 4; ++i)
+#pragma unroll
+        for (int j = 0; j < 16; ++j)
+#pragma unroll
+            for (int r = 0; r < 4; ++r)
+                out[(size_t)(16 * (4 * wave + i) + 4 * (lane >> 4) + r) * patch_dim + 16 * j + (lane & 15)] = acc[i][j][r];
+}
+
+__global__ __launch_bounds__(256)
+void patch_wgrad_hc_reduce_kernel(const float* __restrict__ part, float* __restrict__ out, int n4, int n_parts) {
+    const int i = blockIdx.x * 256 + threadIdx.x;
+    if (i >= n4) return;
+    f32x4 a = {0.f, 0.f, 0.f, 0.f};
+#pragma unroll 8
+    for (int s = 0; s < n_parts; ++s) a += *reinterpret_cast<const f32x4*>(part + ((size_t)s * n4 + i) * 4);
+    *reinterpret_cast<f32x4*>(out + (size_t)i * 4) = a;
+}
+
+}
+
+int mpo_launch_patch_wgrad_hc(const void* records, const float* u, const void* x, int total_rows, int patch_dim, float* part,
+                              float* d_weight, int workgroups, hipStream_t stream) {
+    MPO_CHECK(patch_dim >= HC_CB && patch_dim % HC_CB == 0 && (256 % (patch_dim / HC_CB)) == 0 && patch_dim <= 2048,
+              "patch weight gradient (coefficient form): built for embed 256 and patch_dim in {256, 512, 1024, 2048} (got %d)", patch_dim);
+    MPO_CHECK(total_rows >= 1, "patch weight gradient (coefficient form): no rows");
+    MPO_CHECK((int64_t)total_rows * patch_dim * 2 < ((int64_t)1 << 32),
+              "patch weight gradient (coefficient form): the patch matrix must stay below 4 GiB (%d rows of %d)", total_rows, patch_dim);
+    MPO_CHECK(((reinterpret_cast<uintptr_t>(records) | reinterpret_cast<uintptr_t>(x) | reinterpret_cast<uintptr_t>(u)) & 15) == 0,
+              "patch weight gradient (coefficient form): operands must be 16-byte aligned");
+    const int n_cb = patch_dim / HC_CB;
+    MPO_CHECK(workgroups == 0 || (workgroups >= 8 * n_cb && workgroups <= HC_WGS && workgroups % (8 * n_cb) == 0),
+              "patch weight gradient: workgroups must be 0 or a multiple of %d up to %d (got %d)", 8 * n_cb, HC_WGS, workgroups);
+    const int ranges = (workgroups ? workgroups : HC_WGS) / n_cb;
+    const int rpr = ((total_rows + ranges - 1) / ranges + HC_BK - 1) / HC_BK * HC_BK;
+    const int slide_max = (int)(((size_t)total_rows * 512 - bag_coef_layout((size_t)total_rows, 0).u_offset) / (kBagCoefUFloats * sizeof(float))) - 1;
+    MPO_CHECK(slide_max >= 0, "patch weight gradient (coefficient form): %d rows leave no room for a slide's factor", total_rows);
+    patch_wgrad_hc_kernel<<<ranges * n_cb, HC_WAVES * 64, 0, stream>>>(static_cast<const char*>(records), u, static_cast<const __bf16*>(x),
+                                                                      total_rows, patch_dim, rpr, slide_max, part);
+    MPO_LAUNCH_CHECK();
+    const int n4 = HC_E * patch_dim / 4;
+    patch_wgrad_hc_reduce_kernel<<<(n4 + 255) / 256, 256, 0, stream>>>(part, d_weight, n4, ranges);
+    MPO_LAUNCH_CHECK();
+    return 0;
+}
diff --git a/multimodal_path_omic_amd/ops.py b/multimodal_path_omic_amd/ops.py
--- a/multimodal_path_omic_amd/ops.py
+++ b/multimodal_path_omic_amd/ops.py
@@ -324,17 +324,26 @@
 defer_patch_weight_grad = False
 _deferred_patch = []
 
+bag_grad_coefficients = True
+MPO_DBAG_COEFFICIENTS = 2
+MPO_WGRAD_G_COEFFICIENTS = 65536
+
+
+def bag_grad_coefficients_supported(total_rows: int, n_slides: int, patch_dim: int, d_map) -> bool:
+    return (d_map is None and total_rows * 128 + n_slides * 16 * 256 * 4 <= total_rows * 512
+            and total_rows * patch_dim * 2 < 1 << 32)
+
 def flush_patch_weight_grads():
-    for g, x, dw in _deferred_patch:
-        patch_weight_grad(g, x, dw)
+    for g, x, dw, coefficients in _deferred_patch:
+        patch_weight_grad(g, x, dw, coefficients)
     _deferred_patch.clear()
 
-def _patch_weight_grad_now_or_deferred(g, x, dw, weight):
+def _patch_weight_grad_now_or_deferred(g, x, dw, weight, coefficients=False):
     if defer_patch_weight_grad and getattr(weight, "_mpo_grad_view", None) is not None \
             and dw.data_ptr() == weight._mpo_grad_view.data_ptr():
-        _deferred_patch.append((g, x, dw))
+        _deferred_patch.append((g, x, dw, coefficients))
     else:
-        patch_weight_grad(g, x, dw)
+        patch_weight_grad(g, x, dw, coefficients)
 
 
 class PatchFcFn(torch.autograd.Function):
@@ -398,7 +407,7 @@
     return out
 
 
-def patch_weight_grad(g: torch.Tensor, x: torch.Tensor, out: torch.Tensor) -> torch.Tensor:
+def patch_weight_grad(g: torch.Tensor, x: torch.Tensor, out: torch.Tensor, coefficients: bool = False) -> torch.Tensor:
     e, k = out.shape
     if not (g.dtype == torch.bfloat16 and x.dtype == torch.bfloat16 and e in (128, 256, 512) and k in (128, 256, 512, 1024, 2048)
             and g.shape == (x.shape[0], e) and x.shape[1] == k
@@ -410,6 +419,8 @@
     wgs = int(wgrad_workgroups or 0)
     if wgs and k != 1024:
         wgs = 0
+    if coefficients:
+        wgs |= MPO_WGRAD_G_COEFFICIENTS
     L.call("mpo_patch_weight_grad", L.ptr(g), L.ptr(x), g.shape[0], e, k, L.ptr(out), wgs, L.ptr(ws), ws.numel(),
            L.stream_of(g))
     return out
@@ -572,17 +583,18 @@
         d_map = d_map.contiguous() if d_map is not None else None
         d_query, accumulate = _query_grad_buffer(d_qpass, ctx.qpass_owned, query)
         g = torch.empty_like(h_bag)
+        coefficients = bool(bag_grad_coefficients) and bag_grad_coefficients_supported(batch.total_rows, batch.n_slides, x.shape[1], d_map)
         patch_w, patch_b, p_in_w, p_in_b, p_out_w, p_out_b = ctx.param_refs
         d_pw, d_pb = grad_out(patch_w), grad_out(patch_b)
         d_in_w, d_in_b, d_out_w, d_out_b = (grad_out(p) for p in (p_in_w, p_in_b, p_out_w, p_out_b))
         ws = _workspace(lib.mpo_coattn_workspace_bytes(batch.n_slides, n_q, E, batch.max_rows), dev)
         L.call("mpo_coattn_mcat_backward",
             L.ptr(h_bag), L.MPO_BF16, L.ptr(batch.cu), batch.n_slides, batch.total_rows, batch.max_rows, L.ptr(query), n_q, E,
-            L.ptr(in_w), L.ptr(out_w), L.ptr(saved), L.ptr(amap), L.ptr(d_out), L.ptr(d_map), L.ptr(d_query), int(accumulate),
-            L.ptr(g), L.ptr(d_pb), L.ptr(d_in_w), L.ptr(d_in_b), L.ptr(d_out_w), L.ptr(d_out_b), ctx.gate, batch.plan(),
+            L.ptr(in_w), L.ptr(out_w), L.ptr(saved), L.ptr(amap), L.ptr(d_out), L.ptr(d_map), L.ptr(d_query),
+            int(accumulate) | (MPO_DBAG_COEFFICIENTS if coefficients else 0), L.ptr(g), L.ptr(d_pb), L.ptr(d_in_w), L.ptr(d_in_b), L.ptr(d_out_w), L.ptr(d_out_b), ctx.gate, batch.plan(),
             L.ptr(ws), ws.numel(), L.stream_of(query))
         stats["colsum_handoffs"] += 1
-        _patch_weight_grad_now_or_deferred(g, x, d_pw, patch_w)
+        _patch_weight_grad_now_or_deferred(g, x, d_pw, patch_w, coefficients)
         return None, d_pw, d_pb, d_query, d_in_w, d_in_b, d_out_w, d_out_b, None, None, None, None, None
 
 
```

Result: slower. 25070 slides/s (-17.9%).
